# AlessioSam/LADiff

Measured on AMD Instinct MI355X. Metric: motions/sec (196-frame, 50-step DDIM, bs128), higher is better.
Workload: dtype f16x3+f32; 1 GPU; headline:ddim50_cfg7.5_b128_f196_c263_humanml3d; prompts_per_gpu=128, global_batch=128, frames=196, scheduler=ddim, denoising_steps=50, parallelism=dp1, loop=persistent pipeline kernel (16-row blocks x 86)

## Files before the change

### ladiff_amd/csrc/api.hip

```cpp
#include <algorithm>
#include <cstdlib>
#include <cstring>
#include <vector>

#include "model.h"
#include "sampler.h"
#include "../../include/ladiff_hip_debug.h"

using namespace ladiff;

namespace {

inline hipStream_t S(ladiff_stream_t s) { return reinterpret_cast<hipStream_t>(s); }

bool all_set(const float* const* w, size_t n) {
    if (w == nullptr) return false;
    for (size_t i = 0; i < n; ++i)
        if (w[i] == nullptr) return false;
    return true;
}
template <class W>
bool load_weights(W& dst, const float* const* ptrs) {
    if (!all_set(ptrs, sizeof(W) / sizeof(const float*))) return false;
    std::memcpy(&dst, ptrs, sizeof(W));
    return true;
}
const char* name_at(const std::vector<std::string>& n, int i) { return (i >= 0 && i < (int)n.size()) ? n[i].c_str() : nullptr; }

}

#ifdef LADIFF_STAMPS
static unsigned long long* g_stamps = nullptr;
#endif

extern "C" {

int ladiff_version(void) { return LADIFF_ABI_VERSION; }
int ladiff_split_format(void) {
#ifndef LADIFF_SPLIT_BF16
    return 1;
#else
    return 0;
#endif
}

const char* ladiff_error_string(int code) {
    switch (code) {
        case LADIFF_OK: return "ok";
        case LADIFF_ERR_ARG: return "invalid argument (null pointer or negative size)";
        case LADIFF_ERR_SHAPE: return "shape not supported by the gfx950 kernels";
        case LADIFF_ERR_WORKSPACE: return "workspace too small";
        case LADIFF_ERR_UNSUPPORTED: return "configuration branch not built";
        default: return code > 0 ? hipGetErrorString((hipError_t)code) : "unknown ladiff error";
    }
}

int ladiff_denoiser_num_params(void) { return DEN_NPARAMS; }
const char* ladiff_denoiser_param_name(int i) { return name_at(denoiser_param_names(), i); }
int ladiff_decoder_num_params(void) { return DEC_NPARAMS; }
const char* ladiff_decoder_param_name(int i) { return name_at(decoder_param_names(), i); }

int ladiff_gemm(const float* A, int lda, const float* A2, int lda2, int K1, const float* W, int ldw, const float* bias,
                const float* res, int ldres, const float* ln_gamma, const float* ln_beta, float* Y, int ldy, int M,
                int N, int K, int act, ladiff_stream_t stream) {
    LADIFF_CHECK_ARG(A && W && Y && M >= 0 && N > 0 && K > 0);
    GemmArgs g;
    g.A = A; g.lda = lda; g.A2 = A2; g.lda2 = lda2; g.K1 = A2 ? K1 : K; g.W = W; g.ldw = ldw; g.bias = bias;
    g.res = res; g.ldres = ldres; g.ln_g = ln_gamma; g.ln_b = ln_beta; g.Y = Y; g.ldy = ldy; g.M = M; g.N = N; g.K = K;
    g.act = act;
    return launch_gemm(g, S(stream));
}

int ladiff_gemm_resident(const float* A, int lda, const float* A2, int lda2, int K1, const float* W, int ldw,
                         const float* bias, const float* res, int ldres, float* Y, int ldy, int M, int N, int K, int act,
                         int split, float* Ys, ladiff_stream_t stream) {
    LADIFF_CHECK_ARG(A && W && (Y || Ys) && M >= 0 && N > 0 && K > 0);
    if (M == 0) return 0;
    KrArgs g;
    g.A = A; g.lda = lda; g.A2 = A2; g.lda2 = lda2; g.K1 = A2 ? K1 : K; g.W = W; g.ldw = ldw; g.bias = bias;
    g.res = res; g.ldres = ldres; g.Y = Y; g.ldy = ldy; g.M = M; g.N = N; g.K = K; g.act = act;
    g.split = split; g.Ys = Ys;
#ifdef LADIFF_STAMPS
    g.stamps = g_stamps;
#endif
    return launch_gemm_kr(g, S(stream));
}

int ladiff_gemm_split(const float* A, int lda, const float* A2, int lda2, int K1, const float* W, int ldw, const float* bias,
                      const float* res, int ldres, float* Y, float* Ys, int ldy, int M, int N, int K, int act,
                      ladiff_stream_t stream) {
    LADIFF_CHECK_ARG(A && W && (Y || Ys) && M >= 0 && N > 0 && K > 0);
    if (M == 0) return 0;
    GemmArgs g;
    g.A = A; g.lda = lda; g.A2 = A2; g.lda2 = lda2; g.K1 = A2 ? K1 : K; g.W = W; g.ldw = ldw; g.bias = bias;
    g.res = res; g.ldres = ldres; g.Y = Y; g.Ys = Ys; g.ldy = ldy; g.M = M; g.N = N; g.K = K; g.act = act; g.split = 1;
    return launch_gemm(g, S(stream));
}

#ifdef LADIFF_STAMPS
void ladiff_debug_set_stamps(unsigned long long* p) { g_stamps = p; }
void ladiff_debug_set_sys_stamps(unsigned long long* p) { ladiff::g_sys_stamps = p; }
void ladiff_debug_set_probe(int v) { ladiff::g_sys_probe = v; }
#endif

int ladiff_combine_rows(const float* partials, int n_planes, int M, const float* bias, const float* res, int mode,
                        const float* ln_gamma, const float* ln_beta, const float* table, const int32_t* counts, int Bs,
                        int T, int pad_row, float* out, ladiff_stream_t stream) {
    LADIFF_CHECK_ARG(partials && out && n_planes > 0 && M >= 0 && Bs > 0 && T > 0);
    if (mode != RED_PLAIN && mode != RED_LN && mode != RED_LN_ADD && mode != RED_LN_MOD) return LADIFF_ERR_ARG;
    if (mode != RED_PLAIN && !(ln_gamma && ln_beta)) return LADIFF_ERR_ARG;
    if ((mode == RED_LN_ADD || mode == RED_LN_MOD) && !table) return LADIFF_ERR_ARG;
    if (M == 0) return 0;
    return launch_reduce_rows(partials, n_planes, M, bias, res, mode, ln_gamma, ln_beta, table, 0, nullptr, counts, Bs, T,
                              pad_row, 0, out, nullptr, S(stream));
}

int ladiff_layernorm(const float* x, const float* gamma, const float* beta, float* y, int M, ladiff_stream_t stream) {
    LADIFF_CHECK_ARG(x && gamma && beta && y && M >= 0);
    return launch_layernorm(x, gamma, beta, y, M, S(stream));
}

int ladiff_timestep_sinusoid(const int64_t* timesteps, int n, float* out, ladiff_stream_t stream) {
    LADIFF_CHECK_ARG(timesteps && out && n >= 0);
    if (n == 0) return 0;
    return launch_sinusoid(timesteps, n, out, S(stream));
}

int ladiff_decoder_self_attention(const float* qkv, const int32_t* lengths, const uint32_t* keybits, float* out, int B,
                                  int F, ladiff_stream_t stream) {
    LADIFF_CHECK_ARG(qkv && (lengths || keybits) && out && B >= 0);
    return launch_decoder_self_attention(qkv, lengths, keybits, out, B, F, 0, S(stream));
}

int ladiff_self_attention_split(const float* qkv, const int32_t* lengths, const uint32_t* keybits, float* out, int B, int F,
                                 int nheads, int causal, ladiff_stream_t stream) {
    LADIFF_CHECK_ARG(qkv && out && B >= 0);
    return launch_self_attention_split(qkv, lengths, keybits, out, B, F, nheads, causal, 0, S(stream));
}

int ladiff_decoder_cross_attention(const float* q, const float* kv, const int32_t* counts, float* out, int B, int F,
                                   int T, ladiff_stream_t stream) {
    LADIFF_CHECK_ARG(q && kv && out && B >= 0 && F >= 0);
    return launch_decoder_cross_attention(q, kv, counts, out, B, F, T, 0, S(stream));
}

size_t ladiff_denoiser_tables_floats(int n_steps) { return den_tables_floats(n_steps); }
size_t ladiff_denoiser_text_cache_floats(int B2, int n_steps, int n_text) { return den_text_cache_floats(B2, n_steps, n_text); }
size_t ladiff_denoiser_workspace_bytes(int B2, int T, int n_steps, int n_text) {
    return sizeof(float) * std::max({den_forward_ws_floats(B2, T), den_time_layout(nullptr, n_steps).total,
                                     den_text_ws_floats(B2, n_steps, n_text), den_text_ws_floats(B2, n_steps, 1)});
}

int ladiff_denoiser_time_tables(const float* const* w, const float* sinusoid, int n_steps, float* tables, void* ws,
                                size_t ws_bytes, ladiff_stream_t stream) {
    DenoiserW W;
    LADIFF_CHECK_ARG(load_weights(W, w) && sinusoid && tables && ws && n_steps > 0);
    if (ws_bytes < ladiff_denoiser_workspace_bytes(1, 1, n_steps, 1)) return LADIFF_ERR_WORKSPACE;
    return denoiser_time_tables(W, sinusoid, n_steps, tables, (float*)ws, ws_bytes / sizeof(float), S(stream));
}

int ladiff_denoiser_text_cache(const float* const* w, const float* text_emb, int B2, int n_text, const float* tables, int n_steps,
                               float* cache, void* ws, size_t ws_bytes, ladiff_stream_t stream) {
    DenoiserW W;
    LADIFF_CHECK_ARG(load_weights(W, w) && text_emb && tables && cache && ws && B2 > 0 && n_steps > 0 && n_text >= 1);
    if (ws_bytes < ladiff_denoiser_workspace_bytes(B2, 1, n_steps, n_text)) return LADIFF_ERR_WORKSPACE;
    return denoiser_text_cache(W, text_emb, B2, tables, n_steps, cache, (float*)ws, ws_bytes / sizeof(float), S(stream), n_text);
}

int ladiff_denoiser_forward(const float* const* w, const float* const* w_split, const float* tables, const int32_t* d_step,
                            const float* text_cache, int n_text, int n_steps, const float* sample, int Bs, int dup, int T,
                            const int32_t* counts, float* eps, void* ws, size_t ws_bytes, ladiff_stream_t stream) {
    DenoiserW W, WS;
    LADIFF_CHECK_ARG(load_weights(W, w) && tables && d_step && text_cache && sample && eps && ws && Bs > 0 && dup > 0 && n_steps > 0 &&
                     n_text >= 1);
    if (w_split != nullptr) LADIFF_CHECK_ARG(load_weights(WS, w_split));
    if (T < 1 || T > LADIFF_MAX_LATENTS) return LADIFF_ERR_SHAPE;
    if (ws_bytes < ladiff_denoiser_workspace_bytes(Bs * dup, T, n_steps, n_text)) return LADIFF_ERR_WORKSPACE;
    return denoiser_forward(W, w_split ? &WS : nullptr, tables, d_step, text_cache, n_steps, sample, Bs, dup, T, counts, eps, (float*)ws,
                            ws_bytes / sizeof(float), S(stream), 0, -1, 0, n_text);
}

size_t ladiff_linear_cross_attention_workspace_bytes(int B, int T, int n_text) {
    return linear_cross_attention_ws_floats(B, T, n_text) * sizeof(float);
}
int ladiff_linear_cross_attention(const float* const* w, int layer, const float* x, const float* xf, const float* emb,
                                  const int32_t* counts, int B, int T, int n_text, float* out, void* ws, size_t ws_bytes,
                                  ladiff_stream_t stream) {
    DenoiserW W;
    LADIFF_CHECK_ARG(load_weights(W, w) && x && xf && emb && out && ws && B > 0);
    return linear_cross_attention(W, layer, x, xf, emb, counts, B, T, n_text, out, (float*)ws, ws_bytes / sizeof(float), S(stream));
}

int ladiff_cfg_scheduler_step(const float* eps, float* latents, const float* coef, const int32_t* d_step,
                              const float* step_noise, float guidance_scale, int cfg, int B, int T,
                              ladiff_stream_t stream) {
    LADIFF_CHECK_ARG(eps && latents && coef && d_step && B > 0 && T > 0);
    return launch_cfg_step(eps, latents, coef, d_step, step_noise, guidance_scale, cfg, B, T, S(stream));
}
int ladiff_advance_step(int32_t* d_step, ladiff_stream_t stream) {
    LADIFF_CHECK_ARG(d_step);
    return launch_advance(d_step, S(stream));
}
int ladiff_init_latents(const float* noise, const int32_t* counts, float sigma, float* latents, int B, int T,
                        ladiff_stream_t stream) {
    LADIFF_CHECK_ARG(noise && latents && B > 0 && T > 0);
    return launch_init_latents(noise, counts, sigma, latents, B, T, S(stream));
}
int ladiff_finalize_latents(const float* latents, const int32_t* counts, float* z, int B, int T, ladiff_stream_t stream) {
    LADIFF_CHECK_ARG(latents && z && B > 0 && T > 0);
    return launch_finalize_latents(latents, counts, z, B, T, S(stream));
}

int ladiff_sampler_create(void** sampler) {
    LADIFF_CHECK_ARG(sampler);
    *sampler = new Sampler();
    return 0;
}
int ladiff_sampler_destroy(void* sampler) {
    Sampler* sp = reinterpret_cast<Sampler*>(sampler);
    if (sp == nullptr) return 0;
    (void)hipDeviceSynchronize();
    sp->drain_retired();
    if (sp->exec) (void)hipGraphExecDestroy(sp->exec);
    if (sp->setup) (void)hipGraphExecDestroy(sp->setup);
    if (sp->ev0) (void)hipEventDestroy(sp->ev0);
    if (sp->ev1) (void)hipEventDestroy(sp->ev1);
    for (hipEvent_t e : sp->wev) (void)hipEventDestroy(e);
    sp->cap.destroy();
    delete sp;
    return 0;
}

int ladiff_reverse_plan(int B, int T, const int32_t* h_counts, int masked, int loop_mode, int f16x3, int cfg, int* rows_per_block, int* n_blocks) {
    LADIFF_CHECK_ARG(B >= 1 && T >= 1 && T <= LADIFF_MAX_LATENTS && loop_mode >= 1 && loop_mode <= 3 && rows_per_block && n_blocks);
    if (!cfg && masked && h_counts == nullptr) return LADIFF_ERR_UNSUPPORTED;
    std::vector<unsigned char> plan;
    int mr = 2, nb = 0;
    choose_plan(B, T, h_counts, masked != 0, loop_mode, f16x3 != 0, plan, &mr, &nb, cfg != 0);
    *rows_per_block = 16 * mr; *n_blocks = nb;
    return 0;
}

int ladiff_debug_set_stage_waves(int waves_per_simd) {
    LADIFF_CHECK_ARG(waves_per_simd == 1 || waves_per_simd == 2);
    g_waves16 = waves_per_simd;
    return 0;
}

int ladiff_debug_set_handoff(int tagged) {
    LADIFF_CHECK_ARG(tagged == 0 || tagged == 1);
    g_handoff = tagged;
    return 0;
}

int ladiff_debug_set_mlp_variant(int v) {
#ifdef LADIFF_STAMPS
    LADIFF_CHECK_ARG((v >= 0 && v <= 3) || (v >= 11 && v <= 17) || (v >= 21 && v <= 26));
#else
    LADIFF_CHECK_ARG(v >= 0 && v <= 3);
#endif
    g_mlp_variant = v;
    return 0;
}

int ladiff_debug_set_decoder_fusion(int on) {
    LADIFF_CHECK_ARG(on >= 0 && on <= 126 && (on & 3) != 3 && (on & 48) != 48);
    g_dec_out_cross = (on & 64) ? 0 : 1;
    g_dec_fused_mlp = on & 3;
    g_dec_small_rows_path = (on & 4) ? 0 : 1;
    g_dec_final_split = (on & 8) ? 0 : 1;
    g_dec_fused_attn = (on & 16) ? 0 : (on & 32) ? 2 : 1;
    return 0;
}

int ladiff_debug_set_stage_plan(int v) {
    LADIFF_CHECK_ARG(v >= 0 && v <= 1);
    g_stage_plan = v;
    return 0;
}

int ladiff_debug_set_poll_pause(int mask, int len) {
    LADIFF_CHECK_ARG(mask >= 0 && mask <= 255 && len >= 0 && len <= 64);
    g_poll_pause = mask | (len << 8);
    return 0;
}

int ladiff_debug_set_pacing(int eighths, int mask) {
    if (eighths == -1) { g_pace = -1; return 0; }
    LADIFF_CHECK_ARG(eighths >= 0 && eighths <= 8 && mask >= 0 && mask <= 255);
    g_pace = eighths | (mask << 8);
    return 0;
}

int ladiff_debug_set_stage_delay(int mask, int len) {
    LADIFF_CHECK_ARG(mask >= -1 && mask <= 255 && len >= 0 && len <= 64);
    g_stage_delay = mask < 0 ? -1 : (mask | (len << 8));
    return 0;
}

int ladiff_debug_set_loop_thresholds(int look_ahead_from, int small_upto) {
    LADIFF_CHECK_ARG(look_ahead_from >= -1 && small_upto >= -1);
    g_look_ahead_from = look_ahead_from;
    g_small_upto = small_upto;
    return 0;
}

int ladiff_debug_set_graph_epoch_rule(int on) {
    LADIFF_CHECK_ARG(on == 0 || on == 1);
    g_graph_epoch_rule = on;
    return 0;
}

int ladiff_debug_graph_instantiations(void) { return g_graph_instantiations.load(); }

int ladiff_debug_set_xcd_local(int on) {
    LADIFF_CHECK_ARG(on >= 0 && on <= 2);
    g_xcd_local = on;
    return 0;
}

int ladiff_sampler_set_loop(void* sampler, int mode) {
    Sampler* sp = reinterpret_cast<Sampler*>(sampler);
    LADIFF_CHECK_ARG(sp != nullptr && mode >= 0 && mode <= 3);
    sp->loop = mode != 0;
    sp->loop_mode = mode;
    return 0;
}

int ladiff_sampler_loop_ms(void* sampler, float* ms) {
    Sampler* sp = reinterpret_cast<Sampler*>(sampler);
    LADIFF_CHECK_ARG(sp != nullptr && ms != nullptr && sp->ev1 != nullptr);
    LADIFF_HIP(hipEventSynchronize(sp->ev1));
    LADIFF_HIP(hipEventElapsedTime(ms, sp->ev0, sp->ev1));
    return 0;
}

int ladiff_sampler_set_window_timing(void* sampler, int on) {
    Sampler* sp = reinterpret_cast<Sampler*>(sampler);
    LADIFF_CHECK_ARG(sp != nullptr);
    sp->time_windows = on != 0;
    return 0;
}

int ladiff_sampler_window_ms(void* sampler, float* loop_ms_sum, int* n_windows) {
    Sampler* sp = reinterpret_cast<Sampler*>(sampler);
    LADIFF_CHECK_ARG(sp != nullptr && loop_ms_sum != nullptr && n_windows != nullptr);
    float sum = 0.f;
    for (int i = 0; i < sp->n_windows; ++i) {
        float ms = 0.f;
        LADIFF_HIP(hipEventSynchronize(sp->wev[2 * i + 1]));
        LADIFF_HIP(hipEventElapsedTime(&ms, sp->wev[2 * i], sp->wev[2 * i + 1]));
        sum += ms;
    }
    *loop_ms_sum = sum; *n_windows = sp->n_windows;
    return 0;
}

int ladiff_sampler_last_loop(void* sampler, int* pipeline, int* rows_per_block, int* n_blocks) {
    Sampler* sp = reinterpret_cast<Sampler*>(sampler);
    LADIFF_CHECK_ARG(sp != nullptr && pipeline != nullptr);
    *pipeline = sp->last_pipeline;
    if (rows_per_block) *rows_per_block = sp->last_pipeline ? 16 * sp->plan_mr : 0;
    if (n_blocks) *n_blocks = sp->last_pipeline ? sp->plan_nb : 0;
    return 0;
}

int ladiff_sampler_set_noise_generator(void* sampler, uint64_t seed, uint32_t first_prompt, int enable) {
    Sampler* sp = reinterpret_cast<Sampler*>(sampler);
    LADIFF_CHECK_ARG(sp != nullptr);
    sp->gen = NoiseGen{(unsigned)(seed & 0xffffffffull), (unsigned)(seed >> 32), first_prompt, enable ? 1 : 0};
    return 0;
}

int ladiff_noise_fill(uint64_t seed, uint32_t first_prompt, int first_step, int n_steps, int B, int T, float* out, ladiff_stream_t stream) {
    LADIFF_CHECK_ARG(out != nullptr && first_step >= 0 && n_steps >= 0 && B >= 0);
    if (T < 1 || T > LADIFF_MAX_LATENTS) return LADIFF_ERR_SHAPE;
    return launch_noise_fill(NoiseGen{(unsigned)(seed & 0xffffffffull), (unsigned)(seed >> 32), first_prompt, 1}, first_step, n_steps, B, T, out,
                             S(stream));
}

int ladiff_sampler_set_fault(void* sampler, int workgroup, int timeout_ms) {
    Sampler* sp = reinterpret_cast<Sampler*>(sampler);
    LADIFF_CHECK_ARG(sp != nullptr && workgroup >= -1 && workgroup < 256 && timeout_ms >= 0);
    sp->fault_wg = workgroup;
    sp->timeout_ticks = (unsigned long long)timeout_ms * 100000ull;
    return 0;
}

size_t ladiff_reverse_status_offset_bytes(int B, int T, int n_steps, int n_text) {
    if (B < 1 || T < 1 || T > LADIFF_MAX_LATENTS || n_steps < 1 || n_text < 1) return 0;
    const ReverseWs r = carve_reverse(nullptr, B, T, n_steps, n_text);
    return (r.sys_off + sys_status_offset_floats(B, T)) * sizeof(float);
}

int ladiff_reverse_status(void* ws, int B, int T, int n_steps, int n_text, int* code, int* info) {
    LADIFF_CHECK_ARG(ws && code && B > 0 && n_steps > 0);
    if (T < 1 || T > LADIFF_MAX_LATENTS) return LADIFF_ERR_SHAPE;
    const ReverseWs r = carve_reverse(ws, B, T, n_steps, n_text);
    unsigned st[2] = {0u, 0u};
    LADIFF_HIP(hipMemcpy(st, r.sys + sys_status_offset_floats(B, T), sizeof(st), hipMemcpyDeviceToHost));
    *code = (int)st[0];
    if (info) *info = (int)st[1];
    return 0;
}

size_t ladiff_reverse_workspace_bytes(int B, int T, int n_steps, int n_text) { return carve_reverse(nullptr, B, T, n_steps, n_text).total_bytes; }

int ladiff_mlp_ln_fused(const float* xs, const float* x, const float* w1s, const float* b1, const float* w2s, const float* b2,
                        const float* ln_gamma, const float* ln_beta, const float* ln2_gamma, const float* ln2_beta, float* y, float* ys,
                        int M, ladiff_stream_t stream) {
    LADIFF_CHECK_ARG(xs && x && w1s && b1 && w2s && b2 && ln_gamma && ln_beta && (y || ys) && M >= 0);
    if ((ln2_gamma == nullptr) != (ln2_beta == nullptr)) return LADIFF_ERR_ARG;
    return launch_dec_mlp(xs, x, w1s, b1, w2s, b2, ln_gamma, ln_beta, ln2_gamma, ln2_beta, y, ys, M, S(stream));
}

int ladiff_split_rows(const float* x, float* y, int R, int K, ladiff_stream_t stream) {
    LADIFF_CHECK_ARG(x && y && R >= 0 && K > 0);
    if (K % 64) return LADIFF_ERR_SHAPE;
    if (R == 0) return 0;
    return launch_split_rows(x, y, R, K, S(stream));
}

int ladiff_gather_rows(const float* src, const int32_t* index, int n_rows, int row_floats, float* dst, ladiff_stream_t stream) {
    LADIFF_CHECK_ARG(n_rows >= 0 && row_floats > 0);
    if (n_rows == 0) return 0;
    LADIFF_CHECK_ARG(src && index && dst);
    if (row_floats % 4 || (reinterpret_cast<uintptr_t>(src) & 15) || (reinterpret_cast<uintptr_t>(dst) & 15)) return LADIFF_ERR_SHAPE;
    if ((reinterpret_cast<uintptr_t>(index) & 3) || n_rows > (1 << 30)) return LADIFF_ERR_SHAPE;
    return launch_gather_rows(src, index, n_rows, row_floats, dst, S(stream));
}

int ladiff_split_range_stats(const float* const* tensors, const int64_t* counts, int n, int64_t max_count, uint64_t* stats,
                             ladiff_stream_t stream) {
    LADIFF_CHECK_ARG(n >= 0 && max_count >= 0);
    if (n == 0) return 0;
    LADIFF_CHECK_ARG(tensors && counts && stats);
    if (n > 65535 || max_count >= (int64_t(1) << 32)) return LADIFF_ERR_SHAPE;
    return launch_split_range_stats(tensors, counts, n, max_count, reinterpret_cast<unsigned long long*>(stats), S(stream));
}

int ladiff_diffusion_reverse(void* sampler, const float* const* w, const float* const* w_split, uint64_t weights_generation,
                             const float* text_emb, const float* init_noise, const int32_t* counts, const int32_t* final_counts,
                             const int32_t* h_counts, const float* sinusoid, const float* coef, const float* step_noise, float guidance_scale,
                             float init_noise_sigma, int cfg, int B, int T, int n_text, int n_steps, float* z, void* ws, size_t ws_bytes,
                             int reuse_time_tables, ladiff_stream_t stream) {
    DenoiserW W, WS;
    LADIFF_CHECK_ARG(load_weights(W, w) && text_emb && init_noise && sinusoid && coef && z && ws && B > 0 && n_steps > 0);
    if (w_split != nullptr) LADIFF_CHECK_ARG(load_weights(WS, w_split));
    if (T < 1 || T > LADIFF_MAX_LATENTS || n_text < 1) return LADIFF_ERR_SHAPE;
    return diffusion_reverse(reinterpret_cast<Sampler*>(sampler), W, w_split ? &WS : nullptr,
                             ReverseArgs{w, w_split, weights_generation, text_emb, init_noise, counts, final_counts, h_counts, sinusoid, coef,
                                         step_noise, guidance_scale, init_noise_sigma, cfg, B, T, n_text, n_steps, z, ws, ws_bytes,
                                         reuse_time_tables, stream});
}

int ladiff_encoder_num_params(void) { return ENC_NPARAMS; }
const char* ladiff_encoder_param_name(int i) { return name_at(encoder_param_names(), i); }
size_t ladiff_encoder_workspace_bytes(int B, int F, int T, int C) { return enc_ws_floats(B, F, T, C) * sizeof(float); }

int ladiff_vae_encode(const float* const* w, const float* const* w_split, const float* features, const int32_t* lengths,
                      const int32_t* counts, const float* eps, int B, int F, int T, int C, float* mu, float* std,
                      float* latent, void* ws, size_t ws_bytes, ladiff_stream_t stream) {
    EncoderW W, WS;
    LADIFF_CHECK_ARG(load_weights(W, w) && features && lengths && counts && eps && mu && std && latent && ws && B >= 0);
    if (w_split != nullptr) LADIFF_CHECK_ARG(load_weights(WS, w_split));
    return vae_encode(W, w_split ? &WS : nullptr, features, lengths, counts, eps, B, F, T, C, mu, std, latent, (float*)ws,
                      ws_bytes / sizeof(float), S(stream));
}

int ladiff_clip_num_params(void) { return CLIP_NPARAMS; }
const char* ladiff_clip_param_name(int i) { return name_at(clip_param_names(), i); }
size_t ladiff_clip_workspace_bytes(int B, int L) { return clip_ws_floats(B, L) * sizeof(float); }

static bool load_clip(ClipW& dst, const float* const* ptrs, int n_layers) {
    if (ptrs == nullptr || n_layers < 1 || n_layers > CLIP_MAX_LAYERS) return false;
    const int n = CLIP_HEAD_NPARAMS + CLIP_LAYER_NPARAMS * n_layers;
    for (int i = 0; i < n; ++i)
        if (ptrs[i] == nullptr) return false;
    std::memset(&dst, 0, sizeof(dst));
    std::memcpy(&dst, ptrs, n * sizeof(const float*));
    return true;
}

int ladiff_clip_text_encode(const float* const* w, const float* const* w_split, int n_layers, int vocab, const int64_t* ids,
                            int B, int seq, int L, float* out, void* ws, size_t ws_bytes, ladiff_stream_t stream) {
    ClipW W, WS;
    LADIFF_CHECK_ARG(load_clip(W, w, n_layers) && ids && out && ws && B >= 0);
    if (w_split != nullptr) LADIFF_CHECK_ARG(load_clip(WS, w_split, n_layers));
    return clip_text_encode(W, w_split ? &WS : nullptr, n_layers, vocab, ids, B, seq, L, out, (float*)ws,
                            ws_bytes / sizeof(float), S(stream));
}

size_t ladiff_clip_workspace_bytes_ragged(int B, int total_rows) { return clip_ws_floats_rows(B, total_rows) * sizeof(float); }

int ladiff_clip_text_encode_ragged(const float* const* w, const float* const* w_split, int n_layers, int vocab, const int64_t* ids,
                                   int B, int seq, int L, const int32_t* seq_len, const int32_t* row_off, const int32_t* row_seq,
                                   int total_rows, float* out, void* ws, size_t ws_bytes, ladiff_stream_t stream) {
    ClipW W, WS;
    LADIFF_CHECK_ARG(load_clip(W, w, n_layers) && ids && out && ws && B >= 0 && seq_len && row_off && row_seq && total_rows >= 0);
    if (w_split != nullptr) LADIFF_CHECK_ARG(load_clip(WS, w_split, n_layers));
    return clip_text_encode(W, w_split ? &WS : nullptr, n_layers, vocab, ids, B, seq, L, out, (float*)ws,
                            ws_bytes / sizeof(float), S(stream), seq_len, row_off, row_seq, total_rows);
}

int ladiff_t2m_movement_num_params(void) { return (int)t2m_move_param_names().size(); }
const char* ladiff_t2m_movement_param_name(int i) { return name_at(t2m_move_param_names(), i); }
int ladiff_t2m_motion_num_params(void) { return (int)t2m_motion_param_names().size(); }
const char* ladiff_t2m_motion_param_name(int i) { return name_at(t2m_motion_param_names(), i); }
int ladiff_t2m_text_num_params(void) { return (int)t2m_text_param_names().size(); }
const char* ladiff_t2m_text_param_name(int i) { return name_at(t2m_text_param_names(), i); }
size_t ladiff_t2m_movement_workspace_bytes(int B, int F, int Cin) { return t2m_move_ws_floats(B, F, Cin) * sizeof(float); }
size_t ladiff_t2m_motion_workspace_bytes(int B, int T) { return t2m_motion_ws_floats(B, T) * sizeof(float); }
size_t ladiff_t2m_text_workspace_bytes(int B, int L) { return t2m_text_ws_floats(B, L) * sizeof(float); }

int ladiff_t2m_movement_encode(const float* const* w, const float* feats, int ld, int B, int F, int Cin, float* out, void* ws,
                               size_t ws_bytes, ladiff_stream_t stream) {
    LADIFF_CHECK_ARG(all_set(w, t2m_move_param_names().size()) && feats && out && ws && B >= 0);
    return t2m_movement_encode(w, feats, ld, B, F, Cin, out, (float*)ws, ws_bytes / sizeof(float), S(stream));
}
int ladiff_t2m_motion_encode(const float* const* w, const float* movements, const int32_t* m_lens, int B, int T, float* out,
                             void* ws, size_t ws_bytes, ladiff_stream_t stream) {
    LADIFF_CHECK_ARG(all_set(w, t2m_motion_param_names().size()) && movements && m_lens && out && ws && B >= 0);
    return t2m_motion_encode(w, movements, m_lens, B, T, out, (float*)ws, ws_bytes / sizeof(float), S(stream));
}
int ladiff_t2m_text_encode(const float* const* w, const float* word_embs, const float* pos_onehot, const int32_t* cap_lens,
                           int B, int L, float* out, void* ws, size_t ws_bytes, ladiff_stream_t stream) {
    LADIFF_CHECK_ARG(all_set(w, t2m_text_param_names().size()) && word_embs && pos_onehot && cap_lens && out && ws && B >= 0);
    return t2m_text_encode(w, word_embs, pos_onehot, cap_lens, B, L, out, (float*)ws, ws_bytes / sizeof(float), S(stream));
}

int ladiff_feats2joints(const float* feats, const float* mean, const float* std, int B, int F, int C, int njoints,
                        float* joints, ladiff_stream_t stream) {
    LADIFF_CHECK_ARG(feats && mean && std && joints && B >= 0);
    return launch_feats2joints(feats, mean, std, B, F, C, njoints, joints, S(stream));
}

namespace {
int joint_metrics_check(const void* rst, const void* ref, const int32_t* h_lengths, int B, int F, int J, const void* seq_rows, const void* acc) {
    if (J != 21 && J != 22) return LADIFF_ERR_SHAPE;
    if (F < 1 || F > LADIFF_MAX_FRAMES) return LADIFF_ERR_SHAPE;
    for (int b = 0; b < B; ++b)
        if (h_lengths[b] < 1 || h_lengths[b] > F) return LADIFF_ERR_SHAPE;
    if ((reinterpret_cast<uintptr_t>(rst) & 3) || (reinterpret_cast<uintptr_t>(ref) & 3) || (reinterpret_cast<uintptr_t>(seq_rows) & 3) ||
        (reinterpret_cast<uintptr_t>(acc) & 7))
        return LADIFF_ERR_SHAPE;
    return 0;
}
}

int ladiff_joint_ape_ave(const float* joints_rst, const float* joints_ref, const int32_t* lengths, const int32_t* h_lengths, int B, int F,
                         int J, const int32_t* h_part_idx, float factor, float* seq_rows, double* acc, ladiff_stream_t stream) {
    LADIFF_CHECK_ARG(B >= 0);
    if (B == 0) return 0;
    LADIFF_CHECK_ARG(joints_rst && joints_ref && lengths && h_lengths && h_part_idx && seq_rows && acc && factor > 0.f);
    LADIFF_TRY(joint_metrics_check(joints_rst, joints_ref, h_lengths, B, F, J, seq_rows, acc));
    if (reinterpret_cast<uintptr_t>(lengths) & 3) return LADIFF_ERR_SHAPE;
    for (int i = 0; i < 8; ++i)
        if (h_part_idx[i] < 0 || h_part_idx[i] >= (i < 4 ? J - 1 : J)) return LADIFF_ERR_SHAPE;
    return launch_joint_ape_ave(joints_rst, joints_ref, lengths, B, F, J, h_part_idx, factor, seq_rows, acc, S(stream));
}

int ladiff_joint_mr(const float* joints_rst, const float* joints_ref, const int32_t* h_lengths, int B, int F, int J, float* seq_rows,
                    double* acc, ladiff_stream_t stream) {
    LADIFF_CHECK_ARG(B >= 0);
    if (B == 0) return 0;
    LADIFF_CHECK_ARG(joints_rst && joints_ref && h_lengths && seq_rows && acc);
    LADIFF_TRY(joint_metrics_check(joints_rst, joints_ref, h_lengths, B, F, J, seq_rows, acc));
    return launch_joint_mr(joints_rst, joints_ref, B, F, J, seq_rows, acc, S(stream));
}

size_t ladiff_decoder_workspace_bytes(int B, int F, int T, int C) {
    (void)C;
    return dec_ws_floats(B, (size_t)B * F, T) * sizeof(float);
}

int ladiff_vae_decode(const float* const* w, const float* const* w_split, const float* z, const int32_t* lengths,
                      const int32_t* counts, int B, int F, int T, int C, float* feats, void* ws, size_t ws_bytes,
                      ladiff_stream_t stream) {
    DecoderW W, WS;
    LADIFF_CHECK_ARG(load_weights(W, w) && z && lengths && feats && ws && B >= 0);
    if (w_split != nullptr) LADIFF_CHECK_ARG(load_weights(WS, w_split));
    return vae_decode(W, w_split ? &WS : nullptr, z, lengths, counts, nullptr, 0, B, F, T, C, feats, (float*)ws, ws_bytes / sizeof(float),
                      S(stream));
}

namespace {
struct DecodeGraph {
    hipGraphExec_t exec = nullptr;
    GraphSlot slot;
    CaptureStream cap;
};
}

int ladiff_decoder_graph_create(void** graph) {
    LADIFF_CHECK_ARG(graph);
    *graph = new DecodeGraph();
    return 0;
}
int ladiff_decoder_graph_destroy(void* graph) {
    DecodeGraph* g = reinterpret_cast<DecodeGraph*>(graph);
    if (g == nullptr) return 0;
    (void)hipDeviceSynchronize();
    if (g->exec) (void)hipGraphExecDestroy(g->exec);
    g->cap.destroy();
    delete g;
    return 0;
}

int ladiff_vae_decode_graphed(void* graph, const float* const* w, const float* const* w_split, uint64_t weights_generation, const float* z,
                              const int32_t* lengths, const int32_t* counts, const int32_t* row_off, int total_rows, int B, int F, int T,
                              int C, float* feats, void* ws, size_t ws_bytes, ladiff_stream_t stream) {
    DecodeGraph* dg = reinterpret_cast<DecodeGraph*>(graph);
    DecoderW W, WS;
    LADIFF_CHECK_ARG(dg && load_weights(W, w) && z && lengths && feats && ws && B >= 0 && stream != nullptr);
    if (w_split != nullptr) LADIFF_CHECK_ARG(load_weights(WS, w_split));
    if (F < 1 || F > LADIFF_MAX_FRAMES || T < 1 || T > LADIFF_MAX_LATENTS || C < 1) return LADIFF_ERR_SHAPE;
    if (ws_bytes < ladiff_decoder_workspace_bytes(B, F, T, C)) return LADIFF_ERR_WORKSPACE;
    hipStream_t s = S(stream);
    const GraphKey key = decode_key(w, w_split, DEC_NPARAMS, weights_generation, z, lengths, counts, row_off, total_rows, B, F, T, C, feats, ws,
                                    stream, g_dec_fused_mlp, g_dec_small_rows_path, g_dec_final_split, g_mlp_variant, g_dec_fused_attn);
    if (!(dg->exec && dg->slot.key == key && dg->slot.newest())) {
        if (dg->exec) { LADIFF_HIP(hipStreamSynchronize(s)); (void)hipGraphExecDestroy(dg->exec); dg->exec = nullptr; }
        LADIFF_TRY(dec_mlp_prepare());
        LADIFF_TRY(dec_qkv_attn_prepare());
        LADIFF_TRY(dec_cross_prepare());
        LADIFF_TRY(dg->cap.ensure());
        LADIFF_TRY(capture_graph(dg->cap.s, [&](hipStream_t cs) {
            if (row_off != nullptr) LADIFF_TRY(launch_zero_fill(feats, (size_t)B * F * C, cs));
            return vae_decode(W, w_split ? &WS : nullptr, z, lengths, counts, row_off, total_rows, B, F, T, C, feats, (float*)ws,
                              ws_bytes / sizeof(float), cs);
        }, &dg->exec));
        dg->slot.stamp(key);
    }
    LADIFF_HIP(hipGraphLaunch(dg->exec, s));
    return 0;
}

int ladiff_vae_decode_ragged(const float* const* w, const float* const* w_split, const float* z, const int32_t* lengths,
                             const int32_t* counts, const int32_t* row_off, int total_rows, int B, int F, int T, int C, float* feats,
                             void* ws, size_t ws_bytes, ladiff_stream_t stream) {
    DecoderW W, WS;
    LADIFF_CHECK_ARG(load_weights(W, w) && z && lengths && row_off && feats && ws && B >= 0 && total_rows >= 0);
    if (w_split != nullptr) LADIFF_CHECK_ARG(load_weights(WS, w_split));
    if (F < 1 || F > LADIFF_MAX_FRAMES || T < 1 || T > LADIFF_MAX_LATENTS || C < 1) return LADIFF_ERR_SHAPE;
    if (ws_bytes < ladiff_decoder_workspace_bytes(B, F, T, C)) return LADIFF_ERR_WORKSPACE;
    LADIFF_HIP(hipMemsetAsync(feats, 0, (size_t)B * F * C * sizeof(float), S(stream)));
    return vae_decode(W, w_split ? &WS : nullptr, z, lengths, counts, row_off, total_rows, B, F, T, C, feats, (float*)ws,
                      ws_bytes / sizeof(float), S(stream));
}

}
```

### ladiff_amd/csrc/attention.hip

```cpp
#include "kernels.h"

namespace ladiff {

constexpr int SA_FMAX = LADIFF_MAX_FRAMES;
constexpr int SA_NKT = SA_FMAX / 32;

struct AttnGeom { int nheads, ld, koff, voff, out_ld, causal; };

__global__ __launch_bounds__(256) void dec_self_attn_kernel(const float* __restrict__ qkv, const int32_t* __restrict__ lengths,
                                                            const uint32_t* __restrict__ keybits, float* __restrict__ out,
                                                            int B, int F, int split_out, const AttnGeom g,
                                                            const int32_t* __restrict__ row_off, int shared_qkv) {
    __shared__ __attribute__((aligned(16))) float Ks[SA_FMAX * DH];
    __shared__ __attribute__((aligned(16))) float Vs[SA_FMAX * DH];
    const int tid = threadIdx.x, lane = tid & 63, wave = tid >> 6;
    const int b = blockIdx.y / g.nheads, h = blockIdx.y % g.nheads;
    int len = F;
    uint32_t kb[SA_NKT + 1];
    if (keybits != nullptr) {
        len = 1;
#pragma unroll
        for (int i = 0; i < SA_NKT; ++i) {
            kb[i] = keybits[(size_t)b * 8 + i];
            if (kb[i]) len = 32 * i + 32 - __builtin_clz(kb[i]);
        }
        len = len > F ? F : len;
    } else {
        len = lengths != nullptr ? lengths[b] : F;
        len = len < 1 ? 1 : (len > F ? F : len);
#pragma unroll
        for (int i = 0; i < SA_NKT; ++i) kb[i] = len >= 32 * i + 32 ? 0xFFFFFFFFu : (len > 32 * i ? (1u << (len - 32 * i)) - 1u : 0u);
    }
    const int nkt = (len + 31) >> 5;
    size_t row0 = (size_t)b * F;
    if (row_off != nullptr) { row0 = row_off[b]; F = row_off[b + 1] - row_off[b]; }
    const size_t base = (shared_qkv ? (size_t)0 : row0) * g.ld + h * DH;

    for (int id = tid; id < nkt * 32 * 16; id += 256) {
        const int r = id >> 4, c = id & 15;
        f32x4 kk = {0.f, 0.f, 0.f, 0.f}, vv = {0.f, 0.f, 0.f, 0.f};
        if (r < F) {
            const float* src = qkv + base + (size_t)r * g.ld + c * 4;
            kk = ld4(src + g.koff);
            vv = ld4(src + g.voff);
        }
        st4(Ks + r * DH + ((c ^ (r & 15)) << 2), kk);
        st4(Vs + r * DH + c * 4, vv);
    }
    __syncthreads();

    const int qt = blockIdx.x * 4 + wave;
    if (qt * 32 >= F) return;
    const int q = lane & 31, h2 = lane >> 5;
    const int qrow = qt * 32 + q;

    f32x4 qf[8];
#pragma unroll
    for (int g8 = 0; g8 < 8; ++g8) {
        f32x4 v = {0.f, 0.f, 0.f, 0.f};
        if (qrow < F) v = ld4(qkv + base + (size_t)qrow * g.ld + g8 * 8 + h2 * 4);
#pragma unroll
        for (int e = 0; e < 4; ++e) v[e] *= 0.125f;
        qf[g8] = v;
    }

    f32x16 sT[SA_NKT];
    float m = -INFINITY;
#pragma unroll
    for (int kt = 0; kt < SA_NKT; ++kt) {
        if (kt < nkt) {
            f32x16 acc;
#pragma unroll
            for (int i = 0; i < 16; ++i) acc[i] = 0.f;
            const int r = kt * 32 + q;
#pragma unroll
            for (int g8 = 0; g8 < 8; ++g8) {
                const f32x4 a = ld4(Ks + r * DH + ((((g8 << 1) + h2) ^ (r & 15)) << 2));
#pragma unroll
                for (int e = 0; e < 4; ++e) acc = __builtin_amdgcn_mfma_f32_32x32x2f32(a[e], qf[g8][e], acc, 0, 0, 0);
            }
#pragma unroll
            for (int i = 0; i < 16; ++i) {
                const int kin = (i & 3) + 8 * (i >> 2) + 4 * h2;
                const bool ok = ((kb[kt] >> kin) & 1u) && (!g.causal || kt * 32 + kin <= qrow);
                const float s = ok ? acc[i] : -INFINITY;
                acc[i] = s;
                m = fmaxf(m, s);
            }
            sT[kt] = acc;
        }
    }
    m = fmaxf(m, __shfl_xor(m, 32, 64));

    float l = 0.f;
#pragma unroll
    for (int kt = 0; kt < SA_NKT; ++kt) {
        if (kt < nkt) {
#pragma unroll
            for (int i = 0; i < 16; ++i) {
                const float pv = expf(sT[kt][i] - m);
                sT[kt][i] = pv;
                l += pv;
            }
        }
    }
    l += __shfl_xor(l, 32, 64);

    f32x16 o0, o1;
#pragma unroll
    for (int i = 0; i < 16; ++i) { o0[i] = 0.f; o1[i] = 0.f; }
#pragma unroll
    for (int kt = 0; kt < SA_NKT; ++kt) {
        if (kt < nkt) {
#pragma unroll
            for (int i = 0; i < 16; ++i) {
                const int key = kt * 32 + (i & 3) + 8 * (i >> 2) + 4 * h2;
                const float a0 = Vs[key * DH + q];
                const float a1 = Vs[key * DH + 32 + q];
                o0 = __builtin_amdgcn_mfma_f32_32x32x2f32(a0, sT[kt][i], o0, 0, 0, 0);
                o1 = __builtin_amdgcn_mfma_f32_32x32x2f32(a1, sT[kt][i], o1, 0, 0, 0);
            }
        }
    }

    if (qrow < F) {
        const float inv = 1.f / l;
        float* rowp = out + (row0 + qrow) * g.out_ld;
        const int c0 = h * DH + 4 * h2;
#pragma unroll
        for (int rg = 0; rg < 4; ++rg) {
            f32x4 v0, v1;
#pragma unroll
            for (int e = 0; e < 4; ++e) { v0[e] = o0[4 * rg + e] * inv; v1[e] = o1[4 * rg + e] * inv; }
            if (split_out) {
                store_split4(rowp, c0 + 8 * rg, v0);
                store_split4(rowp, c0 + 32 + 8 * rg, v1);
            } else {
                st4(rowp + c0 + 8 * rg, v0);
                st4(rowp + c0 + 32 + 8 * rg, v1);
            }
        }
    }
}


__device__ __forceinline__ void split8(const float (&v)[8], s16x8& hi, s16x8& lo) {
    split8(f32x4{v[0], v[1], v[2], v[3]}, f32x4{v[4], v[5], v[6], v[7]}, hi, lo);
}

template <int FM, int NT>
__global__ __launch_bounds__(NT, NT == 64 ? 2 : 1) void self_attn_split_kernel(const float* __restrict__ qkv, const int32_t* __restrict__ lengths,
                                                               const uint32_t* __restrict__ keybits, float* __restrict__ out,
                                                               int B, int F, int split_out, const AttnGeom g,
                                                               const int32_t* __restrict__ row_off, int shared_qkv) {
    constexpr int NKT = FM / 32, IT = FM * 16 / NT, VLD = FM + 8;
    static_assert(FM % 32 == 0 && (FM * 16) % NT == 0 && NT % 64 == 0 && (FM / 4) % (NT / 64) == 0 && NT / 64 >= FM / 32, "a wave per query tile");
    __shared__ __attribute__((aligned(16))) s16 Kp[2 * FM * DH];
    __shared__ __attribute__((aligned(16))) s16 Vt[2 * DH * VLD];
    s16* const Kh = Kp; s16* const Kl = Kp + FM * DH;
    s16* const Vth = Vt; s16* const Vtl = Vt + DH * VLD;
    float* const Vtmp = reinterpret_cast<float*>(Kp);
    const int tid = threadIdx.x, lane = tid & 63, wave = tid >> 6;
    const int b = blockIdx.x / g.nheads, h = blockIdx.x % g.nheads;
    int len = F;
    uint32_t kb[NKT + 1];
    if (keybits != nullptr) {
        len = 1;
#pragma unroll
        for (int i = 0; i < NKT; ++i) {
            kb[i] = keybits[(size_t)b * 8 + i];
            if (kb[i]) len = 32 * i + 32 - __builtin_clz(kb[i]);
        }
        len = len > F ? F : len;
    } else {
        len = lengths != nullptr ? lengths[b] : F;
        len = len < 1 ? 1 : (len > F ? F : len);
#pragma unroll
        for (int i = 0; i < NKT; ++i) kb[i] = len >= 32 * i + 32 ? 0xFFFFFFFFu : (len > 32 * i ? (1u << (len - 32 * i)) - 1u : 0u);
    }
    const int nkt = (len + 31) >> 5;
    size_t row0 = (size_t)b * F;
    if (row_off != nullptr) { row0 = row_off[b]; F = row_off[b + 1] - row_off[b]; }
    const size_t base = (shared_qkv ? (size_t)0 : row0) * g.ld + h * DH;

    const int qt = wave;
    const int q = lane & 31, h2 = lane >> 5;
    const int qrow = qt * 32 + q;

    s16x8 qh[4], ql[4];
#pragma unroll
    for (int ks = 0; ks < 4; ++ks) {
        float v[8] = {0.f, 0.f, 0.f, 0.f, 0.f, 0.f, 0.f, 0.f};
        if (qrow < F) {
            const f32x4 a = ld4(qkv + base + (size_t)qrow * g.ld + 16 * ks + 8 * h2);
            const f32x4 c = ld4(qkv + base + (size_t)qrow * g.ld + 16 * ks + 8 * h2 + 4);
#pragma unroll
            for (int e = 0; e < 4; ++e) { v[e] = a[e] * (0.125f * 1.4426950408889634f); v[4 + e] = c[e] * (0.125f * 1.4426950408889634f); }
        }
        split8(v, qh[ks], ql[ks]);
    }


    f32x4 kk[IT], vv[IT];
#pragma unroll
    for (int it = 0; it < IT; ++it) {
        const int id = tid + it * NT, r = id >> 4, c = id & 15;
        kk[it] = f32x4{0.f, 0.f, 0.f, 0.f}; vv[it] = kk[it];
        if (r < nkt * 32 && r < F) {
            const float* src = qkv + base + (size_t)r * g.ld + c * 4;
            kk[it] = ld4(src + g.koff);
            vv[it] = ld4(src + g.voff);
        }
    }
#pragma unroll
    for (int it = 0; it < IT; ++it) {
        const int id = tid + it * NT, r = id >> 4, c = id & 15;
        if (r < nkt * 32) st4(Vtmp + r * DH + c * 4, vv[it]);
    }
    __syncthreads();
    {
        const int d = tid & 63, kg = tid >> 6;
        for (int p = 0; p < FM / 4 / (NT / 64); ++p) {
            const int k0 = (p * (NT / 64) + kg) * 4;
            if (k0 < nkt * 32) {
                s16x4 hi, lo;
                split4(Vtmp[k0 * DH + d], Vtmp[(k0 + 1) * DH + d], Vtmp[(k0 + 2) * DH + d], Vtmp[(k0 + 3) * DH + d], hi, lo);
                *reinterpret_cast<s16x4*>(Vth + d * VLD + k0) = hi;
                *reinterpret_cast<s16x4*>(Vtl + d * VLD + k0) = lo;
            }
        }
    }
    __syncthreads();
#pragma unroll
    for (int it = 0; it < IT; ++it) {
        const int id = tid + it * NT, r = id >> 4, c = id & 15;
        if (r < nkt * 32) {
            s16x4 hi, lo;
            split4(kk[it], hi, lo);
            const int off = r * DH + ((((c >> 1) ^ ((r >> 1) & 7)) << 3) | ((c & 1) << 2));
            *reinterpret_cast<s16x4*>(Kh + off) = hi;
            *reinterpret_cast<s16x4*>(Kl + off) = lo;
        }
    }
    __syncthreads();

    if (qt * 32 >= F) return;

    f32x16 sT[NKT];
    float m = -INFINITY;
#pragma unroll
    for (int kt = 0; kt < NKT; ++kt) {
        if (kt < nkt) {
            f32x16 acc;
#pragma unroll
            for (int i = 0; i < 16; ++i) acc[i] = 0.f;
            const int r = kt * 32 + q;
#pragma unroll
            for (int ks = 0; ks < 4; ++ks) {
                const int off = r * DH + (((2 * ks + h2) ^ ((r >> 1) & 7)) << 3);
                const s16x8 kh = *reinterpret_cast<const s16x8*>(Kh + off);
                const s16x8 kl = *reinterpret_cast<const s16x8*>(Kl + off);
                acc = MFMA32_S16(kl, qh[ks], acc, 0, 0, 0);
                acc = MFMA32_S16(kh, ql[ks], acc, 0, 0, 0);
                acc = MFMA32_S16(kh, qh[ks], acc, 0, 0, 0);
            }
            if (kb[kt] == 0xFFFFFFFFu && !g.causal) {
#pragma unroll
                for (int i = 0; i < 16; ++i) m = fmaxf(m, acc[i]);
            } else {
#pragma unroll
                for (int i = 0; i < 16; ++i) {
                    const int kin = (i & 3) + 8 * (i >> 2) + 4 * h2;
                    const bool ok = ((kb[kt] >> kin) & 1u) && (!g.causal || kt * 32 + kin <= qrow);
                    const float s = ok ? acc[i] : -INFINITY;
                    acc[i] = s;
                    m = fmaxf(m, s);
                }
            }
            sT[kt] = acc;
        }
    }
    m = fmaxf(m, __shfl_xor(m, 32, 64));

    float l = 0.f;
#pragma unroll
    for (int kt = 0; kt < NKT; ++kt) {
        if (kt < nkt) {
#pragma unroll
            for (int i = 0; i < 16; ++i) {
                const float pv = __builtin_amdgcn_exp2f(sT[kt][i] - m);
                sT[kt][i] = pv;
                l += pv;
            }
        }
    }
    l += __shfl_xor(l, 32, 64);

    f32x16 o0, o1;
#pragma unroll
    for (int i = 0; i < 16; ++i) { o0[i] = 0.f; o1[i] = 0.f; }
#pragma unroll
    for (int kt = 0; kt < NKT; ++kt) {
        if (kt < nkt) {
#pragma unroll
            for (int mm = 0; mm < 2; ++mm) {
                float pv[8];
#pragma unroll
                for (int j = 0; j < 8; ++j) pv[j] = sT[kt][8 * mm + j];
                s16x8 ph, pl;
                split8(pv, ph, pl);
                const int k1 = 32 * kt + 16 * mm + 4 * h2;
#pragma unroll
                for (int t = 0; t < 2; ++t) {
                    const int voff = (32 * t + q) * VLD + k1;
                    const s16x4 h_a = *reinterpret_cast<const s16x4*>(Vth + voff), h_b = *reinterpret_cast<const s16x4*>(Vth + voff + 8);
                    const s16x4 l_a = *reinterpret_cast<const s16x4*>(Vtl + voff), l_b = *reinterpret_cast<const s16x4*>(Vtl + voff + 8);
                    const s16x8 vh = {h_a[0], h_a[1], h_a[2], h_a[3], h_b[0], h_b[1], h_b[2], h_b[3]};
                    const s16x8 vl = {l_a[0], l_a[1], l_a[2], l_a[3], l_b[0], l_b[1], l_b[2], l_b[3]};
                    f32x16& o = t == 0 ? o0 : o1;
                    o = MFMA32_S16(vl, ph, o, 0, 0, 0);
                    o = MFMA32_S16(vh, pl, o, 0, 0, 0);
                    o = MFMA32_S16(vh, ph, o, 0, 0, 0);
                }
            }
        }
    }

    if (qrow < F) {
        const float inv = 1.f / l;
        float* rowp = out + (row0 + qrow) * g.out_ld;
        const int c0 = h * DH + 4 * h2;
#pragma unroll
        for (int rg = 0; rg < 4; ++rg) {
            f32x4 v0, v1;
#pragma unroll
            for (int e = 0; e < 4; ++e) { v0[e] = o0[4 * rg + e] * inv; v1[e] = o1[4 * rg + e] * inv; }
            if (split_out) {
                store_split4(rowp, c0 + 8 * rg, v0);
                store_split4(rowp, c0 + 32 + 8 * rg, v1);
            } else {
                st4(rowp + c0 + 8 * rg, v0);
                st4(rowp + c0 + 32 + 8 * rg, v1);
            }
        }
    }
}

int launch_self_attention_split(const float* qkv, const int32_t* lengths, const uint32_t* keybits, float* out, int B, int F,
                                 int nheads, int causal, int split_out, hipStream_t s, const int32_t* row_off, int shared_qkv) {
    if (F > SA_FMAX || F < 1 || nheads < 1) return LADIFF_ERR_SHAPE;
    if (B == 0) return 0;
    const int W = nheads * DH;
    const AttnGeom g{nheads, 3 * W, W, 2 * W, W, causal};
    if (F <= 32) hipLaunchKernelGGL((self_attn_split_kernel<32, 64>), dim3(B * nheads), dim3(64), 0, s, qkv, lengths, keybits, out, B, F, split_out, g, row_off, shared_qkv);
    else hipLaunchKernelGGL((self_attn_split_kernel<SA_FMAX, 512>), dim3(B * nheads), dim3(512), 0, s, qkv, lengths, keybits, out, B, F, split_out, g, row_off, shared_qkv);
    LADIFF_LAUNCH_CHECK();
    return 0;
}

int launch_self_attention(const float* qkv, const int32_t* lengths, const uint32_t* keybits, float* out, int B, int F, int nheads,
                          int causal, int split_out, hipStream_t s, const int32_t* row_off) {
    if (F > SA_FMAX || F < 1 || nheads < 1) return LADIFF_ERR_SHAPE;
    if (B == 0) return 0;
    const int W = nheads * DH;
    const AttnGeom g{nheads, 3 * W, W, 2 * W, W, causal};
    const int nqt = (F + 31) / 32;
    hipLaunchKernelGGL(dec_self_attn_kernel, dim3((nqt + 3) / 4, B * nheads), dim3(256), 0, s, qkv, lengths, keybits, out, B, F,
                       split_out, g, row_off, 0);
    LADIFF_LAUNCH_CHECK();
    return 0;
}

int launch_decoder_self_attention(const float* qkv, const int32_t* lengths, const uint32_t* keybits, float* out, int B, int F,
                                  int split_out, hipStream_t s, const int32_t* row_off, int shared_qkv) {
    if (F > SA_FMAX || F < 1) return LADIFF_ERR_SHAPE;
    if (lengths == nullptr && keybits == nullptr) return LADIFF_ERR_ARG;
    if (B == 0) return 0;
    const AttnGeom g{H, 3 * D, D, 2 * D, D, 0};
    const int nqt = (F + 31) / 32;
    hipLaunchKernelGGL(dec_self_attn_kernel, dim3((nqt + 3) / 4, B * H), dim3(256), 0, s, qkv, lengths, keybits, out, B, F,
                       split_out, g, row_off, shared_qkv);
    LADIFF_LAUNCH_CHECK();
    return 0;
}

template <int T>
__global__ __launch_bounds__(256) void dec_cross_attn_kernel(const float* __restrict__ q, const float* __restrict__ kv,
                                                             const int32_t* __restrict__ counts, float* __restrict__ out,
                                                             int B, int F, int M, int split_out) {
    const int row = blockIdx.x * 4 + (threadIdx.x >> 6);
    if (row >= M) return;
    const int c = (threadIdx.x & 63) * 4;
    const int b = row / F;
    int nv = counts ? counts[b] : T;
    nv = nv < 1 ? 1 : (nv > T ? T : nv);
    f32x4 qv = ld4(q + (size_t)row * D + c);
    float s[T];
    float m = -INFINITY;
#pragma unroll
    for (int j = 0; j < T; ++j) {
        const f32x4 kk = ld4(kv + ((size_t)j * B + b) * 512 + c);
        float d = (qv[0] * 0.125f) * kk[0] + (qv[1] * 0.125f) * kk[1] + (qv[2] * 0.125f) * kk[2] + (qv[3] * 0.125f) * kk[3];
        d = row16_sum(d);
        s[j] = j < nv ? d : -INFINITY;
        m = fmaxf(m, s[j]);
    }
    float l = 0.f;
    f32x4 o = {0.f, 0.f, 0.f, 0.f};
#pragma unroll
    for (int j = 0; j < T; ++j) {
        const float pv = expf(s[j] - m);
        l += pv;
        const f32x4 vv = ld4(kv + ((size_t)j * B + b) * 512 + 256 + c);
#pragma unroll
        for (int e = 0; e < 4; ++e) o[e] += pv * vv[e];
    }
    const float inv = 1.f / l;
#pragma unroll
    for (int e = 0; e < 4; ++e) o[e] *= inv;
    if (split_out) store_split4(out + (size_t)row * D, c, o);
    else st4(out + (size_t)row * D + c, o);
}

int launch_decoder_cross_attention(const float* q, const float* kv, const int32_t* counts, float* out, int B, int F,
                                   int T, int split_out, hipStream_t s) {
    const int M = B * F;
    if (M == 0) return 0;
    const dim3 grid((M + 3) / 4), block(256);
#define LADIFF_CA_CASE(TT) \
    case TT: hipLaunchKernelGGL(dec_cross_attn_kernel<TT>, grid, block, 0, s, q, kv, counts, out, B, F, M, split_out); break;
    switch (T) {
        LADIFF_CA_CASE(1) LADIFF_CA_CASE(2) LADIFF_CA_CASE(3) LADIFF_CA_CASE(4)
        LADIFF_CA_CASE(5) LADIFF_CA_CASE(6) LADIFF_CA_CASE(7) LADIFF_CA_CASE(8)
        default: return LADIFF_ERR_SHAPE;
    }
#undef LADIFF_CA_CASE
    LADIFF_LAUNCH_CHECK();
    return 0;
}

template <int T>
__global__ __launch_bounds__(256) void den_self_attn_kernel(const float* __restrict__ qkv, const float* __restrict__ text_kv,
                                                            const float* __restrict__ tables, int kv_off, int step_stride,
                                                            const int32_t* __restrict__ d_step,
                                                            const int32_t* __restrict__ counts, int Bs, int b_off,
                                                            float* __restrict__ out, int split_out) {
    const int b2 = blockIdx.x;
    const int bg = b_off + b2;
    const int col = threadIdx.x;
    float qv[T], kk[T + 2], vv[T + 2];
#pragma unroll
    for (int i = 0; i < T; ++i) {
        const float* r = qkv + ((size_t)b2 * T + i) * 768 + col;
        qv[i] = r[0] * 0.125f;
        kk[i] = r[256];
        vv[i] = r[512];
    }
    kk[T] = text_kv[(size_t)bg * 512 + col];
    vv[T] = text_kv[(size_t)bg * 512 + 256 + col];
    const float* tk = tables + (size_t)(*d_step) * step_stride + kv_off;
    kk[T + 1] = tk[col];
    vv[T + 1] = tk[256 + col];
    int nv = counts ? counts[bg % Bs] : T;
    nv = nv > T ? T : nv;
    __shared__ __attribute__((aligned(16))) float so[T * D];
#pragma unroll
    for (int i = 0; i < T; ++i) {
        float s[T + 2];
        float m = -INFINITY;
#pragma unroll
        for (int j = 0; j < T + 2; ++j) {
            const float d = wave_sum(qv[i] * kk[j]);
            s[j] = (j < T && j >= nv) ? -INFINITY : d;
            m = fmaxf(m, s[j]);
        }
        float l = 0.f, o = 0.f;
#pragma unroll
        for (int j = 0; j < T + 2; ++j) {
            const float pv = expf(s[j] - m);
            l += pv;
            o += pv * vv[j];
        }
        if (split_out) so[i * D + col] = o / l;
        else out[((size_t)b2 * T + i) * D + col] = o / l;
    }
    if (split_out) {
        __syncthreads();
        for (int u = threadIdx.x; u < T * (D / 4); u += 256) {
            const int r = u / (D / 4), c4 = (u % (D / 4)) * 4;
            store_split4(out + ((size_t)b2 * T + r) * D, c4, ld4(so + r * D + c4));
        }
    }
}

int launch_denoiser_self_attention(const float* qkv, const float* text_kv, const float* tables, int kv_off,
                                   int step_stride, const int32_t* d_step, const int32_t* counts, int Bs, int b_off,
                                   int b_n, int T, float* out, int split_out, hipStream_t s) {
    if (b_n == 0) return 0;
    const dim3 grid(b_n), block(256);
#define LADIFF_SA_CASE(TT)                                                                                          \
    case TT:                                                                                                        \
        hipLaunchKernelGGL(den_self_attn_kernel<TT>, grid, block, 0, s, qkv, text_kv, tables, kv_off, step_stride, \
                           d_step, counts, Bs, b_off, out, split_out);                                                                \
        break;
    switch (T) {
        LADIFF_SA_CASE(1) LADIFF_SA_CASE(2) LADIFF_SA_CASE(3) LADIFF_SA_CASE(4)
        LADIFF_SA_CASE(5) LADIFF_SA_CASE(6) LADIFF_SA_CASE(7) LADIFF_SA_CASE(8)
        default: return LADIFF_ERR_SHAPE;
    }
#undef LADIFF_SA_CASE
    LADIFF_LAUNCH_CHECK();
    return 0;
}

}
```

### ladiff_amd/csrc/dec_cross.hip

```cpp
#include <mutex>
#include "kernels.h"
#include "tile_mma.h"

namespace ladiff { extern unsigned long long* g_sys_stamps; }

namespace ladiff {

namespace {
constexpr int TM = LADIFF_MAX_LATENTS;
}

__global__ __launch_bounds__(256) void dec_cross_prep_kernel(const DecCrossPrepBatch pb, int B, int T, int tiles_per_wg) {
    const int h = blockIdx.y, layer = blockIdx.z, tid = threadIdx.x, lane = tid & 63, c16 = lane & 15, kq = lane >> 4;
    const int wave = __builtin_amdgcn_readfirstlane(tid >> 6);
    const float* __restrict__ kv = pb.kv[layer]; const float* __restrict__ wq = pb.wq[layer]; const float* __restrict__ bq = pb.bq[layer];
    const float* __restrict__ wo = pb.wo[layer]; float* __restrict__ gu = pb.gu[layer];
    float* __restrict__ cc = gu + (size_t)B * H * T * 2 * D;
    const int M = T * B, ntiles = (M + 15) / 16;
    float gq[4][16], uo[4][16], bqv[16];
#pragma unroll
    for (int t = 0; t < 4; ++t) {
        const int n = 64 * wave + 16 * t + c16;
#pragma unroll
        for (int s = 0; s < 16; ++s) gq[t][s] = wq[(size_t)(h * DH + 16 * kq + s) * D + n];
#pragma unroll
        for (int s4 = 0; s4 < 16; s4 += 4) {
            const f32x4 w4 = ld4(wo + (size_t)n * D + h * DH + 16 * kq + s4);
#pragma unroll
            for (int e = 0; e < 4; ++e) uo[t][s4 + e] = w4[e];
        }
    }
#pragma unroll
    for (int s4 = 0; s4 < 16; s4 += 4) {
        const f32x4 b4 = ld4(bq + h * DH + 16 * kq + s4);
#pragma unroll
        for (int e = 0; e < 4; ++e) bqv[s4 + e] = b4[e];
    }
    const int tile1 = (blockIdx.x + 1) * tiles_per_wg < ntiles ? (blockIdx.x + 1) * tiles_per_wg : ntiles;
    for (int tile = blockIdx.x * tiles_per_wg; tile < tile1; ++tile) {
        const int arow = 16 * tile + c16 < M ? 16 * tile + c16 : M - 1;
        const float* kr = kv + (size_t)arow * 2 * D + h * DH + 16 * kq;
        float ak[16], av[16];
#pragma unroll
        for (int s4 = 0; s4 < 16; s4 += 4) {
            const f32x4 k4 = ld4(kr + s4), v4 = ld4(kr + D + s4);
#pragma unroll
            for (int e = 0; e < 4; ++e) { ak[s4 + e] = k4[e]; av[s4 + e] = v4[e]; }
        }
        f32x4 ag[4], au[4];
#pragma unroll
        for (int t = 0; t < 4; ++t) { ag[t] = f32x4{0.f, 0.f, 0.f, 0.f}; au[t] = ag[t]; }
#pragma unroll
        for (int s = 0; s < 16; ++s)
#pragma unroll
            for (int t = 0; t < 4; ++t) {
                ag[t] = __builtin_amdgcn_mfma_f32_16x16x4f32(ak[s], gq[t][s], ag[t], 0, 0, 0);
                au[t] = __builtin_amdgcn_mfma_f32_16x16x4f32(av[s], uo[t][s], au[t], 0, 0, 0);
            }
#pragma unroll
        for (int i = 0; i < 4; ++i) {
            const int bt = 16 * tile + 4 * kq + i;
            if (bt < M) {
                const int j = bt / B, b = bt - j * B;
                float* o = gu + ((((size_t)b * H + h) * T + j) * 2) * D + 64 * wave + c16;
#pragma unroll
                for (int t = 0; t < 4; ++t) { o[16 * t] = ag[t][i] * 0.125f; o[D + 16 * t] = au[t][i]; }
            }
        }
        if (wave == 0) {
            float c = 0.f;
#pragma unroll
            for (int s = 0; s < 16; ++s) c = fmaf(bqv[s], ak[s], c);
            c += __shfl_xor(c, 16, 64); c += __shfl_xor(c, 32, 64);
            const int bt = 16 * tile + c16;
            if (kq == 0 && bt < M) { const int j = bt / B, b = bt - j * B; cc[((size_t)b * H + h) * T + j] = c * 0.125f; }
        }
    }
}

template <int T>
__device__ __forceinline__ void cross_row(const f32x4 (&xv)[4], f32x4 (&acc)[4], const float* sm, const float* cs, int nv, int c0) {
#pragma unroll 1
    for (int h = 0; h < H; ++h) {
        float sc[T];
#pragma unroll
        for (int j = 0; j < T; ++j) {
            const float* gp = sm + ((size_t)(h * T + j) * 2) * D + c0;
            float d = 0.f;
#pragma unroll
            for (int k = 0; k < 4; ++k) {
                const f32x4 g4 = ld4(gp + 64 * k);
                d = fmaf(xv[k][0], g4[0], fmaf(xv[k][1], g4[1], fmaf(xv[k][2], g4[2], fmaf(xv[k][3], g4[3], d))));
            }
            sc[j] = d;
        }
#pragma unroll
        for (int j = 0; j < T; ++j) sc[j] = row16_sum(sc[j]) + cs[h * T + j];
        float m = -INFINITY;
#pragma unroll
        for (int j = 0; j < T; ++j) { sc[j] = j < nv ? sc[j] : -INFINITY; m = fmaxf(m, sc[j]); }
        float l = 0.f;
#pragma unroll
        for (int j = 0; j < T; ++j) { sc[j] = __builtin_amdgcn_exp2f((sc[j] - m) * 1.4426950408889634f); l += sc[j]; }
        const float inv = 1.f / l;
#pragma unroll
        for (int j = 0; j < T; ++j) {
            const float pj = sc[j] * inv;
            const float* up = sm + ((size_t)(h * T + j) * 2 + 1) * D + c0;
#pragma unroll
            for (int k = 0; k < 4; ++k) {
                const f32x4 u4 = ld4(up + 64 * k);
                acc[k][0] = fmaf(pj, u4[0], acc[k][0]); acc[k][1] = fmaf(pj, u4[1], acc[k][1]);
                acc[k][2] = fmaf(pj, u4[2], acc[k][2]); acc[k][3] = fmaf(pj, u4[3], acc[k][3]);
            }
        }
    }
}

template <int TT>
__global__ __launch_bounds__(256) void dec_cross_apply_kernel(const float* __restrict__ x, const float* __restrict__ gu,
                                                              const float* __restrict__ cc, const int32_t* __restrict__ counts,
                                                              const float* __restrict__ bo, const float* __restrict__ g2,
                                                              const float* __restrict__ b2, int F, int rows_per_wg,
                                                              float* __restrict__ y, float* __restrict__ ys,
                                                              const int32_t* __restrict__ row_off, const float* __restrict__ g1,
                                                              const float* __restrict__ b1) {
    extern __shared__ __attribute__((aligned(16))) float sm[];
    constexpr int T = TT, HT = H * TT;
    const int b = blockIdx.x, tid = threadIdx.x, lane = tid & 63, wave = tid >> 6;
    const float* src = gu + (size_t)b * HT * 2 * D;
    for (int u = tid; u < HT * 2 * D / 4; u += 256) st4(sm + 4 * u, ld4(src + 4 * u));
    float* cs = sm + (size_t)HT * 2 * D;
    if (tid < HT) cs[tid] = cc[(size_t)b * HT + tid];
    int nv = counts != nullptr ? counts[b] : T;
    nv = nv > T ? T : nv;
    __syncthreads();
    const int l16 = lane & 15, grp = lane >> 4, c0 = 4 * l16;
    f32x4 bo4[4], gg[4], bb[4];
#pragma unroll
    for (int k = 0; k < 4; ++k) { bo4[k] = ld4(bo + c0 + 64 * k); gg[k] = ld4(g2 + c0 + 64 * k); bb[k] = ld4(b2 + c0 + 64 * k); }
    size_t row0 = (size_t)b * F;
    if (row_off != nullptr) { row0 = row_off[b]; F = row_off[b + 1] - row_off[b]; }
    const int f0 = blockIdx.y * rows_per_wg;
    const int f1 = f0 + rows_per_wg < F ? f0 + rows_per_wg : F;
    for (int fb = f0; fb < f1; fb += 16) {
        const int f = fb + 4 * wave + grp;
        const bool live = f < f1;
        const size_t row = row0 + (live ? f : f1 - 1);
        f32x4 xv[4], acc[4];
#pragma unroll
        for (int k = 0; k < 4; ++k) xv[k] = ld4(x + row * D + c0 + 64 * k);
        if (g1 != nullptr) {
            float s1 = 0.f;
#pragma unroll
            for (int k = 0; k < 4; ++k) s1 += (xv[k][0] + xv[k][1]) + (xv[k][2] + xv[k][3]);
            const float mean1 = row16_sum(s1) * (1.f / 256.f);
            float q1 = 0.f;
#pragma unroll
            for (int k = 0; k < 4; ++k)
#pragma unroll
                for (int i = 0; i < 4; ++i) { const float dlt = xv[k][i] - mean1; q1 += dlt * dlt; }
            const float rstd1 = rsqrtf(row16_sum(q1) * (1.f / 256.f) + LN_EPS);
#pragma unroll
            for (int k = 0; k < 4; ++k) {
                const f32x4 ga = ld4(g1 + c0 + 64 * k), be = ld4(b1 + c0 + 64 * k);
#pragma unroll
                for (int i = 0; i < 4; ++i) xv[k][i] = (xv[k][i] - mean1) * rstd1 * ga[i] + be[i];
            }
        }
#pragma unroll
        for (int k = 0; k < 4; ++k)
#pragma unroll
            for (int i = 0; i < 4; ++i) acc[k][i] = bo4[k][i] + xv[k][i];
        cross_row<T>(xv, acc, sm, cs, nv, c0);
        float sum = 0.f;
#pragma unroll
        for (int k = 0; k < 4; ++k) sum += (acc[k][0] + acc[k][1]) + (acc[k][2] + acc[k][3]);
        const float mean = row16_sum(sum) * (1.f / 256.f);
        float q = 0.f;
#pragma unroll
        for (int k = 0; k < 4; ++k)
#pragma unroll
            for (int i = 0; i < 4; ++i) { const float dlt = acc[k][i] - mean; q += dlt * dlt; }
        const float rstd = rsqrtf(row16_sum(q) * (1.f / 256.f) + LN_EPS);
        if (live) {
#pragma unroll
            for (int k = 0; k < 4; ++k) {
                f32x4 o;
#pragma unroll
                for (int i = 0; i < 4; ++i) o[i] = (acc[k][i] - mean) * rstd * gg[k][i] + bb[k][i];
                st4(y + row * D + c0 + 64 * k, o);
                if (ys != nullptr) store_split4(ys + row * D, c0 + 64 * k, o);
            }
        }
    }
}


constexpr int OC_ROWS = 32;
constexpr int OC_TILE = OC_ROWS * 1024;
constexpr int OC_CT = OC_ROWS * CLD * 4;
constexpr int OC_XN = OC_ROWS * CLD * 4;
constexpr int OC_SLD = 36;
constexpr int OC_PS = 8 * OC_ROWS * OC_SLD * 4;
constexpr int OC_PT = OC_ROWS * 256;

struct OutCrossArgs {
    const float* att;
    const float* x0;
    const float* wo;
    const float* bo; const float* g1; const float* b1;
    const float* gu; const float* cc;
    const float* bo_c; const float* g2; const float* b2;
    const int32_t* counts; const int32_t* row_off;
    float* y; float* ys;
    int F, rows_per_wg;
    unsigned long long* stamps;
};

#ifdef LADIFF_STAMPS
#define OC_STAMP(i) do { if (p.stamps != nullptr && blockIdx.x == 3 && blockIdx.y == 0 && threadIdx.x == 0 && npass < 6) p.stamps[npass * 16 + (i)] = __builtin_amdgcn_s_memrealtime(); } while (0)
#else
#define OC_STAMP(i) do { } while (0)
#endif

__device__ __forceinline__ void oc_barrier() { asm volatile("s_waitcnt lgkmcnt(0)\n\ts_barrier" ::: "memory"); }

template <int TT>
__global__ __launch_bounds__(512, 1) void dec_out_cross_kernel(const OutCrossArgs p) {
    __shared__ __attribute__((aligned(1024))) char tile[OC_TILE];
    __shared__ __attribute__((aligned(1024))) char ps_b[OC_PS];
    __shared__ __attribute__((aligned(1024))) char ct_b[OC_CT];
    __shared__ __attribute__((aligned(1024))) char xn_b[OC_XN];
    __shared__ __attribute__((aligned(16))) float sc[OC_ROWS * OC_SLD];
    __shared__ __attribute__((aligned(256))) char ptile[OC_PT];
    __shared__ __attribute__((aligned(16))) float vec[6 * D];
    __shared__ float cs[32];
    constexpr int T = TT, HT = H * TT;
    static_assert(HT <= 32, "the (head, token) columns fit one k-step");
    float* ct = reinterpret_cast<float*>(ct_b);
    float* xn = reinterpret_cast<float*>(xn_b);
    float* ps = reinterpret_cast<float*>(ps_b);
    const int b = blockIdx.x, tid = threadIdx.x, lane = tid & 63, frow = lane & 15, fk = lane >> 4;
    const int wave = __builtin_amdgcn_readfirstlane(tid >> 6);
    int npass = 0;
    OC_STAMP(15);
    WFrag<0, 2, 1> gf, uf;
    {
        const float* gub = p.gu + (size_t)b * HT * 2 * D;
#pragma unroll
        for (int j = 0; j < 2; ++j) {
            const int hj = 16 * j + frow;
            f32x4 a = {0.f, 0.f, 0.f, 0.f}, c = a;
            if (hj < HT) { const float* g = gub + (size_t)hj * 2 * D + 32 * wave + 8 * fk; a = ld4(g); c = ld4(g + 4); }
            split8(a, c, gf.hi[j][0], gf.lo[j][0]);
            const int col = 32 * wave + 16 * j + frow;
            f32x4 u0 = {0.f, 0.f, 0.f, 0.f}, u1 = u0;
#pragma unroll
            for (int e = 0; e < 4; ++e) {
                if (8 * fk + e < HT) u0[e] = gub[((size_t)(8 * fk + e) * 2 + 1) * D + col];
                if (8 * fk + 4 + e < HT) u1[e] = gub[((size_t)(8 * fk + 4 + e) * 2 + 1) * D + col];
            }
            split8(u0, u1, uf.hi[j][0], uf.lo[j][0]);
        }
        if (tid < 32) cs[tid] = tid < HT ? p.cc[(size_t)b * HT + tid] : 0.f;
        const float* vs[6] = {p.bo, p.g1, p.b1, p.bo_c, p.g2, p.b2};
        if (tid < 6 * (D / 4)) st4(vec + 4 * tid, ld4(vs[tid / (D / 4)] + 4 * (tid % (D / 4))));
    }
    WFrag<0, 2, 8> wf;
    {
#pragma unroll 1
        for (int half = 0; half < 2; ++half) {
            if (half == 1) __syncthreads();
#pragma unroll
            for (int qq = 0; qq < 4; ++qq) {
                const int q = (qq + b) & 3;
                char* dst = q == 0 ? tile : q == 1 ? ps_b : q == 2 ? ct_b : xn_b;
#pragma unroll
                for (int kk = 0; kk < 4; ++kk) {
                    const int lr32 = wave + 8 * kk, r = 32 * q + lr32;
                    const char* src = reinterpret_cast<const char*>(p.wo) + ((size_t)(128 * half + r) << 10) + ((lane & 48) << 4) + ((((lane & 15) ^ r) & 15) << 4);
                    __builtin_amdgcn_global_load_lds(reinterpret_cast<const float*>(src), (__attribute__((address_space(3))) void*)(dst + lr32 * 1024), 16, 0, 0);
                }
            }
            __builtin_amdgcn_s_waitcnt(0xF70);
            __syncthreads();
            if ((wave >> 2) == half) {
                const int q = wave & 3;
                const char* srcb = q == 0 ? tile : q == 1 ? ps_b : q == 2 ? ct_b : xn_b;
#pragma unroll
                for (int j = 0; j < 2; ++j)
#pragma unroll
                    for (int st = 0; st < 8; ++st) {
                        const int r = 16 * j + frow;
                        wf.hi[j][st] = *reinterpret_cast<const s16x8*>(a_slot<4>(const_cast<char*>(srcb), r, st >> 1, 4 * (st & 1) + fk));
                        wf.lo[j][st] = *reinterpret_cast<const s16x8*>(a_slot<4>(const_cast<char*>(srcb), r, st >> 1, 8 + 4 * (st & 1) + fk));
                    }
            }
        }
        __syncthreads();
    }
    int nv = p.counts != nullptr ? p.counts[b] : T;
    nv = nv > T ? T : nv;
    int F = p.F;
    size_t row0 = (size_t)b * F;
    if (p.row_off != nullptr) { row0 = p.row_off[b]; F = p.row_off[b + 1] - p.row_off[b]; }
    const int f0 = blockIdx.y * p.rows_per_wg;
    const int f1 = f0 + p.rows_per_wg < F ? f0 + p.rows_per_wg : F;
    if (f0 >= f1) return;
    const int l16 = lane & 15, grp = lane >> 4, c0 = 4 * l16, lr = 4 * wave + grp;
    typedef unsigned u32x4_o __attribute__((ext_vector_type(4)));
    const float* x0s = ps;
    auto dma_att = [&](int fb) {
#pragma unroll
        for (int i = 0; i < 4; ++i) {
            const int r = wave + 8 * i, f = fb + r < f1 ? fb + r : f1 - 1;
            unsigned vo = ((lane & 48) << 4) + ((((lane & 15) ^ r) & 15) << 4);
            asm volatile("" : "+v"(vo));
            const char* src = reinterpret_cast<const char*>(p.att) + ((row0 + f) << 10) + vo;
            __builtin_amdgcn_global_load_lds(reinterpret_cast<const float*>(src), (__attribute__((address_space(3))) void*)(tile + r * 1024), 16, 0, 0);
        }
    };
    auto dma_x0 = [&](int fb) {
#pragma unroll
        for (int i = 0; i < 4; ++i) {
            const int r = wave + 8 * i, f = fb + r < f1 ? fb + r : f1 - 1;
            unsigned vo = lane << 4;
            asm volatile("" : "+v"(vo));
            const char* src = reinterpret_cast<const char*>(p.x0) + ((row0 + f) << 10) + vo;
            __builtin_amdgcn_global_load_lds(reinterpret_cast<const float*>(src), (__attribute__((address_space(3))) void*)(ps_b + r * 1024), 16, 0, 0);
        }
    };
    dma_att(f0);
    dma_x0(f0);
    __builtin_amdgcn_s_waitcnt(0xF70);
    __syncthreads();
    for (int fb = f0; fb < f1; fb += OC_ROWS, ++npass) {
        OC_STAMP(0);
        OC_STAMP(1);
        f32x4 acc2[2][2];
        zero_acc(acc2);
        mma<0, 4, 2, 8, 2>(tile, wf, acc2);
        OC_STAMP(2);
        const int f = fb + lr;
        const bool live = f < f1;
        const size_t row = row0 + (live ? f : f1 - 1);
        f32x4 xv[4];
        stage_c(ct, acc2, [&](int j) { return 32 * wave + 16 * j; });
        __builtin_amdgcn_s_waitcnt(0xF70);
        __syncthreads();
        OC_STAMP(3);
        {
            const float* cr = ct + lr * CLD + c0;
#pragma unroll
            for (int k = 0; k < 4; ++k) {
                const f32x4 o = ld4(cr + 64 * k), bo = ld4(vec + c0 + 64 * k), r0 = ld4(x0s + lr * D + c0 + 64 * k);
#pragma unroll
                for (int i = 0; i < 4; ++i) xv[k][i] = (o[i] + bo[i]) + r0[i];
            }
            float s1 = 0.f;
#pragma unroll
            for (int k = 0; k < 4; ++k) s1 += (xv[k][0] + xv[k][1]) + (xv[k][2] + xv[k][3]);
            const float mean1 = row16_sum(s1) * (1.f / 256.f);
            float q1 = 0.f;
#pragma unroll
            for (int k = 0; k < 4; ++k)
#pragma unroll
                for (int i = 0; i < 4; ++i) { const float dlt = xv[k][i] - mean1; q1 += dlt * dlt; }
            const float rstd1 = rsqrtf(row16_sum(q1) * (1.f / 256.f) + LN_EPS);
#pragma unroll
            for (int k = 0; k < 4; ++k) {
                const f32x4 ga = ld4(vec + D + c0 + 64 * k), be = ld4(vec + 2 * D + c0 + 64 * k);
#pragma unroll
                for (int i = 0; i < 4; ++i) xv[k][i] = (xv[k][i] - mean1) * rstd1 * ga[i] + be[i];
                st4(xn + lr * CLD + c0 + 64 * k, xv[k]);
                tile_put4<0, 4>(tile, lr, c0 + 64 * k, xv[k]);
            }
        }
        OC_STAMP(4);
        __syncthreads();
        OC_STAMP(5);
        {
            u32x4_o ah[2], al[2];
#pragma unroll
            for (int i = 0; i < 2; ++i) {
                ah[i] = *reinterpret_cast<const u32x4_o*>(a_slot<4>(tile, 16 * i + frow, wave >> 1, 4 * (wave & 1) + fk));
                al[i] = *reinterpret_cast<const u32x4_o*>(a_slot<4>(tile, 16 * i + frow, wave >> 1, 8 + 4 * (wave & 1) + fk));
            }
            f32x4 as[2][2];
            zero_acc(as);
#pragma unroll
            for (int i = 0; i < 2; ++i)
#pragma unroll
                for (int j = 0; j < 2; ++j) as[i][j] = MFMA16_S16(__builtin_bit_cast(s16x8, al[i]), gf.hi[j][0], as[i][j], 0, 0, 0);
#pragma unroll
            for (int i = 0; i < 2; ++i)
#pragma unroll
                for (int j = 0; j < 2; ++j) as[i][j] = MFMA16_S16(__builtin_bit_cast(s16x8, ah[i]), gf.lo[j][0], as[i][j], 0, 0, 0);
#pragma unroll
            for (int i = 0; i < 2; ++i)
#pragma unroll
                for (int j = 0; j < 2; ++j) as[i][j] = MFMA16_S16(__builtin_bit_cast(s16x8, ah[i]), gf.hi[j][0], as[i][j], 0, 0, 0);
            float* pw = ps + wave * (OC_ROWS * OC_SLD);
#pragma unroll
            for (int i = 0; i < 2; ++i)
#pragma unroll
                for (int j = 0; j < 2; ++j)
#pragma unroll
                    for (int r = 0; r < 4; ++r) pw[(16 * i + 4 * fk + r) * OC_SLD + 16 * j + frow] = as[i][j][r];
        }
        __syncthreads();
        OC_STAMP(6);
        if (fb + OC_ROWS < f1) dma_att(fb + OC_ROWS);
        {
            float tot[2];
#pragma unroll
            for (int u = 0; u < 2; ++u) {
                const int hj = 16 * u + l16;
                float a = 0.f;
#pragma unroll
                for (int w = 0; w < 8; ++w) a += ps[w * (OC_ROWS * OC_SLD) + lr * OC_SLD + hj];
                tot[u] = a + cs[hj];
                sc[lr * OC_SLD + hj] = tot[u];
            }
            asm volatile("s_waitcnt lgkmcnt(0)" ::: "memory");
            __builtin_amdgcn_wave_barrier();
            float hs[2][T];
            int hh[2], jj[2];
#pragma unroll
            for (int u = 0; u < 2; ++u) {
                const int hj = 16 * u + l16;
                hh[u] = hj < HT ? hj / T : 0; jj[u] = hj - hh[u] * T;
#pragma unroll
                for (int t = 0; t < T; ++t) hs[u][t] = sc[lr * OC_SLD + hh[u] * T + t];
            }
#pragma unroll
            for (int u = 0; u < 2; ++u) {
                const int hj = 16 * u + l16;
                float m = -INFINITY, l = 0.f;
#pragma unroll
                for (int t = 0; t < T; ++t) m = t < nv ? fmaxf(m, hs[u][t]) : m;
#pragma unroll
                for (int t = 0; t < T; ++t) l += t < nv ? __builtin_amdgcn_exp2f((hs[u][t] - m) * 1.4426950408889634f) : 0.f;
                float pr = __builtin_amdgcn_exp2f((tot[u] - m) * 1.4426950408889634f) / l;
                if (!(hj < HT && jj[u] < nv)) pr = 0.f;
                tile_put1<0, 1>(ptile, lr, hj, pr);
            }
        }
        oc_barrier();
        OC_STAMP(7);
        f32x4 ao[2][2];
        zero_acc(ao);
        mma<0, 1, 2, 1, 2>(ptile, uf, ao);
        stage_c(ct, ao, [&](int j) { return 32 * wave + 16 * j; });
        __builtin_amdgcn_s_waitcnt(0xF70);
        oc_barrier();
        OC_STAMP(8);
        {
            const float* cr = ct + lr * CLD + c0;
            f32x4 acc[4];
#pragma unroll
            for (int k = 0; k < 4; ++k) {
                const f32x4 o = ld4(cr + 64 * k), bc = ld4(vec + 3 * D + c0 + 64 * k), x1 = ld4(xn + lr * CLD + c0 + 64 * k);
#pragma unroll
                for (int i = 0; i < 4; ++i) acc[k][i] = (bc[i] + x1[i]) + o[i];
            }
            if (fb + OC_ROWS < f1) dma_x0(fb + OC_ROWS);
            float sum = 0.f;
#pragma unroll
            for (int k = 0; k < 4; ++k) sum += (acc[k][0] + acc[k][1]) + (acc[k][2] + acc[k][3]);
            const float mean = row16_sum(sum) * (1.f / 256.f);
            float q = 0.f;
#pragma unroll
            for (int k = 0; k < 4; ++k)
#pragma unroll
                for (int i = 0; i < 4; ++i) { const float dlt = acc[k][i] - mean; q += dlt * dlt; }
            const float rstd = rsqrtf(row16_sum(q) * (1.f / 256.f) + LN_EPS);
            if (live) {
#pragma unroll
                for (int k = 0; k < 4; ++k) {
                    const f32x4 ga = ld4(vec + 4 * D + c0 + 64 * k), be = ld4(vec + 5 * D + c0 + 64 * k);
                    f32x4 o;
#pragma unroll
                    for (int i = 0; i < 4; ++i) o[i] = (acc[k][i] - mean) * rstd * ga[i] + be[i];
                    st4(p.y + row * D + c0 + 64 * k, o);
                    if (p.ys != nullptr) store_split4(p.ys + row * D, c0 + 64 * k, o);
                }
            }
        }
        OC_STAMP(9);
    }
}

int dec_cross_prepare() {
    static std::mutex mu;
    static bool attr_set[64] = {};
    int dev = 0;
    LADIFF_HIP(hipGetDevice(&dev));
    if (dev < 0 || dev >= 64) return LADIFF_ERR_ARG;
    std::lock_guard<std::mutex> lock(mu);
    if (!attr_set[dev]) {
        LADIFF_HIP(hipFuncSetAttribute(reinterpret_cast<const void*>(dec_cross_apply_kernel<8>), hipFuncAttributeMaxDynamicSharedMemorySize,
                                       (int)(((size_t)H * TM * 2 * D + H * TM) * sizeof(float))));
        const void* oc[8] = {reinterpret_cast<const void*>(dec_out_cross_kernel<1>), reinterpret_cast<const void*>(dec_out_cross_kernel<2>),
                             reinterpret_cast<const void*>(dec_out_cross_kernel<3>), reinterpret_cast<const void*>(dec_out_cross_kernel<4>),
                             reinterpret_cast<const void*>(dec_out_cross_kernel<5>), reinterpret_cast<const void*>(dec_out_cross_kernel<6>),
                             reinterpret_cast<const void*>(dec_out_cross_kernel<7>), reinterpret_cast<const void*>(dec_out_cross_kernel<8>)};
        for (int t = 1; t <= 8; ++t)
            (void)oc[t - 1];
        attr_set[dev] = true;
    }
    return 0;
}

int launch_decoder_cross_prep(const DecCrossPrepBatch& pb, int n, int B, int T, hipStream_t s) {
    if (B == 0 || n == 0) return 0;
    if (T < 1 || T > TM || n > DEC_PREP_MAX) return LADIFF_ERR_SHAPE;
    const int ntiles = (T * B + 15) / 16;
    int tpw = 1;
    while (tpw < 8 && (ntiles + 2 * tpw - 1) / (2 * tpw) * H * n >= 160) tpw *= 2;
    hipLaunchKernelGGL(dec_cross_prep_kernel, dim3((ntiles + tpw - 1) / tpw, H, n), dim3(256), 0, s, pb, B, T, tpw);
    LADIFF_LAUNCH_CHECK();
    return 0;
}

int launch_decoder_cross_apply(const float* x, const float* bo, const float* g2, const float* b2, const int32_t* counts, int B, int F,
                               int T, const float* gu_ws, float* y, float* ys, hipStream_t s, const int32_t* row_off, const float* g1,
                               const float* b1) {
    if (B == 0 || F == 0) return 0;
    if (T < 1 || T > TM) return LADIFF_ERR_SHAPE;
    const float* gu = gu_ws;
    const float* cc = gu_ws + (size_t)B * H * T * 2 * D;
    int chunks = (512 + B - 1) / B;
    if (chunks < 1) chunks = 1;
    if (chunks > (F + 3) / 4) chunks = (F + 3) / 4;
    const int rows_per_wg = ((F + chunks - 1) / chunks + 15) / 16 * 16;
    chunks = (F + rows_per_wg - 1) / rows_per_wg;
    const size_t lds = ((size_t)H * T * 2 * D + H * T) * sizeof(float);
    LADIFF_TRY(dec_cross_prepare());
#define LADIFF_DC_CASE(TT)                                                                                                   \
    case TT:                                                                                                                 \
        hipLaunchKernelGGL(dec_cross_apply_kernel<TT>, dim3(B, chunks), dim3(256), lds, s, x, gu, cc, counts, bo, g2, b2, F, \
                           rows_per_wg, y, ys, row_off, g1, b1);                                                                              \
        break;
    switch (T) {
        LADIFF_DC_CASE(1) LADIFF_DC_CASE(2) LADIFF_DC_CASE(3) LADIFF_DC_CASE(4)
        LADIFF_DC_CASE(5) LADIFF_DC_CASE(6) LADIFF_DC_CASE(7) LADIFF_DC_CASE(8)
        default: return LADIFF_ERR_SHAPE;
    }
#undef LADIFF_DC_CASE
    LADIFF_LAUNCH_CHECK();
    return 0;
}

int launch_decoder_out_cross(const float* att_s, const float* x0, const float* wo_s, const float* bo, const float* g1, const float* b1,
                             const float* bo_c, const float* g2, const float* b2, const int32_t* counts, int B, int F, int T,
                             const float* gu_ws, float* y, float* ys, hipStream_t s, const int32_t* row_off) {
    if (B == 0 || F == 0) return 0;
    if (T < 1 || T > TM) return LADIFF_ERR_SHAPE;
    int chunks = (256 + B - 1) / B;
    if (chunks > (F + OC_ROWS - 1) / OC_ROWS) chunks = (F + OC_ROWS - 1) / OC_ROWS;
    if (chunks < 1) chunks = 1;
    const int rows_per_wg = ((F + chunks - 1) / chunks + OC_ROWS - 1) / OC_ROWS * OC_ROWS;
    chunks = (F + rows_per_wg - 1) / rows_per_wg;
    LADIFF_TRY(dec_cross_prepare());
    OutCrossArgs a{att_s, x0, wo_s, bo, g1, b1, gu_ws, gu_ws + (size_t)B * H * T * 2 * D, bo_c, g2, b2, counts, row_off, y, ys, F, rows_per_wg, nullptr};
#ifdef LADIFF_STAMPS
    a.stamps = g_sys_stamps;
#endif
#define LADIFF_OC_CASE(TT) \
    case TT: hipLaunchKernelGGL(dec_out_cross_kernel<TT>, dim3(B, chunks), dim3(512), 0, s, a); break;
    switch (T) {
        LADIFF_OC_CASE(1) LADIFF_OC_CASE(2) LADIFF_OC_CASE(3) LADIFF_OC_CASE(4)
        LADIFF_OC_CASE(5) LADIFF_OC_CASE(6) LADIFF_OC_CASE(7) LADIFF_OC_CASE(8)
        default: return LADIFF_ERR_SHAPE;
    }
#undef LADIFF_OC_CASE
    LADIFF_LAUNCH_CHECK();
    return 0;
}

}
```

### ladiff_amd/csrc/decoder.hip

```cpp
#include "model.h"
#ifdef LADIFF_STAMPS
#include <cstdlib>
#endif

namespace ladiff {

#ifdef LADIFF_STAMPS
#define DEC_CUT() do { if (dec_cut >= 0 && ++dec_launched >= dec_cut) return 0; } while (0)
#else
#define DEC_CUT() do { } while (0)
#endif

constexpr int DEC_SMALL_ROWS = 4096;
std::atomic<int> g_dec_out_cross{1};
std::atomic<int> g_dec_fused_attn{1};
std::atomic<int> g_dec_final_split{1};
std::atomic<int> g_dec_small_rows_path{1};
std::atomic<int> g_dec_fused_mlp{1};

static GemmArgs lin(const float* A, int lda, const float* W, const float* bias, float* Y, int ldy, int M, int N, int K,
                    int act = ACT_NONE) {
    GemmArgs g;
    g.A = A; g.lda = lda; g.W = W; g.ldw = K; g.bias = bias; g.Y = Y; g.ldy = ldy; g.M = M; g.N = N; g.K = K; g.act = act;
    return g;
}

int vae_decode(const DecoderW& w, const DecoderW* wsp, const float* z, const int32_t* lengths, const int32_t* counts,
               const int32_t* row_off, int R, int B, int F, int T, int C, float* feats, float* ws, size_t ws_floats, hipStream_t s) {
    if (F < 1 || F > LADIFF_MAX_FRAMES || T < 1 || T > LADIFF_MAX_LATENTS || C < 1) return LADIFF_ERR_SHAPE;
    const bool ragged = row_off != nullptr;
    if (ragged && (R < 0 || (size_t)R > (size_t)B * F)) return LADIFF_ERR_SHAPE;
    const int M = ragged ? R : B * F;
    DecWs a = dec_layout(ws, B, (size_t)M, T);
    if (ws_floats < a.total) return LADIFF_ERR_WORKSPACE;
    if (M == 0) return 0;
#ifdef LADIFF_STAMPS
    const char* dec_cut_env = getenv("LADIFF_DEC_CUT");
    const int dec_cut = dec_cut_env ? atoi(dec_cut_env) : -1;
    int dec_launched = 0;
    if (dec_cut == 0) return 0;
#endif
    const bool sp = wsp != nullptr;
    if (!sp) { for (float*& t : a.Ps) t = nullptr; for (float*& t : a.SKs) t = nullptr; }
    float *const *P = a.P, *const *SK = a.SK, *const *Ps = a.Ps, *const *SKs = a.SKs;
    float *qkv = a.qkv, *att = a.att, *hid = a.hid, *kv = a.kv, *guws = a.guws, *pex = a.pex, *pexs = a.pexs, *qkv0 = a.qkv0;
    int32_t* row_out = a.row_out;
    const size_t kv_l = a.kv_layer, gu_l = a.gu_layer;

    {
        GemmArgs g[NL];
        DecCrossPrepBatch pb;
        for (int l = 0; l < NL; ++l) {
            const DecLayerW& L = w.layer[l];
            g[l] = lin(z, D, L.cross_attn.in_w + (size_t)D * D, L.cross_attn.in_b + D, kv + l * kv_l, 2 * D, T * B, 2 * D, D);
            pb.kv[l] = kv + l * kv_l; pb.wq[l] = L.cross_attn.in_w; pb.bq[l] = L.cross_attn.in_b; pb.wo[l] = L.cross_attn.out_w;
            pb.gu[l] = guws + l * gu_l;
        }
        LADIFF_TRY(launch_gemm_batch(g, NL, s)); DEC_CUT();
        LADIFF_TRY(launch_decoder_cross_prep(pb, NL, B, T, s)); DEC_CUT();
    }

    const bool small = sp && M < DEC_SMALL_ROWS && g_dec_small_rows_path;
    const bool fused_attn = sp && g_dec_fused_attn && (M >= DEC_SMALL_ROWS || g_dec_fused_attn == 2);
    auto krs = [&](const float* A, int K, const float* W, const float* bias, float* Y, float* Ys, int ldy, int N, int act,
                   const float* res, int rows) -> int {
        KrArgs g;
        g.A = A; g.lda = K; g.W = W; g.ldw = K; g.bias = bias; g.Y = Y; g.Ys = Ys; g.ldy = ldy; g.M = rows; g.N = N; g.K = K; g.act = act;
        g.res = res; g.ldres = D; g.split = 1;
        return launch_gemm_kr(g, s);
    };

    auto gemm_ln = [&](const float* A, int K, const float* W, const float* Wsp, const float* bias, const float* res,
                       const NormW& n1, const NormW* n2, float* dst, float* dsts) -> int {
        GemmArgs g = lin(A, K, sp ? Wsp : W, bias, dst, D, M, D, K);
        g.res = res; g.ldres = D;
        if (!sp) {
            g.ln_g = n1.g; g.ln_b = n1.b;
            if (n2) { g.ln2_g = n2->g; g.ln2_b = n2->b; }
            return launch_gemm(g, s);
        }
        g.split = 1;
        LADIFF_TRY(launch_gemm(g, s));
        if (n2)
            return launch_reduce_rows(dst, 1, M, nullptr, nullptr, RED_LN, n1.g, n1.b, nullptr, 0, nullptr, nullptr, 1, 1, 0,
                                      0, dst, dsts, s, nullptr, n2->g, n2->b);
        return launch_reduce_rows(dst, 1, M, nullptr, nullptr, RED_LN, n1.g, n1.b, nullptr, 0, nullptr, nullptr, 1, 1, 0, 0,
                                  dst, dsts, s);
    };

    if (ragged) { LADIFF_TRY(launch_broadcast_pe_ragged(w.query_pe, row_off, B, F, F, P[0], Ps[0], row_out, s)); DEC_CUT(); }
    else { LADIFF_TRY(launch_broadcast_pe(w.query_pe, B, F, P[0], Ps[0], s)); DEC_CUT(); }
    const float* cur = P[0]; const float* curs = Ps[0];
    for (int l = 0; l < NL; ++l) {
        const DecLayerW& L = w.layer[l];
        const DecLayerW& Ls = sp ? wsp->layer[l] : w.layer[l];
        const bool is_in = l < NSKIP, is_out = l > NSKIP, last = l == NL - 1;
        if (is_out) {
            const LinearW& sk = w.skip[l - NSKIP - 1];
            if (small) {
                RowLnArgs g;
                g.A = curs; g.lda = D; g.A2 = SKs[NL - 1 - l]; g.lda2 = D; g.K1 = D; g.W = wsp->skip[l - NSKIP - 1].w; g.ldw = 2 * D; g.bias = sk.b;
                g.Y = P[3]; g.Ys = Ps[3]; g.ldy = D; g.M = M; g.K = 2 * D;
                LADIFF_TRY(launch_gemm_rowln(g, s)); DEC_CUT();
            } else {
            GemmArgs g = lin(sp ? curs : cur, D, sp ? wsp->skip[l - NSKIP - 1].w : sk.w, sk.b, P[3], D, M, D, 2 * D);
            g.A2 = sp ? SKs[NL - 1 - l] : SK[NL - 1 - l]; g.lda2 = D; g.K1 = D;
            g.split = sp ? 1 : 0; g.Ys = Ps[3];
            LADIFF_TRY(launch_gemm(g, s)); DEC_CUT();
            }
            cur = P[3]; curs = Ps[3];
        }
        const bool shared = l == 0;
        if (shared) {
            LADIFF_TRY(launch_broadcast_pe(w.query_pe, 1, F, pex, sp ? pexs : nullptr, s)); DEC_CUT();
            if (small) { LADIFF_TRY(krs(pexs, D, Ls.self_attn.in_w, L.self_attn.in_b, qkv0, nullptr, 3 * D, 3 * D, ACT_NONE, nullptr, F)); DEC_CUT(); }
            else {
            GemmArgs g = lin(sp ? pexs : pex, D, Ls.self_attn.in_w, L.self_attn.in_b, qkv0, 3 * D, F, 3 * D, D);
            g.split = sp ? 1 : 0;
            LADIFF_TRY(launch_gemm(g, s)); DEC_CUT();
            }
        } else if (fused_attn) {
        } else if (small) {
            LADIFF_TRY(krs(curs, D, Ls.self_attn.in_w, L.self_attn.in_b, qkv, nullptr, 3 * D, 3 * D, ACT_NONE, nullptr, M)); DEC_CUT();
        } else {
            GemmArgs g = lin(sp ? curs : cur, D, Ls.self_attn.in_w, L.self_attn.in_b, qkv, 3 * D, M, 3 * D, D);
            g.split = sp ? 1 : 0;
            LADIFF_TRY(launch_gemm(g, s)); DEC_CUT();
        }
        const float* qkv_l = shared ? qkv0 : qkv;
        if (fused_attn && !shared) { LADIFF_TRY(launch_dec_qkv_attn(curs, Ls.self_attn.in_w, L.self_attn.in_b, lengths, row_off, att, B, F, 1, s)); DEC_CUT(); }
        else if (sp) { LADIFF_TRY(launch_self_attention_split(qkv_l, lengths, nullptr, att, B, F, H, 0, 1, s, row_off, shared)); DEC_CUT(); }
        else { LADIFF_TRY(launch_decoder_self_attention(qkv_l, lengths, nullptr, att, B, F, 0, s, row_off, shared)); DEC_CUT(); }
        const NormW* n1_late = nullptr;
        if (sp && !small && g_dec_out_cross) {
            LADIFF_TRY(launch_decoder_out_cross(att, cur, Ls.self_attn.out_w, L.self_attn.out_b, L.norm1.g, L.norm1.b, L.cross_attn.out_b,
                                                L.norm2.g, L.norm2.b, counts, B, F, T, guws + l * gu_l, P[2], Ps[2], s, row_off)); DEC_CUT();
        } else {
        if (sp) {
            if (small) { LADIFF_TRY(krs(att, D, Ls.self_attn.out_w, L.self_attn.out_b, P[1], nullptr, D, D, ACT_NONE, cur, M)); DEC_CUT(); }
            else {
            GemmArgs g = lin(att, D, Ls.self_attn.out_w, L.self_attn.out_b, P[1], D, M, D, D);
            g.res = cur; g.ldres = D; g.split = 1;
            LADIFF_TRY(launch_gemm(g, s)); DEC_CUT();
            }
            n1_late = &L.norm1;
        } else {
            LADIFF_TRY(gemm_ln(att, D, L.self_attn.out_w, Ls.self_attn.out_w, L.self_attn.out_b, cur, L.norm1, nullptr, P[1], nullptr)); DEC_CUT();
        }
        LADIFF_TRY(launch_decoder_cross_apply(P[1], L.cross_attn.out_b, L.norm2.g, L.norm2.b, counts, B, F, T, guws + l * gu_l, P[2],
                                              Ps[2], s, row_off, n1_late ? n1_late->g : nullptr, n1_late ? n1_late->b : nullptr)); DEC_CUT();
        }
        float* dst = is_in ? SK[l] : P[0];
        float* dsts = is_in ? SKs[l] : Ps[0];
        if (sp && g_dec_fused_mlp && (M >= dec_mlp_min_rows() || g_dec_fused_mlp == 2)) {
            LADIFF_TRY(launch_dec_mlp(Ps[2], P[2], Ls.lin1.w, L.lin1.b, Ls.lin2.w, L.lin2.b, L.norm3.g, L.norm3.b,
                                      last ? w.norm.g : nullptr, last ? w.norm.b : nullptr, dst, dsts, M, s)); DEC_CUT();
        } else if (small) {
            LADIFF_TRY(krs(Ps[2], D, Ls.lin1.w, L.lin1.b, nullptr, hid, FF, FF, ACT_GELU, nullptr, M)); DEC_CUT();
            LADIFF_TRY(krs(hid, FF, Ls.lin2.w, nullptr, qkv, nullptr, D, D, ACT_NONE, nullptr, M)); DEC_CUT();
            LADIFF_TRY(launch_reduce_rows(qkv, 4, M, L.lin2.b, P[2], RED_LN, L.norm3.g, L.norm3.b, nullptr, 0, nullptr, nullptr, 1, 1, 0, 0,
                                          dst, dsts, s, nullptr, last ? w.norm.g : nullptr, last ? w.norm.b : nullptr));
        } else {
            GemmArgs g = lin(sp ? Ps[2] : P[2], D, Ls.lin1.w, L.lin1.b, sp ? nullptr : hid, FF, M, FF, D, ACT_GELU);
            g.split = sp ? 1 : 0; if (sp) g.Ys = hid;
            LADIFF_TRY(launch_gemm(g, s)); DEC_CUT();
            LADIFF_TRY(gemm_ln(hid, FF, L.lin2.w, Ls.lin2.w, L.lin2.b, P[2], L.norm3, last ? &w.norm : nullptr, dst, dsts)); DEC_CUT();
        }
        cur = dst; curs = dsts;
    }
    if (sp && M >= DEC_SMALL_ROWS && g_dec_final_split) {
        const int Np = (C + 127) / 128 * 128;
        if ((size_t)M * Np > a.hid_floats || (size_t)Np * (D + 1) > a.qkv_floats) return LADIFF_ERR_SHAPE;
        float* wpad = qkv; float* bpad = qkv + (size_t)Np * D;
        LADIFF_TRY(launch_pad_rows(wsp->final_layer.w, w.final_layer.b, wpad, bpad, C, Np, s)); DEC_CUT();
        GemmArgs g = lin(curs, D, wpad, bpad, hid, Np, M, Np, D);
        g.split = 1;
        LADIFF_TRY(launch_gemm(g, s)); DEC_CUT();
        return launch_scatter_feats(hid, Np, C, M, F, ragged ? nullptr : lengths, ragged ? row_out : nullptr, feats, s);
    }
    GemmArgs g = lin(cur, D, w.final_layer.w, w.final_layer.b, feats, C, M, C, D);
    if (ragged) g.row_map = row_out;
    else { g.row_len = lengths; g.rows_per_item = F; }
    return launch_gemm(g, s);
}

}
```

### ladiff_amd/csrc/gemm.h

```cpp
#pragma once
#include "common.h"

namespace ladiff {

struct GemmArgs {
    const float* A = nullptr;  int lda = 0;
    const float* A2 = nullptr; int lda2 = 0;
    int K1 = 0;
    const float* W = nullptr;  int ldw = 0;
    const float* bias = nullptr;
    float* Y = nullptr;        int ldy = 0;
    float* Ys = nullptr;
    int split = 0;
    int M = 0, N = 0, K = 0;
    int act = ACT_NONE;
    const float* res = nullptr; int ldres = 0;
    const float* ln_g = nullptr; const float* ln_b = nullptr;
    const float* ln2_g = nullptr; const float* ln2_b = nullptr;
    const float* mod = nullptr;
    const int32_t* d_step = nullptr; int mod_stride = 0;
    int post_act = ACT_NONE;
    const int32_t* row_len = nullptr; int rows_per_item = 0;
    const int32_t* row_map = nullptr;
    int ksplit = 1; size_t plane = 0;
};

int launch_gemm(const GemmArgs& a, hipStream_t stream);
constexpr int GEMM_BATCH_MAX = 9;
struct GemmBatch { GemmArgs a[GEMM_BATCH_MAX]; };
int launch_gemm_batch(const GemmArgs* list, int n, hipStream_t stream);
int launch_gemm_big_batch(const GemmBatch& b, int n, hipStream_t stream);
bool gemm_big_supported(const GemmArgs& a);
int launch_gemm_big(const GemmArgs& a, hipStream_t stream);

}
```

### ladiff_amd/csrc/gemm_big.hip

```cpp
#include "gemm.h"

namespace ladiff {

namespace {
constexpr int BKB = 32;
template <int N> __device__ __forceinline__ void wait_vm() { asm volatile("s_waitcnt vmcnt(%0)" ::"n"(N) : "memory"); }
__device__ __forceinline__ void dma16(const float* g, float* l) {
    __builtin_amdgcn_global_load_lds(g, (__attribute__((address_space(3))) void*)l, 16, 0, 0);
}
}

template <int BM, int BN, int WM, int WN, bool LN>
__device__ __forceinline__ void gemm_big_body(const GemmArgs& p) {
    constexpr int NW = 4;
    static_assert(WM * WN == NW, "four waves");
    constexpr int TMW = BM / WM, TNW = BN / WN, RM = TMW / 32, RN = TNW / 32;
    constexpr int ROWS = BM + BN;
    constexpr int STAGE = ROWS * BKB;
    constexpr int GRP = 8 * NW;
    constexpr int GA = BM / GRP, GT = ROWS / GRP;
    static_assert(BM % GRP == 0 && BN % GRP == 0, "tiles are multiples of 32 rows");
    constexpr int CLD = BN + 4;
    constexpr int LDSF = (2 * STAGE > BM * CLD) ? 2 * STAGE : BM * CLD;
    constexpr int LPR = BN / 4;
    constexpr int RPI = 64 / LPR;
    constexpr int EI = BM / NW / RPI;
    static_assert(!LN || BN == 256, "LayerNorm needs whole rows");

    __shared__ __attribute__((aligned(1024))) float lds[LDSF];

    const int tid = threadIdx.x, lane = tid & 63;
    const int wave = __builtin_amdgcn_readfirstlane(tid >> 6);
    const int wm = wave / WN, wn = wave % WN;
    const int nbn = p.N / BN;
    const int nbm = (p.M + BM - 1) / BM;
    const int xcd = blockIdx.x & 7, local = blockIdx.x >> 3;
    const int bm = (local / nbn) * 8 + xcd, bn = local % nbn;
    if (bm >= nbm) return;
    const int row0 = bm * BM, col0 = bn * BN;
    const int nk = p.K / BKB;

    const int rl = 8 * wave + (lane >> 3);
    const int kl = (((lane & 7) ^ ((rl >> 1) & 7)) << 2);
    float* const lbase = lds + 8 * wave * BKB;
    auto issue = [&](int kt, int buf) __attribute__((always_inline)) {
        const int k0 = kt * BKB;
        const float* abase; int ald;
        if (k0 < p.K1) { abase = p.A + k0; ald = p.lda; } else { abase = p.A2 + (k0 - p.K1); ald = p.lda2; }
#pragma unroll
        for (int g = 0; g < GT; ++g) {
            const float* src;
            if (g < GA) {
                int gr = row0 + GRP * g + rl; gr = gr < p.M ? gr : p.M - 1;
                src = abase + (size_t)gr * ald + kl;
            } else {
                src = p.W + (size_t)(col0 + GRP * (g - GA) + rl) * p.ldw + k0 + kl;
            }
            dma16(src, lbase + buf * STAGE + GRP * g * BKB);
        }
    };

    f32x16 acc[RM][RN];
#pragma unroll
    for (int i = 0; i < RM; ++i)
#pragma unroll
        for (int j = 0; j < RN; ++j)
#pragma unroll
            for (int r = 0; r < 16; ++r) acc[i][j][r] = 0.f;

    const int frow = lane & 31, fk = lane >> 5;
    auto compute = [&](int buf) __attribute__((always_inline)) {
        const float* sa = lds + buf * STAGE + (wm * TMW) * BKB;
        const float* sb = lds + buf * STAGE + (BM + wn * TNW) * BKB;
#pragma unroll
        for (int g = 0; g < BKB / 8; ++g) {
            const int c = 2 * g + fk;
            f32x4 fa[RM], fb[RN];
#pragma unroll
            for (int i = 0; i < RM; ++i) { const int r = i * 32 + frow; fa[i] = ld4(sa + r * BKB + ((c ^ ((r >> 1) & 7)) << 2)); }
#pragma unroll
            for (int j = 0; j < RN; ++j) { const int r = j * 32 + frow; fb[j] = ld4(sb + r * BKB + ((c ^ ((r >> 1) & 7)) << 2)); }
#pragma unroll
            for (int e = 0; e < 4; ++e)
#pragma unroll
                for (int i = 0; i < RM; ++i)
#pragma unroll
                    for (int j = 0; j < RN; ++j)
                        acc[i][j] = __builtin_amdgcn_mfma_f32_32x32x2f32(fa[i][e], fb[j][e], acc[i][j], 0, 0, 0);
        }
    };

    const int er = wave * (BM / NW) + lane / LPR;
    const int ec = 4 * (lane % LPR);
    f32x4 rv[EI];
#pragma unroll
    for (int e = 0; e < EI; ++e) rv[e] = f32x4{0.f, 0.f, 0.f, 0.f};

    issue(0, 0);
    for (int kt = 0; kt < nk; ++kt) {
        const int buf = kt & 1;
        wait_vm<0>();
        __builtin_amdgcn_s_barrier();
        if (kt + 1 < nk) issue(kt + 1, buf ^ 1);
        if (kt == nk - 1 && p.res != nullptr) {
#pragma unroll
            for (int e = 0; e < EI; ++e) {
                const int gr = row0 + er + e * RPI;
                if (gr < p.M) rv[e] = ld4(p.res + (size_t)gr * p.ldres + col0 + ec);
            }
        }
        compute(buf);
    }
    __builtin_amdgcn_s_barrier();

    float* ct = lds;
#pragma unroll
    for (int i = 0; i < RM; ++i)
#pragma unroll
        for (int j = 0; j < RN; ++j)
#pragma unroll
            for (int r = 0; r < 16; ++r)
                ct[(wm * TMW + i * 32 + (r & 3) + 8 * (r >> 2) + 4 * (lane >> 5)) * CLD + wn * TNW + j * 32 + (lane & 31)] = acc[i][j][r];
    asm volatile("s_waitcnt vmcnt(0) lgkmcnt(0)" ::: "memory");
    __builtin_amdgcn_s_barrier();
#pragma unroll
    for (int e = 0; e < EI; ++e) reg_touch(rv[e]);

    f32x4 bv = {0.f, 0.f, 0.f, 0.f};
    if (p.bias != nullptr) bv = ld4(p.bias + col0 + ec);
    f32x4 g1 = bv, b1 = bv, g2 = bv, b2 = bv;
    if constexpr (LN) {
        g1 = ld4(p.ln_g + ec); b1 = ld4(p.ln_b + ec);
        if (p.ln2_g != nullptr) { g2 = ld4(p.ln2_g + ec); b2 = ld4(p.ln2_b + ec); }
    }
    act_dispatch(p.act, [&](auto ACT) __attribute__((always_inline)) {
#pragma unroll
    for (int e = 0; e < EI; ++e) {
        const int lr = er + e * RPI;
        const int gr = row0 + lr;
        f32x4 v = ld4(ct + lr * CLD + ec);
#pragma unroll
        for (int q = 0; q < 4; ++q) v[q] = act_c<decltype(ACT)::value>(v[q] + bv[q]) + rv[e][q];
        if constexpr (LN) {
#pragma unroll
            for (int pass = 0; pass < 2; ++pass) {
                if (pass == 1 && p.ln2_g == nullptr) break;
                const float mean = wave_sum((v[0] + v[1]) + (v[2] + v[3])) * (1.f / 256.f);
                float sq = 0.f;
#pragma unroll
                for (int q = 0; q < 4; ++q) { const float d = v[q] - mean; sq += d * d; }
                const float rstd = rsqrtf(wave_sum(sq) * (1.f / 256.f) + LN_EPS);
#pragma unroll
                for (int q = 0; q < 4; ++q) v[q] = (v[q] - mean) * rstd * (pass ? g2[q] : g1[q]) + (pass ? b2[q] : b1[q]);
            }
        }
        if (gr < p.M) st4(p.Y + (size_t)gr * p.ldy + col0 + ec, v);
    }
    });
}

template <int BM, int BN>
__device__ __forceinline__ void gemm_big_split_body(const GemmArgs& p) {
    constexpr int NW = 4, WM = 2, WN = 2;
    constexpr int TMW = BM / WM, TNW = BN / WN, RM = TMW / 16, RN = TNW / 16;
    constexpr int ROWS = BM + BN;
    constexpr int STAGE = ROWS * 32;
    constexpr int GRP = 8 * NW;
    constexpr int GA = BM / GRP, GT = ROWS / GRP;
    constexpr int CLD = BN + 4;
    constexpr int LPR = BN / 4, RPI = 64 / LPR, EI = BM / NW / RPI;
    constexpr int LDSF = (2 * STAGE > BM * CLD) ? 2 * STAGE : BM * CLD;

    __shared__ __attribute__((aligned(1024))) float lds[LDSF];

    const int tid = threadIdx.x, lane = tid & 63;
    const int wave = __builtin_amdgcn_readfirstlane(tid >> 6);
    const int wm = wave / WN, wn = wave % WN;
    const int argM = pin_s(p.M), argK1 = pin_s(p.K1), ldy = pin_s(p.ldy), act = pin_s(p.act);
    float* const argY = pin_s(p.Y); float* const argYs = pin_s(p.Ys);
    const int nbn = p.N / BN;
    const int nbm = (argM + BM - 1) / BM;
    const int xcd = blockIdx.x & 7, local = blockIdx.x >> 3;
    const int bm = (local / nbn) * 8 + xcd, bn = local % nbn;
    if (bm >= nbm) return;
    const int row0 = bm * BM, col0 = bn * BN;
    const int ksplit = pin_s(p.ksplit), kz = ksplit > 1 ? (int)blockIdx.y : 0;
    const int nk_all = p.K / 32, nk = nk_all / ksplit, kt0 = kz * nk;

    const int rl = 8 * wave + (lane >> 3);
    const int cs = (lane & 7) ^ ((rl >> 1) & 7);
    const int kl = (cs < 4 ? cs * 4 : 32 + (cs - 4) * 4);
    float* const lbase = lds + 8 * wave * 32;
    auto issue = [&](int ktl, int buf) __attribute__((always_inline)) {
        const int kt = kt0 + ktl;
        const int k0 = (kt >> 1) * 64, hf = (kt & 1) * 16;
        const float* abase; int ald;
        if (k0 < argK1) { abase = p.A + k0; ald = p.lda; } else { abase = p.A2 + (k0 - argK1); ald = p.lda2; }
#pragma unroll
        for (int g = 0; g < GT; ++g) {
            const float* src;
            if (g < GA) {
                int gr = row0 + GRP * g + rl; gr = gr < argM ? gr : argM - 1;
                src = abase + (size_t)gr * ald + hf + kl;
            } else {
                src = p.W + (size_t)(col0 + GRP * (g - GA) + rl) * p.ldw + k0 + hf + kl;
            }
            dma16(src, lbase + buf * STAGE + GRP * g * 32);
        }
    };

    f32x4 acc[RM][RN];
#pragma unroll
    for (int i = 0; i < RM; ++i)
#pragma unroll
        for (int j = 0; j < RN; ++j) acc[i][j] = f32x4{0.f, 0.f, 0.f, 0.f};

    const int frow = lane & 15, fk = lane >> 4;
    const int sw = (frow >> 1) & 7;
    auto compute = [&](int buf) __attribute__((always_inline)) {
        const float* sa = lds + buf * STAGE + (wm * TMW) * 32;
        const float* sb = lds + buf * STAGE + (BM + wn * TNW) * 32;
        s16x8 ah[RM], al[RM], bh[RN], bl[RN];
#pragma unroll
        for (int i = 0; i < RM; ++i) {
            const int r = i * 16 + frow;
            ah[i] = __builtin_bit_cast(s16x8, ld4(sa + r * 32 + ((fk ^ sw) << 2)));
            al[i] = __builtin_bit_cast(s16x8, ld4(sa + r * 32 + (((4 + fk) ^ sw) << 2)));
        }
#pragma unroll
        for (int j = 0; j < RN; ++j) {
            const int r = j * 16 + frow;
            bh[j] = __builtin_bit_cast(s16x8, ld4(sb + r * 32 + ((fk ^ sw) << 2)));
            bl[j] = __builtin_bit_cast(s16x8, ld4(sb + r * 32 + (((4 + fk) ^ sw) << 2)));
        }
#pragma unroll
        for (int i = 0; i < RM; ++i)
#pragma unroll
            for (int j = 0; j < RN; ++j) acc[i][j] = MFMA16_S16(al[i], bh[j], acc[i][j], 0, 0, 0);
#pragma unroll
        for (int i = 0; i < RM; ++i)
#pragma unroll
            for (int j = 0; j < RN; ++j) acc[i][j] = MFMA16_S16(ah[i], bl[j], acc[i][j], 0, 0, 0);
#pragma unroll
        for (int i = 0; i < RM; ++i)
#pragma unroll
            for (int j = 0; j < RN; ++j) acc[i][j] = MFMA16_S16(ah[i], bh[j], acc[i][j], 0, 0, 0);
    };

    const int er = wave * (BM / NW) + lane / LPR;
    const int ec = 4 * (lane % LPR);
    f32x4 rv[EI];
#pragma unroll
    for (int e = 0; e < EI; ++e) rv[e] = f32x4{0.f, 0.f, 0.f, 0.f};
    f32x4 bv = {0.f, 0.f, 0.f, 0.f};

    issue(0, 0);
    for (int kt = 0; kt < nk; ++kt) {
        const int buf = kt & 1;
        wait_vm<0>();
        __builtin_amdgcn_s_barrier();
        if (kt + 1 < nk) issue(kt + 1, buf ^ 1);
        if (kt == nk - 1 && ksplit == 1) {
            if (p.bias != nullptr) bv = ld4(p.bias + col0 + ec);
            if (p.res != nullptr) {
#pragma unroll
                for (int e = 0; e < EI; ++e) {
                    const int gr = row0 + er + e * RPI;
                    if (gr < argM) rv[e] = ld4(p.res + (size_t)gr * p.ldres + col0 + ec);
                }
            }
        }
        compute(buf);
    }
    __builtin_amdgcn_s_barrier();

    float* ct = lds;
#pragma unroll
    for (int i = 0; i < RM; ++i)
#pragma unroll
        for (int j = 0; j < RN; ++j)
#pragma unroll
            for (int r = 0; r < 4; ++r)
                ct[(wm * TMW + i * 16 + 4 * (lane >> 4) + r) * CLD + wn * TNW + j * 16 + (lane & 15)] = acc[i][j][r];
    asm volatile("s_waitcnt vmcnt(0) lgkmcnt(0)" ::: "memory");
    __builtin_amdgcn_s_barrier();
    reg_touch(bv);
#pragma unroll
    for (int e = 0; e < EI; ++e) reg_touch(rv[e]);

    if (ksplit > 1) {
        float* const Yz = argY + (size_t)kz * p.plane;
#pragma unroll
        for (int e = 0; e < EI; ++e) {
            const int lr = er + e * RPI;
            const int gr = row0 + lr;
            if (gr < argM) st4g(Yz + (size_t)gr * ldy + col0 + ec, ld4(ct + lr * CLD + ec));
        }
        return;
    }
    act_dispatch(act, [&](auto ACT) __attribute__((always_inline)) {
#pragma unroll
        for (int e = 0; e < EI; ++e) {
            const int lr = er + e * RPI;
            const int gr = row0 + lr;
            f32x4 v = ld4(ct + lr * CLD + ec);
#pragma unroll
            for (int q = 0; q < 4; ++q) v[q] = act_c<decltype(ACT)::value>(v[q] + bv[q]) + rv[e][q];
            if (gr < argM) {
                if (argY != nullptr) st4g(argY + (size_t)gr * ldy + col0 + ec, v);
                if (argYs != nullptr) store_split4g(argYs + (size_t)gr * ldy, col0 + ec, v);
            }
        }
    });
}

template <int BM, int BN>
__global__ __launch_bounds__(256, 2) void gemm_big_split_kernel(const GemmArgs p) { gemm_big_split_body<BM, BN>(p); }
template <int BM, int BN>
__global__ __launch_bounds__(256, 2) void gemm_big_split_batch_kernel(const GemmBatch b) { gemm_big_split_body<BM, BN>(b.a[blockIdx.y]); }

template <int BM, int BN, int WM, int WN, bool LN>
__global__ __launch_bounds__(256) void gemm_big_kernel(const GemmArgs p) { gemm_big_body<BM, BN, WM, WN, LN>(p); }
template <int BM, int BN, int WM, int WN, bool LN>
__global__ __launch_bounds__(256) void gemm_big_batch_kernel(const GemmBatch b) { gemm_big_body<BM, BN, WM, WN, LN>(b.a[blockIdx.y]); }

template <int BM, int BN, int WM, int WN, bool LN>
static int launch_big_batch(const GemmBatch& b, int n, hipStream_t s) {
    const GemmArgs& a = b.a[0];
    const int nbm = (a.M + BM - 1) / BM, nbn = a.N / BN;
    const int grid = ((nbm + 7) / 8) * 8 * nbn;
    hipLaunchKernelGGL((gemm_big_batch_kernel<BM, BN, WM, WN, LN>), dim3(grid, n), dim3(256), 0, s, b);
    LADIFF_LAUNCH_CHECK();
    return 0;
}

template <int BM, int BN, int WM, int WN, bool LN>
static int launch_big(const GemmArgs& a, hipStream_t s) {
    const int nbm = (a.M + BM - 1) / BM, nbn = a.N / BN;
    const int grid = ((nbm + 7) / 8) * 8 * nbn;
    hipLaunchKernelGGL((gemm_big_kernel<BM, BN, WM, WN, LN>), dim3(grid), dim3(256), 0, s, a);
    LADIFF_LAUNCH_CHECK();
    return 0;
}

bool gemm_big_supported(const GemmArgs& a) {
    if (a.split) return a.M > 0 && a.K % 64 == 0 && a.K1 % 64 == 0 && a.N % 128 == 0 && a.lda % 4 == 0 && a.ldw % 4 == 0 && (!a.A2 || a.lda2 % 4 == 0) &&
                        a.ldy % 64 == 0 && !a.ln_g && !a.mod && !a.row_len && !a.row_map && a.post_act == ACT_NONE && (a.Y || a.Ys);
    if (a.M < 4096 || a.K % BKB || a.K1 % BKB || (a.lda % 4) || (a.ldw % 4) || (a.A2 && (a.lda2 % 4))) return false;
    if ((a.ldy % 4) || (a.res && (a.ldres % 4)) || a.mod || a.row_len || a.row_map || a.post_act != ACT_NONE) return false;
    if (a.ln_g != nullptr) return a.N == 256;
    return a.N % 128 == 0;
}

int launch_gemm_big(const GemmArgs& a, hipStream_t s) {
    if (a.split) {
        const int nbm = (a.M + 127) / 128, nbn = a.N / 128;
        const int ks = a.ksplit > 1 ? a.ksplit : 1;
        if (ks > 1 && ((a.K / 32) % ks != 0 || a.Y == nullptr || a.Ys != nullptr || a.plane == 0)) return LADIFF_ERR_ARG;
        if (nbm * nbn <= 256 && a.M > 64) {
            const int nbm64 = (a.M + 63) / 64;
            hipLaunchKernelGGL((gemm_big_split_kernel<64, 128>), dim3(((nbm64 + 7) / 8) * 8 * nbn, ks), dim3(256), 0, s, a);
        } else {
            hipLaunchKernelGGL((gemm_big_split_kernel<128, 128>), dim3(((nbm + 7) / 8) * 8 * nbn, ks), dim3(256), 0, s, a);
        }
        LADIFF_LAUNCH_CHECK();
        return 0;
    }
    if (a.ksplit > 1) return LADIFF_ERR_ARG;
    if (a.ln_g != nullptr) return launch_big<64, 256, 2, 2, true>(a, s);
    return launch_big<128, 128, 2, 2, false>(a, s);
}

int launch_gemm_big_batch(const GemmBatch& b, int n, hipStream_t s) {
    for (int i = 0; i < n; ++i) if (b.a[i].ksplit > 1) return LADIFF_ERR_ARG;
    if (b.a[0].split) {
        const GemmArgs& a = b.a[0];
        const int nbm = (a.M + 127) / 128, nbn = a.N / 128;
        hipLaunchKernelGGL((gemm_big_split_batch_kernel<128, 128>), dim3(((nbm + 7) / 8) * 8 * nbn, n), dim3(256), 0, s, b);
        LADIFF_LAUNCH_CHECK();
        return 0;
    }
    if (b.a[0].ln_g != nullptr) return launch_big_batch<64, 256, 2, 2, true>(b, n, s);
    return launch_big_batch<128, 128, 2, 2, false>(b, n, s);
}

}
```

### ladiff_amd/csrc/graph_key.h

```cpp
#pragma once
#include <algorithm>
#include <cstddef>
#include <cstdint>
#include <cstdlib>
#include <cstring>

namespace ladiff {

struct GraphKey {
    static constexpr int CAPACITY = 32;
    uint64_t v[CAPACITY] = {0};
    int n = 0;

    GraphKey& add(uint64_t x) {
        if (n == CAPACITY) std::abort();
        v[n++] = x;
        return *this;
    }
    GraphKey& add(const void* p) { return add((uint64_t) reinterpret_cast<uintptr_t>(p)); }
    GraphKey& add(int x) { return add((uint64_t)(int64_t)x); }
    GraphKey& add(unsigned x) { return add((uint64_t)x); }
    GraphKey& add(float x) {
        uint32_t u;
        static_assert(sizeof(u) == sizeof(x), "float is 32 bits");
        std::memcpy(&u, &x, sizeof(u));
        return add((uint64_t)u);
    }
    bool operator==(const GraphKey& o) const { return n == o.n && std::equal(v, v + n, o.v); }
    bool operator!=(const GraphKey& o) const { return !(*this == o); }
};

inline uint64_t fnv1a_ptrs(const float* const* p, int n, uint64_t h) {
    for (int i = 0; i < n; ++i) {
        const uint64_t x = reinterpret_cast<uintptr_t>(p[i]);
        for (int b = 0; b < 8; ++b) { h ^= (x >> (8 * b)) & 0xff; h *= 1099511628211ull; }
    }
    return h;
}
inline uint64_t weights_hash(const float* const* w, const float* const* w_split, int n) {
    const uint64_t h = fnv1a_ptrs(w, n, 1469598103934665603ull);
    return w_split != nullptr ? fnv1a_ptrs(w_split, n, h ^ 0x9e3779b97f4a7c15ull) : h;
}

struct ReverseArgs {
    const float* const* w;
    const float* const* w_split;
    uint64_t weights_generation;
    const float *text_emb, *init_noise;
    const int32_t *counts, *final_counts, *h_counts;
    const float *sinusoid, *coef, *step_noise;
    float guidance_scale, init_noise_sigma;
    int cfg, B, T, n_text, n_steps;
    float* z;
    void* ws;
    size_t ws_bytes;
    int reuse_time_tables;
    void* stream;
};

inline GraphKey sampler_key(const ReverseArgs& a, int n_params, bool pipeline, int plan_mr, int plan_nb, const unsigned noise[4]) {
    GraphKey k;
    k.add(a.ws);
    k.add(a.counts);
    k.add(a.final_counts);
    k.add(a.coef);
    k.add(a.step_noise);
    k.add(a.stream);
    k.add(a.text_emb);
    k.add(a.init_noise);
    k.add(a.z);
    k.add(a.B);
    k.add(a.T);
    k.add(a.n_steps);
    k.add(a.cfg);
    k.add(a.n_text);
    k.add(a.w_split != nullptr ? 1 : 0);
    k.add(pipeline ? 1 : 0);
    k.add(pipeline ? plan_mr : 0);
    k.add(pipeline ? plan_nb : 0);
    k.add(a.guidance_scale);
    k.add(a.init_noise_sigma);
    for (int i = 0; i < 4; ++i) k.add(pipeline ? 0u : noise[i]);
    k.add(weights_hash(a.w, a.w_split, n_params));
    k.add(a.weights_generation);
    return k;
}

inline GraphKey decode_key(const float* const* w, const float* const* w_split, int n_params, uint64_t weights_generation, const float* z,
                           const int32_t* lengths, const int32_t* counts, const int32_t* row_off, int total_rows, int B, int F, int T, int C,
                           const float* feats, const void* ws, const void* stream, int dec_fused_mlp, int dec_small_rows_path,
                           int dec_final_split, int mlp_variant, int dec_fused_attn) {
    GraphKey k;
    k.add(z);
    k.add(lengths);
    k.add(counts);
    k.add(row_off);
    k.add(feats);
    k.add(ws);
    k.add(stream);
    k.add(B);
    k.add(F);
    k.add(T);
    k.add(C);
    k.add(total_rows);
    k.add(w_split != nullptr ? 1 : 0);
    k.add(dec_fused_mlp);
    k.add(dec_small_rows_path);
    k.add(dec_final_split);
    k.add(mlp_variant);
    k.add(dec_fused_attn);
    k.add(weights_hash(w, w_split, n_params));
    k.add(weights_generation);
    return k;
}

}
```

### ladiff_amd/csrc/kernels.h

```cpp
#pragma once
#include "common.h"
#include "noise_gen.h"

namespace ladiff {

enum RedMode : int { RED_PLAIN = 0, RED_LN = 1, RED_LN_ADD = 2, RED_LN_MOD = 3 };
int launch_reduce_rows(const float* P, int S, int M, const float* bias, const float* res, int mode, const float* g,
                       const float* b, const float* tab, int tab_step_stride, const int32_t* d_step,
                       const int32_t* counts, int Bs, int T, int pad_row, int b_off, float* out, float* outs, hipStream_t s,
                       const int32_t* d_base = nullptr, const float* g2 = nullptr, const float* b2 = nullptr);
int launch_split_rows(const float* x, float* y, int R, int K, hipStream_t s);
int launch_gather_rows(const float* src, const int32_t* index, int n_rows, int row_floats, float* dst, hipStream_t s);
int launch_split_range_stats(const float* const* xs, const int64_t* counts, int n, int64_t max_count, unsigned long long* stats,
                             hipStream_t s);
int launch_layernorm(const float* x, const float* g, const float* b, float* y, int M, hipStream_t s);
constexpr int DEC_PREP_MAX = 9;
struct DecCrossPrepBatch { const float* kv[DEC_PREP_MAX]; const float* wq[DEC_PREP_MAX]; const float* bq[DEC_PREP_MAX];
                           const float* wo[DEC_PREP_MAX]; float* gu[DEC_PREP_MAX]; };
constexpr int ROW_BATCH_MAX = 9;
struct RowBatch { const float* a[ROW_BATCH_MAX]; const float* g[ROW_BATCH_MAX]; const float* b[ROW_BATCH_MAX]; float* y[ROW_BATCH_MAX]; };
int launch_layernorm_batch(const RowBatch& rb, int n, int M, hipStream_t s);
int launch_ca_table_input_batch(const RowBatch& rb, int n_layers, int step_stride, int n, int B2, hipStream_t s, int split_out = 0);
int launch_ca_table_input(const float* nval, const float* beta, const float* mod, int step_stride, int n, int B2, float* u,
                          hipStream_t s);
int launch_add_pe(const float* sample, const float* pe, int Bs, int b_off, int b_n, int T, float* x, float* xs, hipStream_t s);
int launch_broadcast_pe(const float* pe, int B, int F, float* x, float* xs, hipStream_t s);
int launch_broadcast_pe_ragged(const float* pe, const int32_t* row_off, int B, int F, int F_out, float* x, float* xs, int32_t* row_out,
                               hipStream_t s);
int launch_relu(const float* x, float* y, size_t n, hipStream_t s);
int launch_pad_rows(const float* src, const float* srcb, float* dst, float* dstb, int C, int Np, hipStream_t s);
int launch_zero_fill(float* x, size_t n, hipStream_t s);
int launch_silu(const float* x, float* y, size_t n, hipStream_t s);
int launch_sinusoid(const int64_t* t, int n, float* out, hipStream_t s);
int launch_cfg_step(const float* eps, float* lat, const float* coef, const int32_t* d_step, const float* noise,
                    float g, int cfg, int B, int T, hipStream_t s);
int launch_advance(int32_t* d_step, hipStream_t s);
int launch_step_tail(float* x, float* xs, const float* ng, const float* nb, float* lat, const float* coef, int32_t* d_step,
                     const float* noise, const float* pe, float g, int cfg, int B, int T, hipStream_t s, const NoiseGen& gen = NoiseGen{0u, 0u, 0u, 0});
int launch_noise_fill(const NoiseGen& gen, int step0, int n, int B, int T, float* out, hipStream_t s);
int launch_init_latents(const float* noise, const int32_t* counts, float sigma, float* lat, int B, int T, hipStream_t s);
int launch_finalize_latents(const float* lat, const int32_t* counts, float* z, int B, int T, hipStream_t s, const unsigned* status = nullptr);

int launch_dec_qkv_attn(const float* xs, const float* w, const float* bias, const int32_t* lengths, const int32_t* row_off, float* out,
                        int B, int F, int split_out, hipStream_t s);
int launch_scatter_feats(const float* tmp, int ldt, int C, int M, int F, const int32_t* row_len, const int32_t* row_map, float* feats,
                         hipStream_t s);
int launch_pad_cols(const float* x, float* y, int R, int C, int Cp, hipStream_t s);
int launch_encoder_assemble(const float* token, const float* emb, const float* pe, const int32_t* lengths,
                            const int32_t* counts, int B, int F, int T, float* x, float* xs, uint32_t* keybits, hipStream_t s);
int launch_encoder_finalize(const float* out, const float* eps, const int32_t* counts, int B, int T, int S, float* mu, float* sd,
                            float* latent, hipStream_t s);

int launch_lca_kv(const float* key, const float* value, int B, int N, float* att, hipStream_t s);
int launch_lca_apply(const float* q, const float* att, const int32_t* counts, int Bs, int b_off, int b_n, int T, const float* mod,
                     int step_stride, int sample_stride, const int32_t* d_step, const float* g, const float* be, float* u,
                     hipStream_t s);
int launch_denoiser_self_attention_general(const float* qkv, const float* text_kv, int N, const float* tables, int kv_off,
                                           int step_stride, const int32_t* d_step, const int32_t* counts, int Bs, int b_off,
                                           int b_n, int T, float* out, hipStream_t s);

int launch_decoder_cross_prep(const DecCrossPrepBatch& pb, int n, int B, int T, hipStream_t s);
int launch_decoder_out_cross(const float* att_s, const float* x0, const float* wo_s, const float* bo, const float* g1, const float* b1,
                             const float* bo_c, const float* g2, const float* b2, const int32_t* counts, int B, int F, int T,
                             const float* gu_ws, float* y, float* ys, hipStream_t s, const int32_t* row_off);
int launch_decoder_cross_apply(const float* x, const float* bo, const float* g2, const float* b2, const int32_t* counts, int B, int F,
                               int T, const float* gu_ws, float* y, float* ys, hipStream_t s, const int32_t* row_off = nullptr,
                               const float* g1 = nullptr, const float* b1 = nullptr);

int launch_feats2joints(const float* feats, const float* mean, const float* stdv, int B, int F, int C, int J, float* joints,
                        hipStream_t s);

int launch_joint_ape_ave(const float* rst, const float* ref, const int32_t* lengths, int B, int F, int J, const int32_t* part_idx,
                         float factor, float* seq_rows, double* acc, hipStream_t s);
int launch_joint_mr(const float* rst, const float* ref, int B, int F, int J, float* seq_rows, double* acc, hipStream_t s);

int launch_denoiser_self_attention(const float* qkv, const float* text_kv, const float* tables, int kv_off,
                                   int step_stride, const int32_t* d_step, const int32_t* counts, int Bs, int b_off,
                                   int b_n, int T, float* out, int split_out, hipStream_t s);
int launch_decoder_self_attention(const float* qkv, const int32_t* lengths, const uint32_t* keybits, float* out, int B, int F,
                                  int split_out, hipStream_t s, const int32_t* row_off = nullptr, int shared_qkv = 0);
int launch_self_attention(const float* qkv, const int32_t* lengths, const uint32_t* keybits, float* out, int B, int F, int nheads,
                          int causal, int split_out, hipStream_t s, const int32_t* row_off = nullptr);
int launch_self_attention_split(const float* qkv, const int32_t* lengths, const uint32_t* keybits, float* out, int B, int F,
                                 int nheads, int causal, int split_out, hipStream_t s, const int32_t* row_off = nullptr, int shared_qkv = 0);
int launch_decoder_cross_attention(const float* q, const float* kv, const int32_t* counts, float* out, int B, int F,
                                   int T, int split_out, hipStream_t s);

}
```

### ladiff_amd/csrc/model.h

```cpp
#pragma once
#include <atomic>
#include "gemm.h"
#include "gemm_kr.h"
#include "graph_key.h"
#include "kernels.h"
#include "systolic_plan.h"
#include "weights.h"
#include "workspace.h"

namespace ladiff {

int denoiser_time_tables(const DenoiserW& w, const float* sinus, int n, float* tables, float* ws, size_t ws_floats, hipStream_t s);
int denoiser_text_cache(const DenoiserW& w, const float* text, int B2, const float* tables, int n_steps, float* cache,
                        float* ws, size_t ws_floats, hipStream_t s, int ntxt = 1);
int denoiser_forward(const DenoiserW& w, const DenoiserW* w_split, const float* tables, const int32_t* d_step,
                     const float* cache, int n_steps, const float* sample, int Bs, int dup, int T, const int32_t* counts, float* eps, float* ws,
                     size_t ws_floats, hipStream_t s, int b_lo = 0, int b_n = -1, int loop_mode = 0, int ntxt = 1,
                     const int32_t* d_base = nullptr);
int denoiser_text_static(const DenoiserW& w, const float* text, int B2, float* cache, float* ws, size_t ws_floats, hipStream_t s);
int denoiser_ctab(const DenoiserW& w, const float* tables_lo, int n, float* cache, int B2, float* u, size_t u_floats, hipStream_t s,
                  const DenoiserW* w_split = nullptr);
int linear_cross_attention(const DenoiserW& w, int layer, const float* x, const float* xf, const float* emb, const int32_t* counts,
                           int B, int T, int N, float* out, float* ws, size_t ws_floats, hipStream_t s);

struct Sampler;
int diffusion_reverse(Sampler* sp, const DenoiserW& w, const DenoiserW* w_split, const ReverseArgs& a);

extern std::atomic<int> g_dec_fused_mlp;
extern std::atomic<int> g_dec_small_rows_path;
extern std::atomic<int> g_dec_final_split;
extern std::atomic<int> g_dec_out_cross;
extern std::atomic<int> g_stage_plan;
extern std::atomic<int> g_poll_pause;
extern std::atomic<int> g_stage_delay;
extern std::atomic<int> g_pace;
extern std::atomic<int> g_look_ahead_from, g_small_upto;
extern std::atomic<int> g_dec_fused_attn;
extern std::atomic<int> g_mlp_variant;
int dec_mlp_prepare();
int dec_qkv_attn_prepare();
int dec_cross_prepare();
int dec_mlp_min_rows();
int vae_decode(const DecoderW& w, const DecoderW* w_split, const float* z, const int32_t* lengths, const int32_t* counts,
               const int32_t* row_off, int R, int B, int F, int T, int C, float* feats, float* ws, size_t ws_floats, hipStream_t s);

int launch_dec_mlp(const float* xs, const float* x, const float* w1, const float* b1, const float* w2, const float* b2, const float* g3,
                   const float* be3, const float* g4, const float* be4, float* y, float* ys, int M, hipStream_t s);

int vae_encode(const EncoderW& w, const EncoderW* w_split, const float* features, const int32_t* lengths,
               const int32_t* counts, const float* eps, int B, int F, int T, int C, float* mu, float* sd, float* latent, float* ws,
               size_t ws_floats, hipStream_t s);

#ifdef LADIFF_STAMPS
extern unsigned long long* g_sys_stamps;
extern int g_sys_probe;
#endif
bool sys_supported(int B, int T, int cfg, bool split);
extern std::atomic<int> g_waves16;
extern std::atomic<int> g_handoff;
int sys_reset_status(float* ws, hipStream_t s);
extern std::atomic<int> g_xcd_local;
int sys_build_stages(const DenoiserW& W, const DenoiserW& WS, float* ws, int MR, int NB, std::vector<unsigned char>& host);
int launch_systolic_loop(const DenoiserW& W, float* ws, const float* tables, const float* tkv, const float* ctab, int n_ctab,
                         const float* coef, const float* noise, float* lat, const int32_t* counts, float gscale, int B, int T,
                         int step_lo, int n, int fp32, int MR, int NB, hipStream_t s, int cfg = 1, int fault_wg = -1,
                         unsigned long long timeout_ticks = 0, const NoiseGen& gen = NoiseGen{0u, 0u, 0u, 0});

int launch_qkv_attention(const float* x, const float* w, const float* bias, const float* text_kv, const float* tables,
                         int kv_off, int step_stride, const int32_t* d_step, const int32_t* counts, int Bs, int b_off,
                         int b_n, int T, float* out, hipStream_t s);

int clip_text_encode(const ClipW& w, const ClipW* w_split, int n_layers, int vocab, const int64_t* ids, int B, int S, int L,
                     float* out, float* ws, size_t ws_floats, hipStream_t s, const int32_t* seq_len = nullptr,
                     const int32_t* row_off = nullptr, const int32_t* row_seq = nullptr, int total_rows = 0);

const std::vector<std::string>& t2m_move_param_names();
const std::vector<std::string>& t2m_motion_param_names();
const std::vector<std::string>& t2m_text_param_names();
int t2m_movement_encode(const float* const* w, const float* feats, int ld, int B, int F, int Cin, float* out, float* ws,
                        size_t ws_floats, hipStream_t s);
int t2m_motion_encode(const float* const* w, const float* mov, const int32_t* m_lens, int B, int T, float* out, float* ws,
                      size_t ws_floats, hipStream_t s);
int t2m_text_encode(const float* const* w, const float* word_embs, const float* pos_onehot, const int32_t* cap_lens, int B, int L,
                    float* out, float* ws, size_t ws_floats, hipStream_t s);

}
```

### ladiff_amd/csrc/rowops.hip

```cpp
#include <algorithm>

#include "kernels.h"

namespace ladiff {

constexpr int ROWS_PER_BLOCK = 4;

__device__ __forceinline__ void row_stats(const f32x4 v, float& mean, float& rstd) {
    float s = wave_sum(v[0] + v[1] + v[2] + v[3]);
    mean = s * (1.f / 256.f);
    float q = 0.f;
#pragma unroll
    for (int i = 0; i < 4; ++i) { const float d = v[i] - mean; q += d * d; }
    q = wave_sum(q);
    rstd = rsqrtf(q * (1.f / 256.f) + LN_EPS);
}

__global__ __launch_bounds__(256) void layernorm_kernel(const float* __restrict__ x, const float* __restrict__ g,
                                                        const float* __restrict__ b, float* __restrict__ y, int M) {
    const int row = blockIdx.x * ROWS_PER_BLOCK + (threadIdx.x >> 6);
    const int c = (threadIdx.x & 63) * 4;
    if (row >= M) return;
    f32x4 v = ld4(x + (size_t)row * D + c);
    float mean, rstd;
    row_stats(v, mean, rstd);
    const f32x4 gg = ld4(g + c), bb = ld4(b + c);
#pragma unroll
    for (int i = 0; i < 4; ++i) v[i] = (v[i] - mean) * rstd * gg[i] + bb[i];
    st4(y + (size_t)row * D + c, v);
}

__global__ __launch_bounds__(256) void layernorm_batch_kernel(const RowBatch rb, int M) {
    const int row = blockIdx.x * ROWS_PER_BLOCK + (threadIdx.x >> 6);
    const int c = (threadIdx.x & 63) * 4;
    if (row >= M) return;
    const int k = blockIdx.y;
    f32x4 v = ld4(rb.a[k] + (size_t)row * D + c);
    float mean, rstd;
    row_stats(v, mean, rstd);
    const f32x4 gg = ld4(rb.g[k] + c), bb = ld4(rb.b[k] + c);
#pragma unroll
    for (int i = 0; i < 4; ++i) v[i] = (v[i] - mean) * rstd * gg[i] + bb[i];
    st4(rb.y[k] + (size_t)row * D + c, v);
}
int launch_layernorm_batch(const RowBatch& rb, int n, int M, hipStream_t s) {
    if (M == 0 || n == 0) return 0;
    LADIFF_CHECK_ARG(n >= 1 && n <= ROW_BATCH_MAX);
    hipLaunchKernelGGL(layernorm_batch_kernel, dim3((M + ROWS_PER_BLOCK - 1) / ROWS_PER_BLOCK, n), dim3(256), 0, s, rb, M);
    LADIFF_LAUNCH_CHECK();
    return 0;
}

int launch_layernorm(const float* x, const float* g, const float* b, float* y, int M, hipStream_t s) {
    if (M == 0) return 0;
    hipLaunchKernelGGL(layernorm_kernel, dim3((M + ROWS_PER_BLOCK - 1) / ROWS_PER_BLOCK), dim3(256), 0, s, x, g, b, y, M);
    LADIFF_LAUNCH_CHECK();
    return 0;
}

struct RedArgs {
    const float* P; const float* bias; const float* res; const float* g; const float* b; const float* tab;
    const int32_t* d_step; const int32_t* counts; float* out; float* outs;
    const int32_t* d_base;
    const float* g2; const float* b2;
    size_t plane;
    int S, mode, tab_step_stride, Bs, T, pad_row, b_off, M;
};

__global__ __launch_bounds__(256) void reduce_rows_kernel(const RedArgs p) {
    const float* const P = pin_s(p.P); const float* const bias = pin_s(p.bias); const float* const res = pin_s(p.res);
    const float* const g = pin_s(p.g); const float* const b = pin_s(p.b); const float* const tab = pin_s(p.tab);
    const int32_t* const d_step = pin_s(p.d_step); const int32_t* const counts = pin_s(p.counts);
    const int32_t* const d_base = pin_s(p.d_base);
    float* const out = pin_s(p.out); float* const outs = pin_s(p.outs);
    const size_t plane = pin_s(p.plane);
    const int S = pin_s(p.S), mode = pin_s(p.mode), tab_step_stride = pin_s(p.tab_step_stride), Bs = pin_s(p.Bs),
              T = pin_s(p.T), pad_row = pin_s(p.pad_row), b_off = pin_s(p.b_off), M = pin_s(p.M);
    const int row = blockIdx.x * ROWS_PER_BLOCK + (threadIdx.x >> 6);
    const int c = (threadIdx.x & 63) * 4;
    if (row >= M) return;
    const f32x4 zero = {0.f, 0.f, 0.f, 0.f};
    const float* prow = P + (size_t)row * D + c;
    f32x4 pl[4];
#pragma unroll
    for (int s = 0; s < 4; ++s) pl[s] = s < S ? ld4g(prow + s * plane) : zero;
    const f32x4 bi = bias != nullptr ? ld4g(bias + c) : zero;
    const f32x4 rs = res != nullptr ? ld4g(res + (size_t)row * D + c) : zero;
    f32x4 gg = zero, bb = zero, gg2 = zero, bb2 = zero;
    if (mode != RED_PLAIN) { gg = ld4g(g + c); bb = ld4g(b + c); }
    const bool twice = mode == RED_LN && p.g2 != nullptr;
    if (twice) { gg2 = ld4g(p.g2 + c); bb2 = ld4g(p.b2 + c); }
    int step = d_step != nullptr ? *(const __attribute__((address_space(1))) int32_t*)d_step : 0;
    if (d_base != nullptr) step -= *(const __attribute__((address_space(1))) int32_t*)d_base;
    const int b2 = b_off + row / T, tt = row % T;
    int cnt = 0x7fffffff;
    if (mode == RED_LN_ADD && counts != nullptr) cnt = *(const __attribute__((address_space(1))) int32_t*)(counts + b2 % Bs);
    const float* t = tab + (size_t)step * tab_step_stride;
    f32x4 t0 = zero, t1 = zero;
    if (mode == RED_LN_ADD) { t0 = ld4g(t + (size_t)b2 * D + c); t1 = ld4g(t + (size_t)pad_row * D + c); }
    else if (mode == RED_LN_MOD) { t0 = ld4g(t + c); t1 = ld4g(t + 256 + c); }

    f32x4 v;
#pragma unroll
    for (int i = 0; i < 4; ++i) v[i] = ((pl[0][i] + pl[1][i]) + pl[2][i]) + pl[3][i] + bi[i] + rs[i];
    if (mode != RED_PLAIN) {
        float mean, rstd;
        row_stats(v, mean, rstd);
#pragma unroll
        for (int i = 0; i < 4; ++i) v[i] = (v[i] - mean) * rstd * gg[i] + bb[i];
        if (twice) {
            row_stats(v, mean, rstd);
#pragma unroll
            for (int i = 0; i < 4; ++i) v[i] = (v[i] - mean) * rstd * gg2[i] + bb2[i];
        }
        if (mode == RED_LN_ADD) {
            const bool valid = tt < cnt;
#pragma unroll
            for (int i = 0; i < 4; ++i) v[i] += valid ? t0[i] : t1[i];
        } else if (mode == RED_LN_MOD) {
#pragma unroll
            for (int i = 0; i < 4; ++i) v[i] = silu(v[i] * (1.f + t0[i]) + t1[i]);
        }
    }
    if (out != nullptr) st4g(out + (size_t)row * D + c, v);
    if (outs != nullptr) store_split4g(outs + (size_t)row * D, c, v);
}

int launch_reduce_rows(const float* P, int S, int M, const float* bias, const float* res, int mode, const float* g,
                       const float* b, const float* tab, int tab_step_stride, const int32_t* d_step,
                       const int32_t* counts, int Bs, int T, int pad_row, int b_off, float* out, float* outs, hipStream_t s,
                       const int32_t* d_base, const float* g2, const float* b2) {
    if (S < 1 || S > 4) return LADIFF_ERR_SHAPE;
    RedArgs a;
    a.g2 = g2; a.b2 = b2;
    a.P = P; a.bias = bias; a.res = res; a.g = g; a.b = b; a.tab = tab; a.d_step = d_step; a.counts = counts; a.out = out;
    a.outs = outs; a.plane = (size_t)M * D; a.S = S; a.mode = mode; a.tab_step_stride = tab_step_stride; a.Bs = Bs; a.T = T;
    a.pad_row = pad_row; a.b_off = b_off; a.M = M; a.d_base = d_base;
    hipLaunchKernelGGL(reduce_rows_kernel, dim3((M + ROWS_PER_BLOCK - 1) / ROWS_PER_BLOCK), dim3(256), 0, s, a);
    LADIFF_LAUNCH_CHECK();
    return 0;
}

__global__ __launch_bounds__(256) void ca_table_input_kernel(const float* __restrict__ nval, const float* __restrict__ beta,
                                                             const float* __restrict__ mod, int step_stride, int B2, int M,
                                                             float* __restrict__ u) {
    const int row = blockIdx.x * ROWS_PER_BLOCK + (threadIdx.x >> 6);
    const int c = (threadIdx.x & 63) * 4;
    if (row >= M) return;
    const int step = row / (B2 + 1), b = row % (B2 + 1);
    const float* m = mod + (size_t)step * step_stride;
    const f32x4 sc = ld4(m + c), sh = ld4(m + 256 + c);
    f32x4 v = b < B2 ? ld4(nval + (size_t)b * D + c) : ld4(beta + c);
#pragma unroll
    for (int i = 0; i < 4; ++i) v[i] = silu(v[i] * (1.f + sc[i]) + sh[i]);
    st4(u + (size_t)row * D + c, v);
}
__global__ __launch_bounds__(256) void ca_table_input_batch_kernel(const RowBatch rb, int step_stride, int B2, int M, int split_out) {
    const int row = blockIdx.x * ROWS_PER_BLOCK + (threadIdx.x >> 6);
    const int c = (threadIdx.x & 63) * 4;
    if (row >= M) return;
    const int k = blockIdx.y;
    const int step = row / (B2 + 1), b = row % (B2 + 1);
    const float* m = rb.b[k] + (size_t)step * step_stride;
    const f32x4 sc = ld4(m + c), sh = ld4(m + 256 + c);
    f32x4 v = b < B2 ? ld4(rb.a[k] + (size_t)b * D + c) : ld4(rb.g[k] + c);
#pragma unroll
    for (int i = 0; i < 4; ++i) v[i] = silu(v[i] * (1.f + sc[i]) + sh[i]);
    if (split_out) store_split4(rb.y[k] + (size_t)row * D, c, v);
    else st4(rb.y[k] + (size_t)row * D + c, v);
}
int launch_ca_table_input_batch(const RowBatch& rb, int n_layers, int step_stride, int n, int B2, hipStream_t s, int split_out) {
    const int M = n * (B2 + 1);
    if (M == 0 || n_layers == 0) return 0;
    LADIFF_CHECK_ARG(n_layers >= 1 && n_layers <= ROW_BATCH_MAX);
    hipLaunchKernelGGL(ca_table_input_batch_kernel, dim3((M + ROWS_PER_BLOCK - 1) / ROWS_PER_BLOCK, n_layers), dim3(256), 0, s, rb,
                       step_stride, B2, M, split_out);
    LADIFF_LAUNCH_CHECK();
    return 0;
}

int launch_ca_table_input(const float* nval, const float* beta, const float* mod, int step_stride, int n, int B2, float* u,
                          hipStream_t s) {
    const int M = n * (B2 + 1);
    hipLaunchKernelGGL(ca_table_input_kernel, dim3((M + ROWS_PER_BLOCK - 1) / ROWS_PER_BLOCK), dim3(256), 0, s, nval, beta, mod,
                       step_stride, B2, M, u);
    LADIFF_LAUNCH_CHECK();
    return 0;
}

__global__ __launch_bounds__(256) void add_pe_kernel(const float* __restrict__ sample, const float* __restrict__ pe,
                                                     int Bs, int T, int M, int b_off, float* __restrict__ x, float* __restrict__ xs) {
    const int row = blockIdx.x * ROWS_PER_BLOCK + (threadIdx.x >> 6);
    const int c = (threadIdx.x & 63) * 4;
    if (row >= M) return;
    const int b2 = b_off + row / T, t = row % T;
    f32x4 v = ld4(sample + ((size_t)(b2 % Bs) * T + t) * D + c);
    const f32x4 p = ld4(pe + (size_t)t * D + c);
#pragma unroll
    for (int i = 0; i < 4; ++i) v[i] += p[i];
    st4(x + (size_t)row * D + c, v);
    if (xs != nullptr) store_split4(xs + (size_t)row * D, c, v);
}

int launch_add_pe(const float* sample, const float* pe, int Bs, int b_off, int b_n, int T, float* x, float* xs, hipStream_t s) {
    const int M = b_n * T;
    hipLaunchKernelGGL(add_pe_kernel, dim3((M + ROWS_PER_BLOCK - 1) / ROWS_PER_BLOCK), dim3(256), 0, s, sample, pe, Bs, T, M, b_off, x, xs);
    LADIFF_LAUNCH_CHECK();
    return 0;
}

__global__ __launch_bounds__(256) void broadcast_pe_kernel(const float* __restrict__ pe, int F, int M, float* __restrict__ x,
                                                           float* __restrict__ xs) {
    const int row = blockIdx.x * ROWS_PER_BLOCK + (threadIdx.x >> 6);
    const int c = (threadIdx.x & 63) * 4;
    if (row >= M) return;
    const f32x4 v = ld4(pe + (size_t)(row % F) * D + c);
    st4(x + (size_t)row * D + c, v);
    if (xs != nullptr) store_split4(xs + (size_t)row * D, c, v);
}

__global__ __launch_bounds__(256) void broadcast_pe_ragged_kernel(const float* __restrict__ pe, const int32_t* __restrict__ row_off,
                                                                  int F, int F_out, float* __restrict__ x, float* __restrict__ xs,
                                                                  int32_t* __restrict__ row_out) {
    const int b = blockIdx.y, f = blockIdx.x * ROWS_PER_BLOCK + (threadIdx.x >> 6);
    const int c = (threadIdx.x & 63) * 4;
    const int r0 = row_off[b];
    if (f >= F || f >= row_off[b + 1] - r0) return;
    const size_t row = (size_t)r0 + f;
    const f32x4 v = ld4(pe + (size_t)f * D + c);
    st4(x + row * D + c, v);
    if (xs != nullptr) store_split4(xs + row * D, c, v);
    if (c == 0) row_out[row] = b * F_out + f;
}
int launch_broadcast_pe_ragged(const float* pe, const int32_t* row_off, int B, int F, int F_out, float* x, float* xs, int32_t* row_out,
                               hipStream_t s) {
    if (B == 0) return 0;
    hipLaunchKernelGGL(broadcast_pe_ragged_kernel, dim3((F + ROWS_PER_BLOCK - 1) / ROWS_PER_BLOCK, B), dim3(256), 0, s, pe, row_off, F,
                       F_out, x, xs, row_out);
    LADIFF_LAUNCH_CHECK();
    return 0;
}

int launch_broadcast_pe(const float* pe, int B, int F, float* x, float* xs, hipStream_t s) {
    const int M = B * F;
    hipLaunchKernelGGL(broadcast_pe_kernel, dim3((M + ROWS_PER_BLOCK - 1) / ROWS_PER_BLOCK), dim3(256), 0, s, pe, F, M, x, xs);
    LADIFF_LAUNCH_CHECK();
    return 0;
}

__global__ __launch_bounds__(256) void gather_rows_kernel(const float* __restrict__ src, const int32_t* __restrict__ index, int n_rows,
                                                          int row4, float* __restrict__ dst) {
    const int row = blockIdx.x * ROWS_PER_BLOCK + (threadIdx.x >> 6);
    if (row >= n_rows) return;
    const float* s = src + (size_t)index[row] * row4 * 4;
    float* d = dst + (size_t)row * row4 * 4;
    for (int c = threadIdx.x & 63; c < row4; c += 64) st4(d + c * 4, ld4(s + c * 4));
}
int launch_gather_rows(const float* src, const int32_t* index, int n_rows, int row_floats, float* dst, hipStream_t s) {
    if (n_rows == 0) return 0;
    hipLaunchKernelGGL(gather_rows_kernel, dim3((n_rows + ROWS_PER_BLOCK - 1) / ROWS_PER_BLOCK), dim3(256), 0, s, src, index, n_rows,
                       row_floats / 4, dst);
    LADIFF_LAUNCH_CHECK();
    return 0;
}

__global__ __launch_bounds__(256) void split_rows_kernel(const float* __restrict__ x, float* __restrict__ y, int K, size_t n4) {
    const size_t i = (size_t)blockIdx.x * 256 + threadIdx.x;
    if (i >= n4) return;
    const size_t row = (i * 4) / K;
    const int k = (int)((i * 4) % K);
    store_split4(y + row * K, k, ld4(x + i * 4));
}
int launch_split_rows(const float* x, float* y, int R, int K, hipStream_t s) {
    const size_t n4 = (size_t)R * K / 4;
    hipLaunchKernelGGL(split_rows_kernel, dim3((unsigned)((n4 + 255) / 256)), dim3(256), 0, s, x, y, K, n4);
    LADIFF_LAUNCH_CHECK();
    return 0;
}

#ifndef LADIFF_SPLIT_BF16
constexpr float SPLIT_EXACT_MAX = 65504.f;
#else
constexpr float SPLIT_EXACT_MAX = 3.402823466e38f;
#endif

struct SplitRangeAcc {
    float max_abs = 0.f, max_err = 0.f;
    uint32_t nonfinite = 0, beyond = 0, coarse = 0;
    __device__ __forceinline__ void add(float x, float hi, float lo) {
        const float ax = fabsf(x);
        if (!(ax <= 3.402823466e38f)) {
            ++nonfinite;
            if (ax == __builtin_huge_valf()) max_abs = ax;
            return;
        }
        max_abs = fmaxf(max_abs, ax);
        if (ax > SPLIT_EXACT_MAX) ++beyond;
        const float err = fabsf((x - hi) - lo);
        max_err = fmaxf(max_err, err);
        if (ax != 0.f && err > ax * 0x1p-11f) ++coarse;
    }
};

__global__ __launch_bounds__(256) void split_range_stats_kernel(const float* const* __restrict__ xs, const int64_t* __restrict__ counts,
                                                                unsigned long long* __restrict__ stats) {
    const int t = blockIdx.y;
    const int64_t c = counts[t];
    if (c <= 0) return;
    const float* __restrict__ x = xs[t];
    const size_t n = (size_t)c, stride = (size_t)gridDim.x * 256;
    const size_t tid = (size_t)blockIdx.x * 256 + threadIdx.x;
    const size_t n4 = (reinterpret_cast<uintptr_t>(x) & 15) == 0 ? n / 4 : 0;
    SplitRangeAcc a;
    for (size_t i = tid; i < n4; i += stride) {
        const f32x4 v = ld4(x + i * 4);
        s16x4 hi, lo;
        split4(v, hi, lo);
#pragma unroll
        for (int j = 0; j < 4; ++j) a.add(v[j], (float)hi[j], (float)lo[j]);
    }
    for (size_t i = n4 * 4 + tid; i < n; i += stride) {
        const float v = x[i];
        s16x2 hi, lo;
        split2(v, 0.f, hi, lo);
        a.add(v, (float)hi[0], (float)lo[0]);
    }
    const float m = wave_max_nonneg(a.max_abs), e = wave_max_nonneg(a.max_err);
    const uint32_t nf = wave_sum_u32(a.nonfinite), nb = wave_sum_u32(a.beyond), nc = wave_sum_u32(a.coarse);
    if ((threadIdx.x & 63) == 0) {
        unsigned long long* o = stats + (size_t)t * 5;
        if (m > 0.f) atomicMax(o + 0, (unsigned long long)__float_as_uint(m));
        if (e > 0.f) atomicMax(o + 1, (unsigned long long)__float_as_uint(e));
        if (nf) atomicAdd(o + 2, (unsigned long long)nf);
        if (nb) atomicAdd(o + 3, (unsigned long long)nb);
        if (nc) atomicAdd(o + 4, (unsigned long long)nc);
    }
}
int launch_split_range_stats(const float* const* xs, const int64_t* counts, int n, int64_t max_count, unsigned long long* stats,
                             hipStream_t s) {
    LADIFF_HIP(hipMemsetAsync(stats, 0, (size_t)n * 5 * sizeof(unsigned long long), s));
    const int64_t per_block = 256 * 4 * 8;
    const unsigned bx = (unsigned)std::min<int64_t>(1024, std::max<int64_t>(1, (max_count + per_block - 1) / per_block));
    hipLaunchKernelGGL(split_range_stats_kernel, dim3(bx, (unsigned)n), dim3(256), 0, s, xs, counts, stats);
    LADIFF_LAUNCH_CHECK();
    return 0;
}

__global__ __launch_bounds__(256) void pad_cols_kernel(const float* __restrict__ x, float* __restrict__ y, int C, int Cp, size_t n) {
    const size_t i = (size_t)blockIdx.x * 256 + threadIdx.x;
    if (i >= n) return;
    const size_t r = i / Cp; const int c = (int)(i % Cp);
    y[i] = c < C ? x[r * C + c] : 0.f;
}
int launch_pad_cols(const float* x, float* y, int R, int C, int Cp, hipStream_t s) {
    const size_t n = (size_t)R * Cp;
    if (n == 0) return 0;
    hipLaunchKernelGGL(pad_cols_kernel, dim3((unsigned)((n + 255) / 256)), dim3(256), 0, s, x, y, C, Cp, n);
    LADIFF_LAUNCH_CHECK();
    return 0;
}

__global__ __launch_bounds__(256) void encoder_assemble_kernel(const float* __restrict__ token, const float* __restrict__ emb,
                                                               const float* __restrict__ pe, const int32_t* __restrict__ lengths,
                                                               const int32_t* __restrict__ counts, int F, int T2, int S, int M,
                                                               float* __restrict__ x, float* __restrict__ xs,
                                                               uint32_t* __restrict__ keybits) {
    const int row = blockIdx.x * ROWS_PER_BLOCK + (threadIdx.x >> 6);
    const int c = (threadIdx.x & 63) * 4;
    if (row >= M) return;
    const int b = row / S, sq = row % S;
    f32x4 v = sq < T2 ? ld4(token + (size_t)sq * D + c) : ld4(emb + ((size_t)b * F + (sq - T2)) * D + c);
    const f32x4 p = ld4(pe + (size_t)sq * D + c);
#pragma unroll
    for (int i = 0; i < 4; ++i) v[i] += p[i];
    st4(x + (size_t)row * D + c, v);
    if (xs != nullptr) store_split4(xs + (size_t)row * D, c, v);
    if (sq < 8 && (threadIdx.x & 63) == 0) {
        const int T = T2 / 2, cnt = counts[b], len = lengths[b];
        uint32_t w = 0;
        for (int k = 32 * sq; k < 32 * sq + 32 && k < S; ++k) {
            const bool ok = k < T ? k < cnt : (k < T2 ? (k - T) < cnt : (k - T2) < len);
            if (ok) w |= 1u << (k & 31);
        }
        keybits[(size_t)b * 8 + sq] = w;
    }
}
int launch_encoder_assemble(const float* token, const float* emb, const float* pe, const int32_t* lengths,
                            const int32_t* counts, int B, int F, int T, float* x, float* xs, uint32_t* keybits, hipStream_t s) {
    const int S = 2 * T + F, M = B * S;
    if (S < 8) return LADIFF_ERR_SHAPE;
    hipLaunchKernelGGL(encoder_assemble_kernel, dim3((M + ROWS_PER_BLOCK - 1) / ROWS_PER_BLOCK), dim3(256), 0, s, token, emb, pe,
                       lengths, counts, F, 2 * T, S, M, x, xs, keybits);
    LADIFF_LAUNCH_CHECK();
    return 0;
}

__global__ __launch_bounds__(256) void encoder_finalize_kernel(const float* __restrict__ out, const float* __restrict__ eps,
                                                               const int32_t* __restrict__ counts, int B, int T, int S,
                                                               float* __restrict__ mu, float* __restrict__ sd,
                                                               float* __restrict__ latent) {
    const int row = blockIdx.x * ROWS_PER_BLOCK + (threadIdx.x >> 6);
    const int c = (threadIdx.x & 63) * 4;
    if (row >= B * T) return;
    const int b = row / T, t = row % T;
    const f32x4 m = ld4(out + ((size_t)b * S + t) * D + c), lv = ld4(out + ((size_t)b * S + T + t) * D + c);
    const size_t o = ((size_t)t * B + b) * D + c;
    const f32x4 e = ld4(eps + o);
    f32x4 sdv, z;
    const bool valid = t < counts[b];
#pragma unroll
    for (int i = 0; i < 4; ++i) { sdv[i] = sqrtf(expf(lv[i])); z[i] = valid ? m[i] + sdv[i] * e[i] : 0.f; }
    st4(mu + o, m); st4(sd + o, sdv); st4(latent + o, z);
}
int launch_encoder_finalize(const float* out, const float* eps, const int32_t* counts, int B, int T, int S, float* mu, float* sd,
                            float* latent, hipStream_t s) {
    hipLaunchKernelGGL(encoder_finalize_kernel, dim3((B * T + ROWS_PER_BLOCK - 1) / ROWS_PER_BLOCK), dim3(256), 0, s, out, eps,
                       counts, B, T, S, mu, sd, latent);
    LADIFF_LAUNCH_CHECK();
    return 0;
}

__global__ __launch_bounds__(256) void relu_kernel(const float* __restrict__ x, float* __restrict__ y, size_t n4) {
    const size_t i = (size_t)blockIdx.x * 256 + threadIdx.x;
    if (i >= n4) return;
    f32x4 v = ld4(x + i * 4);
#pragma unroll
    for (int k = 0; k < 4; ++k) v[k] = fmaxf(v[k], 0.f);
    st4(y + i * 4, v);
}
int launch_relu(const float* x, float* y, size_t n, hipStream_t s) {
    const size_t n4 = n / 4;
    hipLaunchKernelGGL(relu_kernel, dim3((unsigned)((n4 + 255) / 256)), dim3(256), 0, s, x, y, n4);
    LADIFF_LAUNCH_CHECK();
    return 0;
}

__global__ __launch_bounds__(256) void zero_fill_kernel(float* __restrict__ x, size_t n4, int tail) {
    const size_t i = (size_t)blockIdx.x * 256 + threadIdx.x;
    if (i < n4) st4(x + i * 4, f32x4{0.f, 0.f, 0.f, 0.f});
    if (blockIdx.x == 0 && (int)threadIdx.x < tail) x[n4 * 4 + threadIdx.x] = 0.f;
}
int launch_zero_fill(float* x, size_t n, hipStream_t s) {
    if (n == 0) return 0;
    const size_t n4 = n / 4;
    hipLaunchKernelGGL(zero_fill_kernel, dim3((unsigned)((n4 + 255) / 256 > 0 ? (n4 + 255) / 256 : 1)), dim3(256), 0, s, x, n4, (int)(n % 4));
    LADIFF_LAUNCH_CHECK();
    return 0;
}

__global__ __launch_bounds__(256) void pad_rows_kernel(const float* __restrict__ src, const float* __restrict__ srcb, float* __restrict__ dst,
                                                       float* __restrict__ dstb, int C) {
    const int r = blockIdx.x, t = threadIdx.x;
    const f32x4 zero = {0.f, 0.f, 0.f, 0.f};
    if (t < 64) st4(dst + (size_t)r * D + 4 * t, r < C ? ld4(src + (size_t)r * D + 4 * t) : zero);
    if (t == 64) dstb[r] = r < C ? srcb[r] : 0.f;
}
int launch_pad_rows(const float* src, const float* srcb, float* dst, float* dstb, int C, int Np, hipStream_t s) {
    hipLaunchKernelGGL(pad_rows_kernel, dim3(Np), dim3(256), 0, s, src, srcb, dst, dstb, C);
    LADIFF_LAUNCH_CHECK();
    return 0;
}

__global__ __launch_bounds__(256) void silu_kernel(const float* __restrict__ x, float* __restrict__ y, size_t n4) {
    const size_t i = (size_t)blockIdx.x * 256 + threadIdx.x;
    if (i >= n4) return;
    f32x4 v = ld4(x + i * 4);
#pragma unroll
    for (int k = 0; k < 4; ++k) v[k] = silu(v[k]);
    st4(y + i * 4, v);
}
int launch_silu(const float* x, float* y, size_t n, hipStream_t s) {
    const size_t n4 = n / 4;
    hipLaunchKernelGGL(silu_kernel, dim3((unsigned)((n4 + 255) / 256)), dim3(256), 0, s, x, y, n4);
    LADIFF_LAUNCH_CHECK();
    return 0;
}

__global__ __launch_bounds__(384) void sinusoid_kernel(const int64_t* __restrict__ t, float* __restrict__ out) {
    const int n = blockIdx.x, i = threadIdx.x;
    const float ex = (-9.210340371976184f * (float)i) / 384.f;
    const float f = (float)exp((double)ex);
    const float a = (float)t[n] * f;
    out[(size_t)n * 768 + i] = (float)cos((double)a);
    out[(size_t)n * 768 + 384 + i] = (float)sin((double)a);
}
int launch_sinusoid(const int64_t* t, int n, float* out, hipStream_t s) {
    hipLaunchKernelGGL(sinusoid_kernel, dim3(n), dim3(384), 0, s, t, out);
    LADIFF_LAUNCH_CHECK();
    return 0;
}

__global__ __launch_bounds__(256) void cfg_step_kernel(const float* __restrict__ eps, float* __restrict__ lat,
                                                       const float* __restrict__ coef, const int32_t* __restrict__ d_step,
                                                       const float* __restrict__ noise, float g, int cfg, size_t n4) {
    const size_t i = (size_t)blockIdx.x * 256 + threadIdx.x;
    if (i >= n4) return;
    const int step = *d_step;
    const float* c = coef + (size_t)step * LADIFF_COEF_STRIDE;
    const float sa = c[0], sb = c[1], kx0 = c[2], kx = c[3], ke = c[4], kn = c[5];
    f32x4 e = ld4(eps + i * 4);
    if (cfg) {
        const f32x4 ec = ld4(eps + (n4 + i) * 4);
#pragma unroll
        for (int k = 0; k < 4; ++k) e[k] = e[k] + g * (ec[k] - e[k]);
    }
    f32x4 x = ld4(lat + i * 4);
    f32x4 z = {0.f, 0.f, 0.f, 0.f};
    if (noise != nullptr && kn != 0.f) z = ld4(noise + ((size_t)step * n4 + i) * 4);
#pragma unroll
    for (int k = 0; k < 4; ++k) {
        const float x0 = (x[k] - sb * e[k]) / sa;
        x[k] = kx0 * x0 + kx * x[k] + ke * e[k] + kn * z[k];
    }
    st4(lat + i * 4, x);
}
int launch_cfg_step(const float* eps, float* lat, const float* coef, const int32_t* d_step, const float* noise,
                    float g, int cfg, int B, int T, hipStream_t s) {
    const size_t n4 = (size_t)B * T * D / 4;
    hipLaunchKernelGGL(cfg_step_kernel, dim3((unsigned)((n4 + 255) / 256)), dim3(256), 0, s, eps, lat, coef, d_step, noise, g, cfg, n4);
    LADIFF_LAUNCH_CHECK();
    return 0;
}

__global__ __launch_bounds__(256) void step_tail_kernel(float* __restrict__ x, float* __restrict__ xs, const float* __restrict__ ng,
                                                        const float* __restrict__ nb, float* __restrict__ lat,
                                                        const float* __restrict__ coef, int32_t* __restrict__ d_step,
                                                        const float* __restrict__ noise, const float* __restrict__ pe, float g,
                                                        int cfg, int B, int T, const NoiseGen gen) {
    const int step = d_step[0];
    const int row = blockIdx.x * ROWS_PER_BLOCK + (threadIdx.x >> 6);
    const int c = (threadIdx.x & 63) * 4;
    const int M = B * T;
    if (row < M) {
        const float* cf = coef + (size_t)step * LADIFF_COEF_STRIDE;
        const float sa = cf[0], sb = cf[1], kx0 = cf[2], kx = cf[3], ke = cf[4], kn = cf[5];
        const f32x4 gg = ld4(ng + c), bb = ld4(nb + c);
        f32x4 eu = ld4(x + (size_t)row * D + c), ec = eu;
        if (cfg) ec = ld4(x + (size_t)(M + row) * D + c);
        float mean, rstd;
        row_stats(eu, mean, rstd);
#pragma unroll
        for (int i = 0; i < 4; ++i) eu[i] = (eu[i] - mean) * rstd * gg[i] + bb[i];
        if (cfg) {
            row_stats(ec, mean, rstd);
#pragma unroll
            for (int i = 0; i < 4; ++i) ec[i] = (ec[i] - mean) * rstd * gg[i] + bb[i];
        }
        f32x4 l = ld4(lat + (size_t)row * D + c);
        f32x4 z = {0.f, 0.f, 0.f, 0.f};
        if (gen.on && kn != 0.f) {
            float zz[4];
            noise_normal4(gen, step, gen.prompt0 + (unsigned)(row / T), row % T, c / 4, zz);
            z = f32x4{zz[0], zz[1], zz[2], zz[3]};
        } else if (noise != nullptr && kn != 0.f) z = ld4(noise + ((size_t)step * M + row) * D + c);
        const f32x4 p = ld4(pe + (size_t)(row % T) * D + c);
        f32x4 xn;
#pragma unroll
        for (int i = 0; i < 4; ++i) {
            const float e = cfg ? eu[i] + g * (ec[i] - eu[i]) : eu[i];
            const float x0 = (l[i] - sb * e) / sa;
            l[i] = kx0 * x0 + kx * l[i] + ke * e + kn * z[i];
            xn[i] = l[i] + p[i];
        }
        st4(lat + (size_t)row * D + c, l);
        st4(x + (size_t)row * D + c, xn);
        if (cfg) st4(x + (size_t)(M + row) * D + c, xn);
        if (xs != nullptr) {
            store_split4(xs + (size_t)row * D, c, xn);
            if (cfg) store_split4(xs + (size_t)(M + row) * D, c, xn);
        }
    }
    __syncthreads();
    if (threadIdx.x == 0) {
        const int ticket = atomicAdd(&d_step[1], 1);
        if (ticket == (int)gridDim.x - 1) { d_step[1] = 0; d_step[0] = step + 1; }
    }
}
int launch_step_tail(float* x, float* xs, const float* ng, const float* nb, float* lat, const float* coef, int32_t* d_step,
                     const float* noise, const float* pe, float g, int cfg, int B, int T, hipStream_t s, const NoiseGen& gen) {
    const int M = B * T;
    hipLaunchKernelGGL(step_tail_kernel, dim3((M + ROWS_PER_BLOCK - 1) / ROWS_PER_BLOCK), dim3(256), 0, s, x, xs, ng, nb, lat, coef,
                       d_step, noise, pe, g, cfg, B, T, gen);
    LADIFF_LAUNCH_CHECK();
    return 0;
}

__global__ __launch_bounds__(256) void noise_fill_kernel(const NoiseGen gen, int step0, int n, int B, int T, float* __restrict__ out) {
    const size_t i = (size_t)blockIdx.x * 256 + threadIdx.x;
    const size_t per_step = (size_t)B * T * (D / 4);
    if (i >= per_step * n) return;
    const int st = (int)(i / per_step);
    const size_t r = i % per_step;
    const int chunk = (int)(r % (D / 4)), row = (int)(r / (D / 4));
    float z[4];
    noise_normal4(gen, step0 + st, gen.prompt0 + (unsigned)(row / T), row % T, chunk, z);
    st4(out + i * 4, f32x4{z[0], z[1], z[2], z[3]});
}
int launch_noise_fill(const NoiseGen& gen, int step0, int n, int B, int T, float* out, hipStream_t s) {
    const size_t n4 = (size_t)n * B * T * (D / 4);
    if (n4 == 0) return 0;
    hipLaunchKernelGGL(noise_fill_kernel, dim3((unsigned)((n4 + 255) / 256)), dim3(256), 0, s, gen, step0, n, B, T, out);
    LADIFF_LAUNCH_CHECK();
    return 0;
}

__global__ void advance_kernel(int32_t* d_step) { if (threadIdx.x == 0) *d_step += 1; }
int launch_advance(int32_t* d_step, hipStream_t s) {
    hipLaunchKernelGGL(advance_kernel, dim3(1), dim3(64), 0, s, d_step);
    LADIFF_LAUNCH_CHECK();
    return 0;
}

__global__ __launch_bounds__(256) void init_latents_kernel(const float* __restrict__ noise, const int32_t* __restrict__ counts,
                                                           float sigma, int T, int M, float* __restrict__ lat) {
    const int row = blockIdx.x * ROWS_PER_BLOCK + (threadIdx.x >> 6);
    const int c = (threadIdx.x & 63) * 4;
    if (row >= M) return;
    const int b = row / T, t = row % T;
    f32x4 v = ld4(noise + (size_t)row * D + c);
    const bool valid = counts == nullptr || t < counts[b];
#pragma unroll
    for (int i = 0; i < 4; ++i) v[i] = valid ? v[i] * sigma : 0.f;
    st4(lat + (size_t)row * D + c, v);
}
int launch_init_latents(const float* noise, const int32_t* counts, float sigma, float* lat, int B, int T, hipStream_t s) {
    const int M = B * T;
    hipLaunchKernelGGL(init_latents_kernel, dim3((M + ROWS_PER_BLOCK - 1) / ROWS_PER_BLOCK), dim3(256), 0, s, noise, counts, sigma, T, M, lat);
    LADIFF_LAUNCH_CHECK();
    return 0;
}

__global__ __launch_bounds__(256) void finalize_latents_kernel(const float* __restrict__ lat, const int32_t* __restrict__ counts,
                                                               int B, int T, int M, float* __restrict__ z,
                                                               const unsigned* __restrict__ status) {
    const int row = blockIdx.x * ROWS_PER_BLOCK + (threadIdx.x >> 6);
    const int c = (threadIdx.x & 63) * 4;
    if (row >= M) return;
    const int b = row / T, t = row % T;
    f32x4 v = ld4(lat + (size_t)row * D + c);
    const bool valid = counts == nullptr || t < counts[b];
    if (!valid) v = f32x4{0.f, 0.f, 0.f, 0.f};
    if (status != nullptr && status[0] != 0u) { const float q = __builtin_nanf(""); v = f32x4{q, q, q, q}; }
    st4(z + ((size_t)t * B + b) * D + c, v);
}
int launch_finalize_latents(const float* lat, const int32_t* counts, float* z, int B, int T, hipStream_t s, const unsigned* status) {
    const int M = B * T;
    hipLaunchKernelGGL(finalize_latents_kernel, dim3((M + ROWS_PER_BLOCK - 1) / ROWS_PER_BLOCK), dim3(256), 0, s, lat, counts, B, T, M, z, status);
    LADIFF_LAUNCH_CHECK();
    return 0;
}

__global__ __launch_bounds__(256) void scatter_feats_kernel(const float* __restrict__ tmp, int ldt, int C, int M, int F,
                                                            const int32_t* __restrict__ row_len, const int32_t* __restrict__ row_map,
                                                            float* __restrict__ feats) {
    const int r = blockIdx.x * ROWS_PER_BLOCK + (threadIdx.x >> 6);
    const int lane = threadIdx.x & 63;
    if (r >= M) return;
    const int dst = row_map != nullptr ? row_map[r] : r;
    const bool valid = row_len == nullptr || (r % F) < row_len[r / F];
    const float* src = tmp + (size_t)r * ldt;
    float* out = feats + (size_t)dst * C;
    for (int c = lane; c < C; c += 64) out[c] = valid ? src[c] : 0.f;
}
int launch_scatter_feats(const float* tmp, int ldt, int C, int M, int F, const int32_t* row_len, const int32_t* row_map, float* feats,
                         hipStream_t s) {
    if (M == 0) return 0;
    hipLaunchKernelGGL(scatter_feats_kernel, dim3((M + ROWS_PER_BLOCK - 1) / ROWS_PER_BLOCK), dim3(256), 0, s, tmp, ldt, C, M, F, row_len, row_map, feats);
    LADIFF_LAUNCH_CHECK();
    return 0;
}

}
```

Baseline: 11350 motions/s.

## Dedupe decoder layer-0 self-attention by length group and write final GEMM directly

```diff
diff --git a/ladiff_amd/csrc/api.hip b/ladiff_amd/csrc/api.hip
--- a/ladiff_amd/csrc/api.hip
+++ b/ladiff_amd/csrc/api.hip
@@ -264,11 +264,12 @@
 }
 
 int ladiff_debug_set_decoder_fusion(int on) {
-    LADIFF_CHECK_ARG(on >= 0 && on <= 126 && (on & 3) != 3 && (on & 48) != 48);
+    LADIFF_CHECK_ARG(on >= 0 && on <= 510 && (on & 3) != 3 && (on & 48) != 48 && (on & 264) != 264);
     g_dec_out_cross = (on & 64) ? 0 : 1;
+    g_dec_layer0_once = (on & 128) ? 0 : 1;
     g_dec_fused_mlp = on & 3;
     g_dec_small_rows_path = (on & 4) ? 0 : 1;
-    g_dec_final_split = (on & 8) ? 0 : 1;
+    g_dec_final_split = (on & 8) ? 0 : (on & 256) ? 2 : 1;
     g_dec_fused_attn = (on & 16) ? 0 : (on & 32) ? 2 : 1;
     return 0;
 }
@@ -618,7 +619,8 @@
     if (ws_bytes < ladiff_decoder_workspace_bytes(B, F, T, C)) return LADIFF_ERR_WORKSPACE;
     hipStream_t s = S(stream);
     const GraphKey key = decode_key(w, w_split, DEC_NPARAMS, weights_generation, z, lengths, counts, row_off, total_rows, B, F, T, C, feats, ws,
-                                    stream, g_dec_fused_mlp, g_dec_small_rows_path, g_dec_final_split, g_mlp_variant, g_dec_fused_attn);
+                                    stream, g_dec_fused_mlp, g_dec_small_rows_path, g_dec_final_split, g_mlp_variant, g_dec_fused_attn,
+                                    g_dec_layer0_once);
     if (!(dg->exec && dg->slot.key == key && dg->slot.newest())) {
         if (dg->exec) { LADIFF_HIP(hipStreamSynchronize(s)); (void)hipGraphExecDestroy(dg->exec); dg->exec = nullptr; }
         LADIFF_TRY(dec_mlp_prepare());
diff --git a/ladiff_amd/csrc/attention.hip b/ladiff_amd/csrc/attention.hip
--- a/ladiff_amd/csrc/attention.hip
+++ b/ladiff_amd/csrc/attention.hip
@@ -152,7 +152,9 @@
 __global__ __launch_bounds__(NT, NT == 64 ? 2 : 1) void self_attn_split_kernel(const float* __restrict__ qkv, const int32_t* __restrict__ lengths,
                                                                const uint32_t* __restrict__ keybits, float* __restrict__ out,
                                                                int B, int F, int split_out, const AttnGeom g,
-                                                               const int32_t* __restrict__ row_off, int shared_qkv) {
+                                                               const int32_t* __restrict__ row_off, int shared_qkv,
+                                                               const int32_t* __restrict__ rep) {
+    if (rep != nullptr && rep[blockIdx.x / g.nheads] != (int)(blockIdx.x / g.nheads)) return;
     constexpr int NKT = FM / 32, IT = FM * 16 / NT, VLD = FM + 8;
     static_assert(FM % 32 == 0 && (FM * 16) % NT == 0 && NT % 64 == 0 && (FM / 4) % (NT / 64) == 0 && NT / 64 >= FM / 32, "a wave per query tile");
     __shared__ __attribute__((aligned(16))) s16 Kp[2 * FM * DH];
@@ -347,13 +349,14 @@
 }
 
 int launch_self_attention_split(const float* qkv, const int32_t* lengths, const uint32_t* keybits, float* out, int B, int F,
-                                 int nheads, int causal, int split_out, hipStream_t s, const int32_t* row_off, int shared_qkv) {
+                                 int nheads, int causal, int split_out, hipStream_t s, const int32_t* row_off, int shared_qkv,
+                                 const int32_t* rep) {
     if (F > SA_FMAX || F < 1 || nheads < 1) return LADIFF_ERR_SHAPE;
     if (B == 0) return 0;
     const int W = nheads * DH;
     const AttnGeom g{nheads, 3 * W, W, 2 * W, W, causal};
-    if (F <= 32) hipLaunchKernelGGL((self_attn_split_kernel<32, 64>), dim3(B * nheads), dim3(64), 0, s, qkv, lengths, keybits, out, B, F, split_out, g, row_off, shared_qkv);
-    else hipLaunchKernelGGL((self_attn_split_kernel<SA_FMAX, 512>), dim3(B * nheads), dim3(512), 0, s, qkv, lengths, keybits, out, B, F, split_out, g, row_off, shared_qkv);
+    if (F <= 32) hipLaunchKernelGGL((self_attn_split_kernel<32, 64>), dim3(B * nheads), dim3(64), 0, s, qkv, lengths, keybits, out, B, F, split_out, g, row_off, shared_qkv, rep);
+    else hipLaunchKernelGGL((self_attn_split_kernel<SA_FMAX, 512>), dim3(B * nheads), dim3(512), 0, s, qkv, lengths, keybits, out, B, F, split_out, g, row_off, shared_qkv, rep);
     LADIFF_LAUNCH_CHECK();
     return 0;
 }
diff --git a/ladiff_amd/csrc/dec_cross.hip b/ladiff_amd/csrc/dec_cross.hip
--- a/ladiff_amd/csrc/dec_cross.hip
+++ b/ladiff_amd/csrc/dec_cross.hip
@@ -216,6 +216,8 @@
     float* y; float* ys;
     int F, rows_per_wg;
     unsigned long long* stamps;
+    const int32_t* rep;
+    float* x1n;
 };
 
 #ifdef LADIFF_STAMPS
@@ -226,7 +228,7 @@
 
 __device__ __forceinline__ void oc_barrier() { asm volatile("s_waitcnt lgkmcnt(0)\n\ts_barrier" ::: "memory"); }
 
-template <int TT>
+template <int TT, int MODE = 0>
 __global__ __launch_bounds__(512, 1) void dec_out_cross_kernel(const OutCrossArgs p) {
     __shared__ __attribute__((aligned(1024))) char tile[OC_TILE];
     __shared__ __attribute__((aligned(1024))) char ps_b[OC_PS];
@@ -245,8 +247,10 @@
     const int wave = __builtin_amdgcn_readfirstlane(tid >> 6);
     int npass = 0;
     OC_STAMP(15);
+    if constexpr (MODE == 1) { if (p.rep[b] != b) return; }
     WFrag<0, 2, 1> gf, uf;
     {
+        if constexpr (MODE != 1) {
         const float* gub = p.gu + (size_t)b * HT * 2 * D;
 #pragma unroll
         for (int j = 0; j < 2; ++j) {
@@ -264,11 +268,13 @@
             split8(u0, u1, uf.hi[j][0], uf.lo[j][0]);
         }
         if (tid < 32) cs[tid] = tid < HT ? p.cc[(size_t)b * HT + tid] : 0.f;
+        }
         const float* vs[6] = {p.bo, p.g1, p.b1, p.bo_c, p.g2, p.b2};
-        if (tid < 6 * (D / 4)) st4(vec + 4 * tid, ld4(vs[tid / (D / 4)] + 4 * (tid % (D / 4))));
+        constexpr int V0 = MODE == 2 ? 3 : 0, V1 = MODE == 1 ? 3 : 6;
+        if (tid >= V0 * (D / 4) && tid < V1 * (D / 4)) st4(vec + 4 * tid, ld4(vs[tid / (D / 4)] + 4 * (tid % (D / 4))));
     }
     WFrag<0, 2, 8> wf;
-    {
+    if constexpr (MODE != 2) {
 #pragma unroll 1
         for (int half = 0; half < 2; ++half) {
             if (half == 1) __syncthreads();
@@ -309,6 +315,14 @@
     const int f1 = f0 + p.rows_per_wg < F ? f0 + p.rows_per_wg : F;
     if (f0 >= f1) return;
     const int l16 = lane & 15, grp = lane >> 4, c0 = 4 * l16, lr = 4 * wave + grp;
+    size_t rrow0 = row0;
+    if constexpr (MODE == 2) { const int rb = p.rep[b]; rrow0 = p.row_off != nullptr ? (size_t)p.row_off[rb] : (size_t)rb * p.F; }
+    f32x4 xnext[4];
+    auto ld_x1n = [&](int fb) {
+        const int f = fb + lr < f1 ? fb + lr : f1 - 1;
+#pragma unroll
+        for (int k = 0; k < 4; ++k) xnext[k] = ld4(p.x1n + (rrow0 + f) * D + c0 + 64 * k);
+    };
     typedef unsigned u32x4_o __attribute__((ext_vector_type(4)));
     const float* x0s = ps;
     auto dma_att = [&](int fb) {
@@ -331,21 +345,32 @@
             __builtin_amdgcn_global_load_lds(reinterpret_cast<const float*>(src), (__attribute__((address_space(3))) void*)(ps_b + r * 1024), 16, 0, 0);
         }
     };
+    if constexpr (MODE == 2) ld_x1n(f0);
+    else {
     dma_att(f0);
     dma_x0(f0);
     __builtin_amdgcn_s_waitcnt(0xF70);
+    }
     __syncthreads();
     for (int fb = f0; fb < f1; fb += OC_ROWS, ++npass) {
         OC_STAMP(0);
         OC_STAMP(1);
+        const int f = fb + lr;
+        const bool live = f < f1;
+        const size_t row = row0 + (live ? f : f1 - 1);
+        f32x4 xv[4];
+        if constexpr (MODE == 2) {
+#pragma unroll
+            for (int k = 0; k < 4; ++k) {
+                xv[k] = xnext[k];
+                st4(xn + lr * CLD + c0 + 64 * k, xv[k]);
+                tile_put4<0, 4>(tile, lr, c0 + 64 * k, xv[k]);
+            }
+        } else {
         f32x4 acc2[2][2];
         zero_acc(acc2);
         mma<0, 4, 2, 8, 2>(tile, wf, acc2);
         OC_STAMP(2);
-        const int f = fb + lr;
-        const bool live = f < f1;
-        const size_t row = row0 + (live ? f : f1 - 1);
-        f32x4 xv[4];
         stage_c(ct, acc2, [&](int j) { return 32 * wave + 16 * j; });
         __builtin_amdgcn_s_waitcnt(0xF70);
         __syncthreads();
@@ -373,9 +398,21 @@
                 const f32x4 ga = ld4(vec + D + c0 + 64 * k), be = ld4(vec + 2 * D + c0 + 64 * k);
 #pragma unroll
                 for (int i = 0; i < 4; ++i) xv[k][i] = (xv[k][i] - mean1) * rstd1 * ga[i] + be[i];
+                if constexpr (MODE == 1) {
+                    if (live) st4(p.x1n + row * D + c0 + 64 * k, xv[k]);
+                } else {
                 st4(xn + lr * CLD + c0 + 64 * k, xv[k]);
                 tile_put4<0, 4>(tile, lr, c0 + 64 * k, xv[k]);
-            }
+                }
+            }
+        }
+        }
+        if constexpr (MODE == 1) {
+            __syncthreads();
+            if (fb + OC_ROWS < f1) { dma_att(fb + OC_ROWS); dma_x0(fb + OC_ROWS); }
+            __builtin_amdgcn_s_waitcnt(0xF70);
+            __syncthreads();
+            continue;
         }
         OC_STAMP(4);
         __syncthreads();
@@ -411,7 +448,7 @@
         }
         __syncthreads();
         OC_STAMP(6);
-        if (fb + OC_ROWS < f1) dma_att(fb + OC_ROWS);
+        if (fb + OC_ROWS < f1) { if constexpr (MODE == 2) ld_x1n(fb + OC_ROWS); else dma_att(fb + OC_ROWS); }
         {
             float tot[2];
 #pragma unroll
@@ -453,7 +490,7 @@
         zero_acc(ao);
         mma<0, 1, 2, 1, 2>(ptile, uf, ao);
         stage_c(ct, ao, [&](int j) { return 32 * wave + 16 * j; });
-        __builtin_amdgcn_s_waitcnt(0xF70);
+        if constexpr (MODE == 0) __builtin_amdgcn_s_waitcnt(0xF70);
         oc_barrier();
         OC_STAMP(8);
         {
@@ -465,7 +502,7 @@
 #pragma unroll
                 for (int i = 0; i < 4; ++i) acc[k][i] = (bc[i] + x1[i]) + o[i];
             }
-            if (fb + OC_ROWS < f1) dma_x0(fb + OC_ROWS);
+            if constexpr (MODE == 0) { if (fb + OC_ROWS < f1) dma_x0(fb + OC_ROWS); }
             float sum = 0.f;
 #pragma unroll
             for (int k = 0; k < 4; ++k) sum += (acc[k][0] + acc[k][1]) + (acc[k][2] + acc[k][3]);
@@ -564,7 +601,8 @@
     const int rows_per_wg = ((F + chunks - 1) / chunks + OC_ROWS - 1) / OC_ROWS * OC_ROWS;
     chunks = (F + rows_per_wg - 1) / rows_per_wg;
     LADIFF_TRY(dec_cross_prepare());
-    OutCrossArgs a{att_s, x0, wo_s, bo, g1, b1, gu_ws, gu_ws + (size_t)B * H * T * 2 * D, bo_c, g2, b2, counts, row_off, y, ys, F, rows_per_wg, nullptr};
+    OutCrossArgs a{att_s, x0, wo_s, bo, g1, b1, gu_ws, gu_ws + (size_t)B * H * T * 2 * D, bo_c, g2, b2, counts, row_off, y, ys, F, rows_per_wg, nullptr,
+                   nullptr, nullptr};
 #ifdef LADIFF_STAMPS
     a.stamps = g_sys_stamps;
 #endif
@@ -580,4 +618,40 @@
     return 0;
 }
 
-}
+int launch_decoder_out_cross_front(const float* att_s, const float* x0, const float* wo_s, const float* bo, const float* g1, const float* b1,
+                                   const int32_t* rep, int B, int F, float* x1n, hipStream_t s, const int32_t* row_off) {
+    if (B == 0 || F == 0) return 0;
+    LADIFF_TRY(dec_cross_prepare());
+    OutCrossArgs a{att_s, x0, wo_s, bo, g1, b1, nullptr, nullptr, nullptr, nullptr, nullptr, nullptr, row_off, nullptr, nullptr, F, OC_ROWS, nullptr,
+                   rep, x1n};
+    hipLaunchKernelGGL((dec_out_cross_kernel<1, 1>), dim3(B, (F + OC_ROWS - 1) / OC_ROWS), dim3(512), 0, s, a);
+    LADIFF_LAUNCH_CHECK();
+    return 0;
+}
+
+int launch_decoder_out_cross_back(const float* x1n, const int32_t* rep, const float* bo_c, const float* g2, const float* b2,
+                                  const int32_t* counts, int B, int F, int T, const float* gu_ws, float* y, float* ys, hipStream_t s,
+                                  const int32_t* row_off) {
+    if (B == 0 || F == 0) return 0;
+    if (T < 1 || T > TM) return LADIFF_ERR_SHAPE;
+    int chunks = (256 + B - 1) / B;
+    if (chunks > (F + OC_ROWS - 1) / OC_ROWS) chunks = (F + OC_ROWS - 1) / OC_ROWS;
+    if (chunks < 1) chunks = 1;
+    const int rows_per_wg = ((F + chunks - 1) / chunks + OC_ROWS - 1) / OC_ROWS * OC_ROWS;
+    chunks = (F + rows_per_wg - 1) / rows_per_wg;
+    LADIFF_TRY(dec_cross_prepare());
+    OutCrossArgs a{nullptr, nullptr, nullptr, nullptr, nullptr, nullptr, gu_ws, gu_ws + (size_t)B * H * T * 2 * D, bo_c, g2, b2, counts, row_off, y, ys, F,
+                   rows_per_wg, nullptr, rep, const_cast<float*>(x1n)};
+#define LADIFF_OC_CASE(TT) \
+    case TT: hipLaunchKernelGGL((dec_out_cross_kernel<TT, 2>), dim3(B, chunks), dim3(512), 0, s, a); break;
+    switch (T) {
+        LADIFF_OC_CASE(1) LADIFF_OC_CASE(2) LADIFF_OC_CASE(3) LADIFF_OC_CASE(4)
+        LADIFF_OC_CASE(5) LADIFF_OC_CASE(6) LADIFF_OC_CASE(7) LADIFF_OC_CASE(8)
+        default: return LADIFF_ERR_SHAPE;
+    }
+#undef LADIFF_OC_CASE
+    LADIFF_LAUNCH_CHECK();
+    return 0;
+}
+
+}
diff --git a/ladiff_amd/csrc/decoder.hip b/ladiff_amd/csrc/decoder.hip
--- a/ladiff_amd/csrc/decoder.hip
+++ b/ladiff_amd/csrc/decoder.hip
@@ -13,6 +13,7 @@
 
 constexpr int DEC_SMALL_ROWS = 4096;
 std::atomic<int> g_dec_out_cross{1};
+std::atomic<int> g_dec_layer0_once{1};
 std::atomic<int> g_dec_fused_attn{1};
 std::atomic<int> g_dec_final_split{1};
 std::atomic<int> g_dec_small_rows_path{1};
@@ -91,6 +92,12 @@
     if (ragged) { LADIFF_TRY(launch_broadcast_pe_ragged(w.query_pe, row_off, B, F, F, P[0], Ps[0], row_out, s)); DEC_CUT(); }
     else { LADIFF_TRY(launch_broadcast_pe(w.query_pe, B, F, P[0], Ps[0], s)); DEC_CUT(); }
     const float* cur = P[0]; const float* curs = Ps[0];
+    const bool l0_once = sp && !small && g_dec_out_cross && M >= DEC_SMALL_ROWS && g_dec_layer0_once;
+    int32_t* const rep = reinterpret_cast<int32_t*>(qkv);
+    if (l0_once) {
+        if ((size_t)B > a.qkv_floats) return LADIFF_ERR_SHAPE;
+        LADIFF_TRY(launch_group_lengths(lengths, B, rep, s)); DEC_CUT();
+    }
     for (int l = 0; l < NL; ++l) {
         const DecLayerW& L = w.layer[l];
         const DecLayerW& Ls = sp ? wsp->layer[l] : w.layer[l];
@@ -129,10 +136,14 @@
         }
         const float* qkv_l = shared ? qkv0 : qkv;
         if (fused_attn && !shared) { LADIFF_TRY(launch_dec_qkv_attn(curs, Ls.self_attn.in_w, L.self_attn.in_b, lengths, row_off, att, B, F, 1, s)); DEC_CUT(); }
-        else if (sp) { LADIFF_TRY(launch_self_attention_split(qkv_l, lengths, nullptr, att, B, F, H, 0, 1, s, row_off, shared)); DEC_CUT(); }
+        else if (sp) { LADIFF_TRY(launch_self_attention_split(qkv_l, lengths, nullptr, att, B, F, H, 0, 1, s, row_off, shared, shared && l0_once ? rep : nullptr)); DEC_CUT(); }
         else { LADIFF_TRY(launch_decoder_self_attention(qkv_l, lengths, nullptr, att, B, F, 0, s, row_off, shared)); DEC_CUT(); }
         const NormW* n1_late = nullptr;
-        if (sp && !small && g_dec_out_cross) {
+        if (shared && l0_once) {
+            LADIFF_TRY(launch_decoder_out_cross_front(att, cur, Ls.self_attn.out_w, L.self_attn.out_b, L.norm1.g, L.norm1.b, rep, B, F, P[1], s, row_off)); DEC_CUT();
+            LADIFF_TRY(launch_decoder_out_cross_back(P[1], rep, L.cross_attn.out_b, L.norm2.g, L.norm2.b, counts, B, F, T, guws + l * gu_l, P[2], Ps[2],
+                                                     s, row_off)); DEC_CUT();
+        } else if (sp && !small && g_dec_out_cross) {
             LADIFF_TRY(launch_decoder_out_cross(att, cur, Ls.self_attn.out_w, L.self_attn.out_b, L.norm1.g, L.norm1.b, L.cross_attn.out_b,
                                                 L.norm2.g, L.norm2.b, counts, B, F, T, guws + l * gu_l, P[2], Ps[2], s, row_off)); DEC_CUT();
         } else {
@@ -170,11 +181,18 @@
     }
     if (sp && M >= DEC_SMALL_ROWS && g_dec_final_split) {
         const int Np = (C + 127) / 128 * 128;
-        if ((size_t)M * Np > a.hid_floats || (size_t)Np * (D + 1) > a.qkv_floats) return LADIFF_ERR_SHAPE;
+        const bool direct = g_dec_final_split != 2;
+        if ((!direct && (size_t)M * Np > a.hid_floats) || (size_t)Np * (D + 1) > a.qkv_floats) return LADIFF_ERR_SHAPE;
         float* wpad = qkv; float* bpad = qkv + (size_t)Np * D;
         LADIFF_TRY(launch_pad_rows(wsp->final_layer.w, w.final_layer.b, wpad, bpad, C, Np, s)); DEC_CUT();
-        GemmArgs g = lin(curs, D, wpad, bpad, hid, Np, M, Np, D);
+        GemmArgs g = lin(curs, D, wpad, bpad, direct ? feats : hid, direct ? C : Np, M, Np, D);
         g.split = 1;
+        if (direct) {
+            g.ncol = C;
+            if (ragged) g.row_map = row_out;
+            else { g.row_len = lengths; g.rows_per_item = F; }
+            return launch_gemm(g, s);
+        }
         LADIFF_TRY(launch_gemm(g, s)); DEC_CUT();
         return launch_scatter_feats(hid, Np, C, M, F, ragged ? nullptr : lengths, ragged ? row_out : nullptr, feats, s);
     }
diff --git a/ladiff_amd/csrc/gemm.h b/ladiff_amd/csrc/gemm.h
--- a/ladiff_amd/csrc/gemm.h
+++ b/ladiff_amd/csrc/gemm.h
@@ -23,6 +23,7 @@
     const int32_t* row_len = nullptr; int rows_per_item = 0;
     const int32_t* row_map = nullptr;
     int ksplit = 1; size_t plane = 0;
+    int ncol = 0;
 };
 
 int launch_gemm(const GemmArgs& a, hipStream_t stream);
diff --git a/ladiff_amd/csrc/gemm_big.hip b/ladiff_amd/csrc/gemm_big.hip
--- a/ladiff_amd/csrc/gemm_big.hip
+++ b/ladiff_amd/csrc/gemm_big.hip
@@ -159,7 +159,7 @@
     });
 }
 
-template <int BM, int BN>
+template <int BM, int BN, bool NARROW = false>
 __device__ __forceinline__ void gemm_big_split_body(const GemmArgs& p) {
     constexpr int NW = 4, WM = 2, WN = 2;
     constexpr int TMW = BM / WM, TNW = BN / WN, RM = TMW / 16, RN = TNW / 16;
@@ -253,6 +253,10 @@
 #pragma unroll
     for (int e = 0; e < EI; ++e) rv[e] = f32x4{0.f, 0.f, 0.f, 0.f};
     f32x4 bv = {0.f, 0.f, 0.f, 0.f};
+    int orow_l = -1, zero_l = 0;
+    float bc[BN / 64];
+#pragma unroll
+    for (int h = 0; h < BN / 64; ++h) bc[h] = 0.f;
 
     issue(0, 0);
     for (int kt = 0; kt < nk; ++kt) {
@@ -260,6 +264,18 @@
         wait_vm<0>();
         __builtin_amdgcn_s_barrier();
         if (kt + 1 < nk) issue(kt + 1, buf ^ 1);
+        if constexpr (NARROW) {
+            if (kt == nk - 1) {
+                const int ncol = pin_s(p.ncol);
+#pragma unroll
+                for (int h = 0; h < BN / 64; ++h) { const int gc = col0 + 64 * h + lane; if (p.bias != nullptr && gc < ncol) bc[h] = p.bias[gc]; }
+                const int gr = row0 + wave * (BM / NW) + lane;
+                if (lane < BM / NW && gr < argM) {
+                    orow_l = p.row_map != nullptr ? p.row_map[gr] : gr;
+                    if (p.row_len != nullptr) zero_l = (gr % p.rows_per_item) >= p.row_len[gr / p.rows_per_item];
+                }
+            }
+        } else
         if (kt == nk - 1 && ksplit == 1) {
             if (p.bias != nullptr) bv = ld4(p.bias + col0 + ec);
             if (p.res != nullptr) {
@@ -288,6 +304,27 @@
 #pragma unroll
     for (int e = 0; e < EI; ++e) reg_touch(rv[e]);
 
+    if constexpr (NARROW) {
+        const int ncol = pin_s(p.ncol);
+        asm volatile("" : "+v"(orow_l), "+v"(zero_l));
+#pragma unroll
+        for (int h = 0; h < BN / 64; ++h) asm volatile("" : "+v"(bc[h]));
+#pragma unroll
+        for (int r = 0; r < BM / NW; ++r) {
+            const int lr = wave * (BM / NW) + r;
+            const int orow = __builtin_amdgcn_readlane(orow_l, r);
+            const bool zero = __builtin_amdgcn_readlane(zero_l, r) != 0;
+            if (orow < 0) break;
+            float* const yr = argY + (size_t)orow * ldy + col0;
+#pragma unroll
+            for (int h = 0; h < BN / 64; ++h) {
+                const int c = 64 * h + lane;
+                const float v = (ct[lr * CLD + c] + bc[h]) + 0.f;
+                if (col0 + c < ncol) *(__attribute__((address_space(1))) float*)(yr + c) = zero ? 0.f : v;
+            }
+        }
+        return;
+    }
     if (ksplit > 1) {
         float* const Yz = argY + (size_t)kz * p.plane;
 #pragma unroll
@@ -314,8 +351,8 @@
     });
 }
 
-template <int BM, int BN>
-__global__ __launch_bounds__(256, 2) void gemm_big_split_kernel(const GemmArgs p) { gemm_big_split_body<BM, BN>(p); }
+template <int BM, int BN, bool NARROW = false>
+__global__ __launch_bounds__(256, 2) void gemm_big_split_kernel(const GemmArgs p) { gemm_big_split_body<BM, BN, NARROW>(p); }
 template <int BM, int BN>
 __global__ __launch_bounds__(256, 2) void gemm_big_split_batch_kernel(const GemmBatch b) { gemm_big_split_body<BM, BN>(b.a[blockIdx.y]); }
 
@@ -344,6 +381,10 @@
 }
 
 bool gemm_big_supported(const GemmArgs& a) {
+    if (a.split && a.ncol > 0)
+        return a.M > 0 && a.K % 64 == 0 && a.K1 % 64 == 0 && a.N % 128 == 0 && a.lda % 4 == 0 && a.ldw % 4 == 0 && (!a.A2 || a.lda2 % 4 == 0) &&
+               a.ncol <= a.N && a.ldy >= a.ncol && a.Y && !a.Ys && !a.res && a.act == ACT_NONE && !a.ln_g && !a.mod && a.post_act == ACT_NONE &&
+               a.ksplit <= 1 && (!a.row_len || a.rows_per_item > 0);
     if (a.split) return a.M > 0 && a.K % 64 == 0 && a.K1 % 64 == 0 && a.N % 128 == 0 && a.lda % 4 == 0 && a.ldw % 4 == 0 && (!a.A2 || a.lda2 % 4 == 0) &&
                         a.ldy % 64 == 0 && !a.ln_g && !a.mod && !a.row_len && !a.row_map && a.post_act == ACT_NONE && (a.Y || a.Ys);
     if (a.M < 4096 || a.K % BKB || a.K1 % BKB || (a.lda % 4) || (a.ldw % 4) || (a.A2 && (a.lda2 % 4))) return false;
@@ -357,7 +398,10 @@
         const int nbm = (a.M + 127) / 128, nbn = a.N / 128;
         const int ks = a.ksplit > 1 ? a.ksplit : 1;
         if (ks > 1 && ((a.K / 32) % ks != 0 || a.Y == nullptr || a.Ys != nullptr || a.plane == 0)) return LADIFF_ERR_ARG;
-        if (nbm * nbn <= 256 && a.M > 64) {
+        if (a.ncol > 0) {
+            if (nbm * nbn <= 256 && a.M > 64) hipLaunchKernelGGL((gemm_big_split_kernel<64, 128, true>), dim3((((a.M + 63) / 64 + 7) / 8) * 8 * nbn), dim3(256), 0, s, a);
+            else hipLaunchKernelGGL((gemm_big_split_kernel<128, 128, true>), dim3(((nbm + 7) / 8) * 8 * nbn), dim3(256), 0, s, a);
+        } else if (nbm * nbn <= 256 && a.M > 64) {
             const int nbm64 = (a.M + 63) / 64;
             hipLaunchKernelGGL((gemm_big_split_kernel<64, 128>), dim3(((nbm64 + 7) / 8) * 8 * nbn, ks), dim3(256), 0, s, a);
         } else {
diff --git a/ladiff_amd/csrc/graph_key.h b/ladiff_amd/csrc/graph_key.h
--- a/ladiff_amd/csrc/graph_key.h
+++ b/ladiff_amd/csrc/graph_key.h
@@ -89,7 +89,7 @@
 inline GraphKey decode_key(const float* const* w, const float* const* w_split, int n_params, uint64_t weights_generation, const float* z,
                            const int32_t* lengths, const int32_t* counts, const int32_t* row_off, int total_rows, int B, int F, int T, int C,
                            const float* feats, const void* ws, const void* stream, int dec_fused_mlp, int dec_small_rows_path,
-                           int dec_final_split, int mlp_variant, int dec_fused_attn) {
+                           int dec_final_split, int mlp_variant, int dec_fused_attn, int dec_layer0_once = 1) {
     GraphKey k;
     k.add(z);
     k.add(lengths);
@@ -109,6 +109,7 @@
     k.add(dec_final_split);
     k.add(mlp_variant);
     k.add(dec_fused_attn);
+    k.add(dec_layer0_once);
     k.add(weights_hash(w, w_split, n_params));
     k.add(weights_generation);
     return k;
diff --git a/ladiff_amd/csrc/kernels.h b/ladiff_amd/csrc/kernels.h
--- a/ladiff_amd/csrc/kernels.h
+++ b/ladiff_amd/csrc/kernels.h
@@ -29,6 +29,7 @@
                                hipStream_t s);
 int launch_relu(const float* x, float* y, size_t n, hipStream_t s);
 int launch_pad_rows(const float* src, const float* srcb, float* dst, float* dstb, int C, int Np, hipStream_t s);
+int launch_group_lengths(const int32_t* lengths, int B, int32_t* rep, hipStream_t s);
 int launch_zero_fill(float* x, size_t n, hipStream_t s);
 int launch_silu(const float* x, float* y, size_t n, hipStream_t s);
 int launch_sinusoid(const int64_t* t, int n, float* out, hipStream_t s);
@@ -63,6 +64,11 @@
 int launch_decoder_out_cross(const float* att_s, const float* x0, const float* wo_s, const float* bo, const float* g1, const float* b1,
                              const float* bo_c, const float* g2, const float* b2, const int32_t* counts, int B, int F, int T,
                              const float* gu_ws, float* y, float* ys, hipStream_t s, const int32_t* row_off);
+int launch_decoder_out_cross_front(const float* att_s, const float* x0, const float* wo_s, const float* bo, const float* g1, const float* b1,
+                                   const int32_t* rep, int B, int F, float* x1n, hipStream_t s, const int32_t* row_off);
+int launch_decoder_out_cross_back(const float* x1n, const int32_t* rep, const float* bo_c, const float* g2, const float* b2,
+                                  const int32_t* counts, int B, int F, int T, const float* gu_ws, float* y, float* ys, hipStream_t s,
+                                  const int32_t* row_off);
 int launch_decoder_cross_apply(const float* x, const float* bo, const float* g2, const float* b2, const int32_t* counts, int B, int F,
                                int T, const float* gu_ws, float* y, float* ys, hipStream_t s, const int32_t* row_off = nullptr,
                                const float* g1 = nullptr, const float* b1 = nullptr);
@@ -82,7 +88,8 @@
 int launch_self_attention(const float* qkv, const int32_t* lengths, const uint32_t* keybits, float* out, int B, int F, int nheads,
                           int causal, int split_out, hipStream_t s, const int32_t* row_off = nullptr);
 int launch_self_attention_split(const float* qkv, const int32_t* lengths, const uint32_t* keybits, float* out, int B, int F,
-                                 int nheads, int causal, int split_out, hipStream_t s, const int32_t* row_off = nullptr, int shared_qkv = 0);
+                                 int nheads, int causal, int split_out, hipStream_t s, const int32_t* row_off = nullptr, int shared_qkv = 0,
+                                 const int32_t* rep = nullptr);
 int launch_decoder_cross_attention(const float* q, const float* kv, const int32_t* counts, float* out, int B, int F,
                                    int T, int split_out, hipStream_t s);
 
diff --git a/ladiff_amd/csrc/model.h b/ladiff_amd/csrc/model.h
--- a/ladiff_amd/csrc/model.h
+++ b/ladiff_amd/csrc/model.h
@@ -30,6 +30,7 @@
 extern std::atomic<int> g_dec_small_rows_path;
 extern std::atomic<int> g_dec_final_split;
 extern std::atomic<int> g_dec_out_cross;
+extern std::atomic<int> g_dec_layer0_once;
 extern std::atomic<int> g_stage_plan;
 extern std::atomic<int> g_poll_pause;
 extern std::atomic<int> g_stage_delay;
diff --git a/ladiff_amd/csrc/rowops.hip b/ladiff_amd/csrc/rowops.hip
--- a/ladiff_amd/csrc/rowops.hip
+++ b/ladiff_amd/csrc/rowops.hip
@@ -461,6 +461,21 @@
     return 0;
 }
 
+__global__ __launch_bounds__(256) void group_lengths_kernel(const int32_t* __restrict__ lengths, int B, int32_t* __restrict__ rep) {
+    for (int b = threadIdx.x; b < B; b += 256) {
+        const int len = lengths[b];
+        int r = 0;
+        while (lengths[r] != len) ++r;
+        rep[b] = r;
+    }
+}
+int launch_group_lengths(const int32_t* lengths, int B, int32_t* rep, hipStream_t s) {
+    if (B == 0) return 0;
+    hipLaunchKernelGGL(group_lengths_kernel, dim3(1), dim3(256), 0, s, lengths, B, rep);
+    LADIFF_LAUNCH_CHECK();
+    return 0;
+}
+
 __global__ __launch_bounds__(256) void silu_kernel(const float* __restrict__ x, float* __restrict__ y, size_t n4) {
     const size_t i = (size_t)blockIdx.x * 256 + threadIdx.x;
     if (i >= n4) return;
```

Result: no change. 11340 motions/s (-0.1%).
